# haowenz/chromap

Measured on AMD Instinct MI355X. Metric: M paired reads mapped/s (ATAC preset, GRCh38 index), higher is better.
Workload: dtype u64

## Files before the change

chromap_amd/csrc/cm_api.hip:

```cpp
#include <hip/hip_runtime.h>
#include <math.h>
#include <stdio.h>
#include <stdlib.h>
#include <string.h>

#include <string>
#include <vector>

#include "../../include/chromap_amd.h"
#include "cm_ctx.h"
#include "cm_kernels.h"
#include "cm_classes.h"
#include "cm_summary.h"
#include "cm_coop.h"
#include <chrono>
#include <mutex>
#include "cm_mapq_tables.h"

static thread_local std::string g_last_error;

#define HIPCHECK(ctx, call)                                                                      \
  do {                                                                                           \
    hipError_t e_ = (call);                                                                      \
    if (e_ != hipSuccess) {                                                                      \
// ... 770 lines not shown
  CmDev d;
  uint32_t n_mm = 0;
  bool s3a_done = false;
  uint32_t n_heavy[CM_HV_LISTS] = {};
  unsigned long long hits_total = 0;
  uint32_t n_hits = 0;
  bool planes = false;
  bool spec = false;
  uint32_t n_m = 0;
  void bind() { cm_bind_dev(c, d, rlo, rhi); }
};
static int stage_begin(RangeRun &r) {
  cmgpu_ctx *c = r.c;
  c->n_ev = 0;
  c->use_perm = false;
  const int rc = ensure_pair_arrays(c, r.n);
  if (rc) return rc;
  HIPCHECK(c, hipMemsetAsync(c->stats.p, 0, CM_ST_N * 8, r.s));
  memset(&r.d, 0, sizeof(r.d));
  cm_ensure_goff(c);
  cm_set_classes(c, r.d);
  r.bind();
  mark(c, "begin");
  if (c->has_barcodes) {
    cm_launch_k_s0b_barcode(r.d, r.n, r.s);
    mark(c, "s0b_barcode");
  }
  return CMGPU_OK;
}
struct MmChunks {
  uint32_t n_chunks;
  uint32_t lo[CM_MM_CHUNKS + 1];
  uint64_t entries[CM_MM_CHUNKS];
  uint32_t part_off[CM_MM_CHUNKS + 1];
};
static uint32_t mm_chunk_count(const RangeRun &r) { return r.n >= (1u << 20) ? (uint32_t)r.c->opt.mm_chunks : (r.n >= (1u << 17) ? 2 : 1); }
static void mm_probe_grids(const cmgpu_ctx *c, MmChunks &k) {
  k.part_off[0] = 0;
  for (uint32_t ch = 0; ch < k.n_chunks; ++ch) k.part_off[ch + 1] = k.part_off[ch] + cm_probe_range_blocks(k.entries[ch], c->opt.probe_variant);
}
template <class Fill>
static int mm_fill_and_probe(RangeRun &r, const MmChunks &k, uint32_t mm_cap, Fill fill) {
  cmgpu_ctx *c = r.c;
  const unsigned long long *marks = (const unsigned long long *)c->mm_marks.p;
  HIPCHECK(c, hipMemsetAsync(r.d.stats + CM_ST_PROBE_STEPS, 0, 2 * 8, r.s));
  for (uint32_t ch = 0; ch < k.n_chunks; ++ch) {
    fill(ch);
    HIPCHECK(c, hipEventRecord(c->chunk_ev[ch], r.s));
    HIPCHECK(c, hipStreamWaitEvent(c->stream2, c->chunk_ev[ch], 0));
    cm_launch_k_probe_range(r.d, marks + ch, k.entries[ch], mm_cap, (uint2 *)c->partials.p + k.part_off[ch], c->stream2, c->opt.probe_variant);
  }
  HIPCHECK(c, hipEventRecord(c->chunk_ev[CM_MM_CHUNKS], c->stream2));
  HIPCHECK(c, hipStreamWaitEvent(r.s, c->chunk_ev[CM_MM_CHUNKS], 0));
  cm_launch_k_probe_reduce(c->partials.p, k.part_off[k.n_chunks], r.d.stats + CM_ST_PROBE_STEPS, r.s);
  return CMGPU_OK;
}
static int stage_minimizers_fused(RangeRun &r, bool flat) {
  cmgpu_ctx *c = r.c; CmDev &d = r.d; hipStream_t s = r.s;
  const uint32_t n = r.n, n2 = r.n2;
  int rc;
  uint64_t cap = (uint64_t)n2 * (c->max_read_len / 4 + 3);
  const uint64_t bound = (uint64_t)c->bases0 + c->bases1 + 1;
  if (cap > bound) cap = bound;
  const uint32_t ppb = flat ? 128u : cm_prep_mm_pairs_per_block(d, c->max_read_len);
  const uint64_t per_read_bound = c->max_read_len > (uint32_t)c->p.k ? c->max_read_len - (uint32_t)c->p.k + 1 : 1;
  MmChunks k;
  k.n_chunks = mm_chunk_count(r);
  for (int attempt = 0; attempt < 2; ++attempt) {
    if (cap > r.limit) return CM_RC_SPLIT;
    k.lo[0] = 0;
    uint32_t chunk_pairs = 0;
    for (uint32_t ch = 0; ch < k.n_chunks; ++ch) {
      uint64_t hi = (uint64_t)n * (ch + 1) / k.n_chunks;
      hi = ch + 1 == k.n_chunks ? n : hi / ppb * ppb;
      k.lo[ch + 1] = (uint32_t)hi;
      const uint32_t pairs = k.lo[ch + 1] - k.lo[ch];
      chunk_pairs = pairs > chunk_pairs ? pairs : chunk_pairs;
      const uint64_t me = 2ull * pairs * (attempt == 0 ? (uint64_t)(c->max_read_len / 4 + 3) : per_read_bound);
      k.entries[ch] = me > cap ? cap : me;
    }
    mm_probe_grids(c, k);
    if (c->mm_hash.ensure((size_t)cap * 8 + 8) || c->mm_ps.ensure((size_t)cap * 4 + 4) || c->pr_val.ensure((size_t)cap * 8 + 8) ||
        (!flat && c->mm_stage.ensure(cm_prep_mm_stage_bytes(d, c->max_read_len, chunk_pairs) + 8)) ||
        c->pr_kind.ensure((size_t)cap + 4) || c->mm_cursor.ensure(8) || c->mm_marks.ensure((CM_MM_CHUNKS + 1) * 8) ||
        c->partials.ensure(((size_t)k.part_off[k.n_chunks] + 1) * 8 + cm_stats_partial_words(n) * 8)) {
      cm_set_error(c, "out of device memory (minimizers)"); return CMGPU_ENOMEM;
    }
    r.bind();
    HIPCHECK(c, hipMemsetAsync(c->mm_cursor.p, 0, 8, s));
    HIPCHECK(c, hipMemsetAsync(c->mm_marks.p, 0, 8, s));
    unsigned long long *cursor = (unsigned long long *)c->mm_cursor.p, *marks = (unsigned long long *)c->mm_marks.p;
    rc = mm_fill_and_probe(r, k, (uint32_t)cap, [&](uint32_t ch) {
      if (flat) cm_launch_k_prep_flat(d, k.lo[ch], k.lo[ch + 1], c->max_read_len, (uint32_t)c->opt.prep_tile_reads, (uint32_t)cap, cursor, s);
      else cm_launch_k_prep_mm(d, k.lo[ch], k.lo[ch + 1], c->max_read_len, (uint32_t)cap, cursor, s, c->mm_stage.p);
      cm_launch_k_copy_u64(cursor, marks + ch + 1, s);
    });
    if (rc) return rc;
    d.mm_cap = (uint32_t)cap;
    HIPCHECK(c, hipMemsetAsync(c->hv_cnt.p, 0, 256, s));
    cm_launch_k_s3a_count(d, n2, s);
    d.mm_cap = 0;
    if ((rc = scan_with_total(c, d.hit_tot, d.hit_off, n2, &r.hits_total, false))) return rc;
    HIPCHECK(c, hipMemcpyAsync(r.n_heavy, c->hv_cnt.p, sizeof(r.n_heavy), hipMemcpyDeviceToHost, s));
    r.s3a_done = true;
    unsigned long long hm[CM_MM_CHUNKS + 1];
    HIPCHECK(c, hipMemcpyAsync(hm, marks, ((size_t)k.n_chunks + 1) * 8, hipMemcpyDeviceToHost, s));
    HIPCHECK(c, cm_stream_sync(s));
    const unsigned long long tot = hm[k.n_chunks];
    bool grid_short = false;
    if (attempt == 0 && tot <= cap)
      for (uint32_t ch = 0; ch < k.n_chunks; ++ch) grid_short = grid_short || hm[ch + 1] - hm[ch] > k.entries[ch];
    if (tot <= cap && !grid_short) { r.n_mm = (uint32_t)tot; break; }
    if (attempt == 1) { cm_set_error(c, "minimizer arrays overflowed twice"); return CMGPU_ECAPACITY; }
    cap = bound;
  }
  mark(c, "s0_s1_s2_trim_minimizers_probe");
  return CMGPU_OK;
}
static int stage_minimizers_two_pass(RangeRun &r) {
  cmgpu_ctx *c = r.c; CmDev &d = r.d; hipStream_t s = r.s;
  int rc;
  cm_launch_k_prep_count(d, r.n, c->max_read_len, s);
  unsigned long long mm_total = 0;
  if ((rc = scan_with_total(c, d.mm_cnt, d.mm_off, r.n2, &mm_total))) return rc;
  if (mm_total > r.limit) return CM_RC_SPLIT;
  const uint32_t n_mm = r.n_mm = (uint32_t)mm_total;
  mark(c, "s0_s1a_trim_count");
  if (c->mm_hash.ensure((size_t)n_mm * 8 + 8) || c->mm_ps.ensure((size_t)n_mm * 4 + 4) || c->pr_val.ensure((size_t)n_mm * 8 + 8) ||
      c->pr_kind.ensure((size_t)n_mm + 4)) { cm_set_error(c, "out of device memory (minimizers)"); return CMGPU_ENOMEM; }
  r.bind();
  MmChunks k;
  k.n_chunks = mm_chunk_count(r);
  for (uint32_t ch = 0; ch <= k.n_chunks; ++ch) k.lo[ch] = (uint32_t)((uint64_t)r.n * ch / k.n_chunks);
  if (c->mm_marks.ensure((CM_MM_CHUNKS + 1) * 8)) { cm_set_error(c, "out of device memory (minimizers)"); return CMGPU_ENOMEM; }
  unsigned long long *marks = (unsigned long long *)c->mm_marks.p;
  unsigned long long hm[CM_MM_CHUNKS + 1];
  cm_launch_k_mm_marks(d.mm_off, k.lo, k.n_chunks + 1, marks, s);
  HIPCHECK(c, hipMemcpyAsync(hm, marks, ((size_t)k.n_chunks + 1) * 8, hipMemcpyDeviceToHost, s));
  HIPCHECK(c, cm_stream_sync(s));
  for (uint32_t ch = 0; ch < k.n_chunks; ++ch) k.entries[ch] = hm[ch + 1] - hm[ch];
  mm_probe_grids(c, k);
  if (c->partials.ensure(((size_t)k.part_off[k.n_chunks] + 1) * 8 + cm_stats_partial_words(r.n) * 8)) { cm_set_error(c, "out of device memory (partials)"); return CMGPU_ENOMEM; }
  if ((rc = mm_fill_and_probe(r, k, n_mm, [&](uint32_t ch) { cm_launch_k_mm_fill(d, k.lo[ch], k.lo[ch + 1], c->max_read_len, s); }))) return rc;
  mark(c, "s1b_s2_minimizers_probe");
  return CMGPU_OK;
}
static int stage_pack_reads(RangeRun &r) {
  cmgpu_ctx *c = r.c;
  r.planes = c->ref_pl_words != 0 && c->opt.planes;
  if (r.planes && c->read_planes.ensure((size_t)r.n2 * cm_read_pl_stride((c->max_read_len + 31) / 32) * 4 + 16)) r.planes = false;
  if (!r.planes) return CMGPU_OK;
  if (!c->stream_pack) {
    int prio_least = 0, prio_greatest = 0;
    (void)hipDeviceGetStreamPriorityRange(&prio_least, &prio_greatest);
    HIPCHECK(c, hipStreamCreateWithPriority(&c->stream_pack, hipStreamNonBlocking, prio_greatest));
  }
  HIPCHECK(c, hipEventRecord(c->chunk_ev[1], r.s));
  HIPCHECK(c, hipStreamWaitEvent(c->stream_pack, c->chunk_ev[1], 0));
  r.d.read_pl = (uint32_t *)c->read_planes.p; r.d.read_pl_w = (c->max_read_len + 31) / 32;
  cm_launch_k_pack_reads(r.d, r.n2, c->stream_pack);
  HIPCHECK(c, hipEventRecord(c->chunk_ev[0], c->stream_pack));
  return CMGPU_OK;
}
static int stage_s3_candidates(RangeRun &r) {
  cmgpu_ctx *c = r.c; CmDev &d = r.d; hipStream_t s = r.s;
  const uint32_t n2 = r.n2;
  if (!r.s3a_done) {
    HIPCHECK(c, hipMemsetAsync(c->hv_cnt.p, 0, 256, s));
    cm_launch_k_s3a_count(d, n2, s);
    HIPCHECK(c, hipMemcpyAsync(r.n_heavy, c->hv_cnt.p, sizeof(r.n_heavy), hipMemcpyDeviceToHost, s));
    const int rc = scan_with_total(c, d.hit_tot, d.hit_off, n2, &r.hits_total);
    if (rc) return rc;
  }
  if (r.hits_total > r.limit) return CM_RC_SPLIT;
  r.n_hits = (uint32_t)r.hits_total;
  if (c->hbuf.ensure((size_t)r.n_hits * 8 + 8) || c->hcnt.ensure((size_t)r.n_hits + 4)) { cm_set_error(c, "out of device memory (hits)"); return CMGPU_ENOMEM; }
  r.bind();
  mark(c, "s3a_count");
  cm_launch_k_s3b_candidates(d, n2, c->max_read_len, s);
  const uint32_t *nh = r.n_heavy;
  cm_launch_k_s3b_heavy(d, nh, s, (c->opt.coop & 1) != 0, c->max_read_len);
  c->use_perm = (uint64_t)nh[CM_L_HIT_B256B] + nh[CM_L_HIT_SLAB] + nh[CM_L_HIT_B512] + nh[CM_L_HIT_B1024] > n2 / 65536 || (uint64_t)nh[CM_L_HIT_WAVE] + nh[CM_L_HIT_WAVE_SMALL] + nh[CM_L_HIT_B256A] > n2 / 256;
  if (c->opt.heavy_last) c->use_perm = c->opt.heavy_last > 0;
  if (c->use_perm) {
    uint32_t *tmp = (uint32_t *)c->hv_tmp.p;
    cm_build_heavy_last(d, r.n, (uint32_t *)c->scratch_a.p, tmp, (uint32_t *)c->scratch_b.p, tmp + n2 + 1, (uint32_t *)c->perm_reads.p,
                        (uint32_t *)c->perm_pairs.p, (uint32_t *)c->scan_tmp.p, s);
  }
  r.bind();
  mark(c, "s3b_candidates");
  return CMGPU_OK;
}
static void size_rescue_pool(RangeRun &r) {
  cmgpu_ctx *c = r.c;
  uint64_t waves = (uint64_t)r.n2 / 512 + 64;
  if (waves > 8192) waves = 8192;
  const uint64_t slack = c->rs_pool_want ? waves * CM_POOL_GRANT / 2 : 0;
  uint64_t want = c->rs_pool_want + c->rs_pool_want / 4 + slack;
  if (c->rs_pool_want > c->rs_pool_cap) want = 2 * c->rs_pool_want + slack;
  if (want < (1u << 22)) want = 1u << 22;
  if (want > 0xfffffff0ull) want = 0xfffffff0ull;
  const auto dbg_t0 = std::chrono::steady_clock::now();
  if (c->rs_pool.ensure((size_t)want * 8) == 0 && c->rs_pool_off.ensure((size_t)r.n2 * 2 * 4 + 16) == 0) c->rs_pool_cap = (uint32_t)(c->rs_pool.cap / 8 > 0xfffffff0ull ? 0xfffffff0ull : c->rs_pool.cap / 8);
  else { c->rs_pool.release(); c->rs_pool_cap = 0; }
  if (cm_debug_pool()) fprintf(stderr, "pool ensure want %llu: %.3f ms\n", (unsigned long long)want, std::chrono::duration<double, std::milli>(std::chrono::steady_clock::now() - dbg_t0).count());
  r.bind();
}
static int stage_s4_rescue_filter(RangeRun &r) {
  cmgpu_ctx *c = r.c; CmDev &d = r.d; hipStream_t s = r.s;
  const uint32_t n2 = r.n2;
  const bool coop = (c->opt.coop & 2) != 0;
  HIPCHECK(c, hipMemsetAsync(c->rs_cnt.p, 0, CM_RS_SEGS * 64, s));
  if (coop) size_rescue_pool(r);
  cm_launch_k_s4a_rescue_count(d, n2, s, coop);
  cm_launch_k_s4a_rescue_list(d, n2, s, coop);
  unsigned long long m_total = 0;
  r.spec = r.allow_spec && c->opt.spec && c->pred_m_ok && (c->pred_n == r.n || c->pred_n == 0xffffffffu) && c->m_cap > 0 && c->m_cap <= r.limit;
  if (r.spec) {
    unsigned long long *acc = (unsigned long long *)c->stats.p + CM_ST_TOTAL;
    HIPCHECK(c, hipMemsetAsync(acc, 0, 8, s));
    cm_launch_k_sum_u32(d.m_tot, n2, acc, s);
    cm_scan_u32(d.m_tot, d.m_off, n2, (uint32_t *)c->scan_tmp.p, s);
    cm_launch_k_check_cap(acc, c->m_cap, (unsigned long long *)c->stats.p + CM_ST_ABORT, s);
    r.n_m = (uint32_t)c->m_cap;
  } else {
    const int rc = scan_with_total(c, d.m_tot, d.m_off, n2, &m_total);
    if (rc) return rc;
    if (m_total > r.limit) return CM_RC_SPLIT;
    uint64_t want = m_total + m_total / 4 + 1024;
    if (want > r.limit) want = r.limit;
    if (want < m_total) want = m_total;
    r.n_m = (uint32_t)want;
    if (cm_ensure_candidate_arrays(c, r.n_m)) { cm_set_error(c, "out of device memory (candidates)"); return CMGPU_ENOMEM; }
    c->m_cap = r.n_m;
  }
  if (cm_debug_pool()) fprintf(stderr, "spec %d m_cap %llu m_total %llu\n", (int)r.spec, (unsigned long long)c->m_cap, m_total);
  r.bind();
  mark(c, "s4a_rescue_count");
  cm_launch_k_s4b_rescue_merge(d, n2, s, coop, c->max_read_len);
  cm_launch_k_s4b_rescue_list(d, n2, s, coop, c->max_read_len);
  mark(c, "s4b_rescue_merge");
  HIPCHECK(c, hipMemsetAsync(c->srt_cnt.p, 0, 8, s));
  cm_launch_k_s4c_reduce(d, r.n, s, (uint32_t)c->opt.coop & (c->p.split ? ~8u : ~0u));
  if (c->use_perm) cm_launch_k_sort_lists(d, 0, s);
  mark(c, "s4c_pair_filter");
  return CMGPU_OK;
}
static int stage_s5_verify(RangeRun &r) {
  cmgpu_ctx *c = r.c; const CmDev &d = r.d; hipStream_t s = r.s;
  const bool coop = (c->opt.coop & 8) != 0 && !c->p.split;
  if (r.planes) HIPCHECK(c, hipStreamWaitEvent(s, c->chunk_ev[0], 0));
  cm_launch_k_s5a_prepare(d, r.n2, s, coop);
  cm_scan_u32(d.nv, d.v_off, r.n2, (uint32_t *)c->scan_tmp.p, s);
  mark(c, "s5a_prepare");
  cm_launch_k_s5b_verify(d, r.n_m, r.n2, s);
  mark(c, "s5b_verify");
  HIPCHECK(c, hipMemsetAsync(c->srt_cnt.p, 0, 8, s));
  cm_launch_k_s5c_finalize(d, r.n2, s, coop);
  if (c->use_perm) cm_launch_k_sort_lists(d, 1, s);
  mark(c, "s5c_accept");
  return CMGPU_OK;
}
static int stage_s6_records(RangeRun &r) {
  cmgpu_ctx *c = r.c; CmDev &d = r.d; hipStream_t s = r.s;
  const uint32_t n = r.n;
  const bool coop = (c->opt.coop & 16) != 0;
  if (c->p.sam) {
    const uint64_t slots = c->single ? n : r.n2, slot0 = c->single ? r.rlo : 2ull * r.rlo;
    const uint32_t md_cap = c->sam_md_cap;
    const uint32_t zw = (2 * c->p.e + 2 <= 18) ? 5 : 8;
    if (c->sam_z.ensure((size_t)c->max_read_len * zw * 4 * n + 16)) { cm_set_error(c, "out of device memory (SAM buffers)"); return CMGPU_ENOMEM; }
    HIPCHECK(c, hipMemsetAsync((uint8_t *)c->sam_rec.p + slot0 * 40, 0, slots * 40, s));
    d.sam_rec = (uint8_t *)c->sam_rec.p + slot0 * 40; d.sam_cigar = (uint32_t *)c->sam_cigar.p + slot0 * CM_SAM_CIGAR_CAP;
    d.sam_md = (uint8_t *)c->sam_md.p + slot0 * md_cap;
    d.sam_z = (uint32_t *)c->sam_z.p; d.sam_md_cap = md_cap;
  }
  if (c->p.sam) cm_launch_k_s6a_pair_sam(d, n, s); else cm_launch_k_s6a_pair(d, n, s, coop);
  mark(c, "s6a_pairing");
  const uint32_t n_chunks = cm_num_chunks_host(n, (uint32_t)c->p.ref_batch, (uint32_t)c->p.grain);
  cm_launch_k_s6b_sample(d, n_chunks, s);
  if (c->p.sam) cm_launch_k_s6c_multi_sam(d, n, s); else cm_launch_k_s6c_multi(d, n, s, coop);
  mark(c, "s6bc_multimappers");
  return CMGPU_OK;
}
static int stage_finish(RangeRun &r, uint64_t *k_out, cmgpu_stats *stats) {
  cmgpu_ctx *c = r.c; hipStream_t s = r.s;
  cm_launch_k_stats(r.d, r.n, (unsigned long long *)c->partials.p, s);
  unsigned long long hst[CM_ST_N];
  uint32_t h_cls[CM_HV_LISTS];
  HIPCHECK(c, hipMemcpyAsync(hst, c->stats.p, sizeof(hst), hipMemcpyDeviceToHost, s));
  HIPCHECK(c, hipMemcpyAsync(h_cls, c->hv_cnt.p, sizeof(h_cls), hipMemcpyDeviceToHost, s));
  HIPCHECK(c, cm_stream_sync(s));
  mark(c, "stats");
  HIPCHECK(c, cm_stream_sync(s));
  const bool aborted = r.spec && hst[CM_ST_ABORT];
  if (!aborted) {
    unsigned long long seen = 0, keep = 0;
    for (uint32_t l = 6; l < CM_HV_LISTS; ++l) if (h_cls[l]) seen |= 1ull << (l == 31 ? 23 : l);
    if (seen & ~r.d.cls_mask) return CM_RC_AGAIN_ALL_CLASSES;
    for (uint32_t l = 0; l < 64; ++l) {
      if ((seen >> l) & 1ull) c->cls_age[l] = 32; else if (c->cls_age[l]) --c->cls_age[l];
      if (c->cls_age[l]) keep |= 1ull << l;
    }
    c->cls_seen = keep;
  } else {
    c->pred_m_ok = false;
    return CM_RC_AGAIN_EXACT_SIZES;
  }
  c->pred_m_ok = true;
  c->pred_n = r.n;
  c->rs_pool_want = hst[CM_ST_POOL];
  if (cm_debug_pool()) fprintf(stderr, "pool: cap %u entries, asked %llu\n", c->rs_pool_cap, (unsigned long long)hst[CM_ST_POOL]);
  if (hst[CM_ST_ERR]) { cm_set_error(c, "internal device error flag " + std::to_string((unsigned long long)hst[CM_ST_ERR])); return CMGPU_ECAPACITY; }
  *k_out = hst[CM_ST_RECORDS];
  c->last_range_lo = r.rlo; c->last_range_hi = r.rhi;
  c->last_n_mm = r.n_mm; c->last_n_hits = r.n_hits; c->last_n_cand_cap = r.n_m;
  if (stats) {
    stats->num_candidates += hst[CM_ST_CAND]; stats->num_mappings += hst[CM_ST_MAPPINGS];
    stats->num_mapped_reads += hst[CM_ST_MAPPED]; stats->num_uniquely_mapped_reads += hst[CM_ST_UNIQ];
    stats->num_minimizers += r.n_mm; stats->probe_steps += hst[CM_ST_PROBE_STEPS]; stats->occurrences_read += hst[CM_ST_OCC];
    stats->num_pairs_rescued += hst[CM_ST_RESCUED]; stats->num_multi_mappers += hst[CM_ST_MULTI];
    stats->num_barcode_in_whitelist += hst[CM_ST_BC_INWL]; stats->num_corrected_barcode += hst[CM_ST_BC_CORR];
  }
  return CMGPU_OK;
}
static int map_range(cmgpu_ctx *c, uint32_t rlo, uint32_t rhi, uint64_t *k_out, cmgpu_stats *stats) {
  bool allow_spec = true;
  int rc;
  *k_out = 0;
  for (;;) {
    RangeRun r = {c, rlo, rhi, rhi - rlo, 2 * (rhi - rlo), allow_spec, c->opt.item_limit, c->stream};
    rc = stage_begin(r);
    if (!rc) {
      const bool flat = c->opt.prep_kernel == 1 && cm_prep_flat_supported(r.d, c->max_read_len, (uint32_t)c->opt.prep_tile_reads);
      const bool fused = flat || (cm_prep_mm_supported(r.d, c->max_read_len) && (c->max_read_len <= 69 || c->opt.long_fused));
      rc = fused ? stage_minimizers_fused(r, flat) : stage_minimizers_two_pass(r);
    }
    if (!rc) rc = stage_pack_reads(r);
    if (!rc) rc = stage_s3_candidates(r);
    if (!rc) rc = stage_s4_rescue_filter(r);
    if (!rc) rc = stage_s5_verify(r);
    if (!rc) rc = stage_s6_records(r);
    if (!rc) rc = stage_finish(r, k_out, stats);
    if (rc == CM_RC_AGAIN_ALL_CLASSES) c->cls_all = true;
    else if (rc == CM_RC_AGAIN_EXACT_SIZES) allow_spec = false;
    else break;
  }
  c->cls_all = false;
  return rc;
}

static int map_split(cmgpu_ctx *c, uint32_t lo, uint32_t hi, uint64_t *k_total, cmgpu_stats *stats) {
  uint64_t k = 0;
  int rc = map_range(c, lo, hi, &k, stats);
  const uint32_t rb = (uint32_t)c->p.ref_batch, n = hi - lo;
  if (rc != CM_RC_SPLIT) { *k_total += k; return rc; }
  if (n <= rb) {
    cm_set_error(c, "a reference batch of " + std::to_string(n) + " pairs needs more than " + std::to_string((unsigned long long)c->opt.item_limit) +
                        " entries in one intermediate array (hits / candidates)");
    return CMGPU_ECAPACITY;
  }
  uint32_t half = (n / 2) / rb * rb;
  if (half == 0) half = rb;
  rc = map_split(c, lo, lo + half, k_total, stats);
  if (rc) return rc;
  return map_split(c, lo + half, hi, k_total, stats);
}

static int lane_prepare(cmgpu_ctx *c, size_t i) {
  while (c->lanes.size() <= i) {
    cmgpu_ctx *l = nullptr;
    const int rc = cmgpu_create_shared(c, &l);
    if (rc) { cm_set_error(c, std::string("lane context: ") + cmgpu_last_error(nullptr)); return rc; }
    c->lanes.push_back(l);
  }
  cmgpu_ctx *l = c->lanes[i];
  auto view = [](DevBuf &dst, const DevBuf &src) { dst.p = src.p; dst.cap = src.cap; dst.owned = false; };
  view(l->bkt_fast, c->bkt_fast); l->fmask = c->fmask;
  view(l->ref_planes, c->ref_planes); l->ref_pl_words = c->ref_pl_words;
  view(l->rb0, c->rb0); view(l->rb1, c->rb1); view(l->ro0, c->ro0); view(l->ro1, c->ro1);
  view(l->rec, c->rec); view(l->rec_ok, c->rec_ok);
// ... 779 lines not shown
```

chromap_amd/csrc/cm_coop.h:

```cpp
#ifndef CM_COOP_H_
#define CM_COOP_H_

#include "cm_stages.h"

CM_HD uint32_t cm_min_u32(uint32_t a, uint32_t b) { return a < b ? a : b; }
CM_HD unsigned long long cm_fetch_add64(unsigned long long *p, unsigned long long v) {
#if defined(__HIP_DEVICE_COMPILE__)
  return atomicAdd(p, v);
#else
  const unsigned long long old = *p;
  *p = old + v;
  return old;
#endif
}
#if defined(__HIP_DEVICE_COMPILE__)
#define CM_PROF_ON(p) ((p) && (blockIdx.x & 31u) == 0u)
#define CM_PROF_BEGIN(d) long long cm_prof_t_ = CM_PROF_ON((d).prof) ? clock64() : 0
#define CM_PROF_MARK(d, g, k) do { if (CM_PROF_ON((d).prof) && (g).t == 0) { const long long now_ = clock64(); atomicAdd(&(d).prof[k], (unsigned long long)(now_ - cm_prof_t_)); cm_prof_t_ = clock64(); } } while (0)
#define CM_PROF_RESET(d) do { if (CM_PROF_ON((d).prof)) cm_prof_t_ = clock64(); } while (0)
#define CM_PROF_COUNT(d, g, k, v) do { if (CM_PROF_ON((d).prof) && (g).t == 0) atomicAdd(&(d).prof[k], (unsigned long long)(v)); } while (0)
#define CM_PROF_PTR_COUNT(p, g, k, v) do { if ((p) && (g).t == 0) atomicAdd(&(p)[k], (unsigned long long)(v)); } while (0)
#define CM_PROF_PTR_BEGIN(p) long long cm_prof_u_ = CM_PROF_ON(p) ? clock64() : 0
#define CM_PROF_PTR_MARK(p, g, k) do { if (CM_PROF_ON(p) && (g).t == 0) { const long long now_ = clock64(); atomicAdd(&(p)[k], (unsigned long long)(now_ - cm_prof_u_)); cm_prof_u_ = clock64(); } } while (0)
#else
// ... 1169 lines not shown
    const bool paired = lo < n2 && !(p2[lo] > a + dist);
    m.k1[i] = paired ? 1 : 0;
    m.x1[i] = paired ? c1[i] : 0;
    if (lo == n2 && i < my_end) my_end = i;
  }
  const uint32_t i_end = (uint32_t)g.min64((uint64_t)my_end);
  for (uint32_t j = g.t; j < n2; j += G) {
    const uint64_t b = p2[j];
    uint32_t lo = 0, hi = n1;
    while (lo < hi) {
      const uint32_t mid = (lo + hi) >> 1;
      if (b > p1[mid] + dist) lo = mid + 1; else hi = mid;
    }
    const bool covered = lo < n1 && !(p1[lo] > b + dist);
    m.k2[j] = covered ? 1 : 0;
    m.x2[j] = covered ? c2[j] : 0;
  }
  g.sync();
  (void)cm_coop_array_scan_max(g, m.x1, n1);
  (void)cm_coop_array_scan_max(g, m.x2, n2);
  for (uint32_t i = g.t; i < n1; i += G) {
    uint32_t cond = 0;
    if (!m.k1[i] && i < i_end) {
      const uint32_t mx = m.x1[i] > 6 ? m.x1[i] : 6;
      cond = ((p1[i] >> 32) == (p2[m.lo1[i]] >> 32) && (uint32_t)c1[i] >= mx) ? 1u : 0u;
    }
    m.of1[i] = (uint16_t)cond;
  }
  for (uint32_t j = g.t; j < n2; j += G) {
    uint32_t cond = 0;
    if (!m.k2[j]) {
      const uint64_t b = p2[j];
      uint32_t lo = 0, hi = n1;
      while (lo < hi) {
        const uint32_t mid = (lo + hi) >> 1;
        if (p1[mid] > b + dist) hi = mid; else lo = mid + 1;
      }
      if (lo < n1) {
        const uint32_t mx = m.x2[j] > 6 ? m.x2[j] : 6;
        cond = ((p1[lo] >> 32) == (b >> 32) && (uint32_t)c2[j] >= mx) ? 1u : 0u;
      }
    }
    m.of2[j] = (uint16_t)cond;
  }
  g.sync();
  for (uint32_t i = g.t; i < n1; i += G) m.x1[i] = (uint8_t)m.of1[i];
  for (uint32_t j = g.t; j < n2; j += G) m.x2[j] = (uint8_t)m.of2[j];
  g.sync();
  (void)cm_coop_array_scan_add(g, m.of1, n1);
  (void)cm_coop_array_scan_add(g, m.of2, n2);
  for (uint32_t i = g.t; i < n1; i += G) {
    const bool keep = (m.k1[i] && i < i_end) || (m.x1[i] && m.of1[i] < 5);
    m.k1[i] = keep ? 1 : 0;
  }
  for (uint32_t j = g.t; j < n2; j += G) {
    const bool keep = m.k2[j] || (m.x2[j] && m.of2[j] < 5);
    m.k2[j] = keep ? 1 : 0;
  }
  g.sync();
  for (uint32_t i = g.t; i < n1; i += G) m.of1[i] = m.k1[i];
  for (uint32_t j = g.t; j < n2; j += G) m.of2[j] = m.k2[j];
  g.sync();
  const uint32_t t1 = cm_coop_array_scan_add(g, m.of1, n1);
  const uint32_t t2 = cm_coop_array_scan_add(g, m.of2, n2);
  for (uint32_t i = g.t; i < n1; i += G)
    if (m.k1[i]) { f1[m.of1[i]] = p1[i]; fc1[m.of1[i]] = c1[i]; }
  for (uint32_t j = g.t; j < n2; j += G)
    if (m.k2[j]) { f2[m.of2[j]] = p2[j]; fc2[m.of2[j]] = c2[j]; }
  *nf1 = t1;
  *nf2 = t2;
}

template <bool STAGED, class GT>
CM_HD void cm_coop_s4c(const CmDev &d, uint32_t pair, GT &g, const CmCoopPairMem &m) {
  const uint32_t r1 = 2 * pair, r2 = r1 + 1;
  const uint32_t G = (uint32_t)GT::G;
  const uint32_t mo1 = d.m_off[r1], mo2 = d.m_off[r2], sh1 = d.ncp[r1] + d.resc_p[r1], sh2 = d.ncp[r2] + d.resc_p[r2];
  const uint32_t mcp1 = d.mcp[r1], mcn1 = d.mcn[r1], mcp2 = d.mcp[r2], mcn2 = d.mcn[r2];
  if (mcp1 > m.P || mcn1 > m.P || mcp2 > m.P || mcn2 > m.P) {
    if (g.t == 0) { cm_s4c_filter(d, pair); cm_s4c_post(d, pair); }
    return;
  }
  uint32_t a, b, c, e2;
  cm_coop_reduce_dir<STAGED>(g, m, (uint32_t)d.p.max_insert, d.mbuf + mo1, d.mcnt + mo1, mcp1, d.mbuf + mo2 + sh2, d.mcnt + mo2 + sh2, mcn2,
                     d.fbuf + mo1, d.fcnt + mo1, &a, d.fbuf + mo2 + sh2, d.fcnt + mo2 + sh2, &b);
  g.sync();
  cm_coop_reduce_dir<STAGED>(g, m, (uint32_t)d.p.max_insert, d.mbuf + mo1 + sh1, d.mcnt + mo1 + sh1, mcn1, d.mbuf + mo2, d.mcnt + mo2, mcp2,
                     d.fbuf + mo1 + sh1, d.fcnt + mo1 + sh1, &c, d.fbuf + mo2, d.fcnt + mo2, &e2);
  g.sync();
  const bool alive = a + c > 0 && b + e2 > 0;
  if (g.t == 0) {
    d.fcp[r1] = a; d.fcn[r2] = b; d.fcn[r1] = c; d.fcp[r2] = e2;
    d.alive[pair] = alive ? 1 : 0;
  }
  if (alive && d.rid_rank) {
    uint64_t *l[4] = {d.fbuf + mo1, d.fbuf + mo1 + sh1, d.fbuf + mo2, d.fbuf + mo2 + sh2};
    const uint32_t n[4] = {a, c, e2, b};
    for (int q = 0; q < 4; ++q)
      for (uint32_t i = g.t; i < n[q]; i += G) l[q][i] = (l[q][i] & 0xffffffffull) | ((uint64_t)d.rid_rank[(uint32_t)(l[q][i] >> 32)] << 32);
  }
}

template <class GT>
CM_HD uint32_t cm_coop_array_scan_max16(GT &g, uint16_t *a, uint32_t n) {
  const uint32_t VT = cm_coop_chunk(n, (uint32_t)GT::G);
  const uint32_t c0 = cm_min_u32(n, g.t * VT), c1 = cm_min_u32(n, c0 + VT);
  uint32_t mx = 0;
  for (uint32_t i = c0; i < c1; ++i) mx = a[i] > mx ? a[i] : mx;
  uint32_t total;
  uint32_t run = g.scanmax(mx, &total);
  for (uint32_t i = c0; i < c1; ++i) { const uint32_t x = a[i]; a[i] = (uint16_t)run; run = x > run ? x : run; }
  g.sync();
  return total;
}

struct CmTwo { int lo, n_lo, hi, n_hi; };
CM_HD void cm_two_add(CmTwo &s, int v, int cnt) {
  if (cnt <= 0) return;
  if (v < s.lo) { s.hi = s.lo; s.n_hi = s.n_lo; s.lo = v; s.n_lo = cnt; }
  else if (v == s.lo) s.n_lo += cnt;
  else if (v == s.hi) s.n_hi += cnt;
  else if (v < s.hi) { s.hi = v; s.n_hi = cnt; }
}
template <class GT>
CM_HD CmTwo cm_coop_two_merge(GT &g, const CmTwo &mine, int none) {
  const int BIAS = 1 << 20;
  CmTwo out;
  out.lo = (int)g.min64((uint64_t)(mine.lo + BIAS)) - BIAS;
  out.n_lo = (int)g.sum(mine.lo == out.lo ? (uint32_t)mine.n_lo : 0u);
  const int c2 = mine.lo > out.lo ? mine.lo : mine.hi;
  out.hi = (int)g.min64((uint64_t)(c2 + BIAS)) - BIAS;
  out.n_hi = (int)g.sum((mine.lo == out.hi ? (uint32_t)mine.n_lo : 0u) + (mine.hi == out.hi ? (uint32_t)mine.n_hi : 0u));
  if (out.lo == none) { out.n_lo = 0; out.hi = none; out.n_hi = 0; }
  if (out.hi == none) out.n_hi = 0;
  return out;
}

struct CmCoopVerMem {
  uint16_t *of, *fr, *pm;
  int16_t *pe;
  uint8_t *vf;
  uint8_t *sc;
  uint32_t P;
};
CM_HD size_t cm_coop_ver_mem_bytes(uint32_t P) { return (size_t)(P + 1) * 6 + (size_t)P * 4 + 32; }
CM_HD CmCoopVerMem cm_coop_ver_mem_at(uint8_t *base, uint32_t P) {
  CmCoopVerMem m;
  m.P = P;
  m.of = reinterpret_cast<uint16_t *>(base);
  m.fr = m.of + P + 1;
  m.pm = m.fr + P + 1;
  m.pe = reinterpret_cast<int16_t *>(m.pm + P + 1);
  m.vf = reinterpret_cast<uint8_t *>(m.pe + P);
  m.sc = m.vf + P;
  return m;
}
template <class GT>
CM_HD uint32_t cm_coop_draft_strand(const CmDev &d, GT &g, const CmCoopVerMem &m, uint32_t L, int strand, const uint64_t *cp, const uint8_t *cc,
                                    uint32_t nc, CmTwo &best, uint64_t *dp, int16_t *de, const int16_t *pre_err, const int16_t *pre_end) {
  const uint32_t G = (uint32_t)GT::G;
  const int e = d.p.e;
  const uint32_t lanes = (uint32_t)d.p.lanes;
  if (nc == 0) return 0;
  for (uint32_t ci = g.t; ci < nc; ci += G) {
    const uint64_t cpos = cp[ci];
    m.pe[ci] = pre_err[ci];
    m.sc[ci] = cc[ci];
    const uint32_t rid = (uint32_t)(cpos >> 32);
    uint32_t position = (uint32_t)cpos;
    if (strand == 1) position = position - L + 1;
// ... 416 lines not shown
```

chromap_amd/csrc/cm_kernels.h:

```cpp
#ifndef CM_KERNELS_H_
#define CM_KERNELS_H_
#include <hip/hip_runtime.h>

#include "cm_types.h"

#define CM_SLAB_CAP 65535u
#define CM_SLAB_BLOCKS 128u
#define CM_DECL_LAUNCH(kname) void cm_launch_##kname(const CmDev &d, uint32_t n, hipStream_t s);
void cm_launch_k_prep_count(const CmDev &d, uint32_t n_pairs, uint32_t max_read_len, hipStream_t s);
void cm_launch_k_mm_fill(const CmDev &d, uint32_t pair_lo, uint32_t pair_hi, uint32_t max_read_len, hipStream_t s);
void cm_launch_k_mm_marks(const uint32_t *mm_off, const uint32_t *lo, uint32_t n_marks, unsigned long long *marks, hipStream_t s);
bool cm_prep_mm_supported(const CmDev &d, uint32_t max_read_len);
bool cm_prep_flat_supported(const CmDev &d, uint32_t max_read_len, uint32_t tile_reads);
void cm_launch_k_prep_flat(const CmDev &d, uint32_t pair_lo, uint32_t pair_hi, uint32_t max_read_len, uint32_t tile_reads, uint32_t mm_cap,
                           unsigned long long *cursor, hipStream_t s);
uint32_t cm_prep_mm_pairs_per_block(const CmDev &d, uint32_t max_read_len);
size_t cm_prep_mm_stage_bytes(const CmDev &d, uint32_t max_read_len, uint32_t pairs);
void cm_launch_k_prep_mm(const CmDev &d, uint32_t pair_lo, uint32_t pair_hi, uint32_t max_read_len, uint32_t mm_cap,
                         unsigned long long *cursor, hipStream_t s, void *gstage);
uint32_t cm_probe_range_blocks(uint64_t max_entries, int variant);
void cm_launch_k_probe_range(const CmDev &d, const unsigned long long *range, uint64_t max_entries, uint32_t cap, void *partials, hipStream_t s, int variant);
void cm_launch_k_probe_reduce(const void *partials, uint32_t blocks, unsigned long long *counters, hipStream_t s);
CM_DECL_LAUNCH(k_s3a_count)
void cm_launch_k_sort_lists(const CmDev &d, int mode, hipStream_t s);
uint32_t cm_s3b_lane_cap(uint32_t max_read_len);
void cm_s3b_heavy_classes(uint32_t *hv_max, uint32_t *hv_big);
void cm_launch_k_s3b_heavy(const CmDev &d, const uint32_t *n_cls, hipStream_t s, bool coop, uint32_t max_read_len);
void cm_launch_k_s3b_candidates(const CmDev &d, uint32_t n, uint32_t max_read_len, hipStream_t s);
void cm_launch_k_s4a_rescue_count(const CmDev &d, uint32_t n, hipStream_t s, bool coop);
void cm_launch_k_s4b_rescue_merge(const CmDev &d, uint32_t n, hipStream_t s, bool coop, uint32_t max_read_len);
uint32_t cm_rescue_seg_cap(uint32_t n_reads);
void cm_launch_k_s4a_rescue_list(const CmDev &d, uint32_t n_reads, hipStream_t s, bool coop);
void cm_launch_k_s4b_rescue_list(const CmDev &d, uint32_t n_reads, hipStream_t s, bool coop, uint32_t max_read_len);
void cm_launch_k_s4c_reduce(const CmDev &d, uint32_t n, hipStream_t s, uint32_t coop);
void cm_launch_k_s5a_prepare(const CmDev &d, uint32_t n, hipStream_t s, bool coop);
void cm_launch_k_s5c_finalize(const CmDev &d, uint32_t n, hipStream_t s, bool coop);
void cm_launch_k_s5b_verify(const CmDev &d, uint32_t max_items, uint32_t n_reads, hipStream_t s);
void cm_launch_k_s6a_pair(const CmDev &d, uint32_t n, hipStream_t s, bool coop);
void cm_launch_k_s6c_multi(const CmDev &d, uint32_t n, hipStream_t s, bool coop);
CM_DECL_LAUNCH(k_s6a_pair_sam)
CM_DECL_LAUNCH(k_s6c_multi_sam)
void cm_launch_k_s6b_sample(const CmDev &d, uint32_t n_chunks, hipStream_t s);
void cm_launch_k_s0b_barcode(const CmDev &d, uint32_t n, hipStream_t s);
void cm_launch_k_bc_abundance(const uint8_t *bcb, const uint32_t *bco, uint32_t lo, uint32_t hi, uint64_t *wl, uint32_t wl_mask,
                              unsigned long long *num_sample, hipStream_t s);
size_t cm_probe_partial_words(uint32_t n);
void cm_launch_k_probe(const uint64_t *bkt, uint32_t bmask, const uint64_t *hash, uint64_t *val, uint8_t *kind,
                       uint32_t n, void *partials, unsigned long long *counters, hipStream_t s, int variant = 0);
size_t cm_stats_partial_words(uint32_t n);
void cm_launch_k_stats(const CmDev &d, uint32_t n, unsigned long long *partials, hipStream_t s);

void cm_build_heavy_last(const CmDev &d, uint32_t n_pairs, uint32_t *fr, uint32_t *sr, uint32_t *fp, uint32_t *sp, uint32_t *perm_reads,
                         uint32_t *perm_pairs, uint32_t *scan_tmp, hipStream_t s);
void cm_launch_k_pack_ref(const uint8_t *ref, uint64_t n_bytes, CmPlRec *pl, hipStream_t s);
void cm_launch_k_pack_reads(const CmDev &d, uint32_t n_reads, hipStream_t s);
void cm_launch_k_check_cap(const unsigned long long *total, unsigned long long cap, unsigned long long *flag, hipStream_t s);
void cm_launch_k_copy_u64(const unsigned long long *src, unsigned long long *dst, hipStream_t s);
void cm_launch_k_sum_u32(const uint32_t *in, uint32_t n, unsigned long long *out, hipStream_t s);
size_t cm_scan_tmp_words(uint32_t n);
void cm_scan_u32(const uint32_t *in, uint32_t *out, uint32_t n, uint32_t *tmp, hipStream_t s);

#endif
```

chromap_amd/csrc/cm_kernels.hip:

```cpp
#include <hip/hip_runtime.h>
#include <stdio.h>
#include <string.h>
#include <cstring>
#include <atomic>
#include <map>
#include <mutex>
#include <utility>
#include <rocprim/rocprim.hpp>

#include "cm_kernels.h"
#include "cm_stages.h"
#include "cm_coop.h"

#define CM_BLOCK 256

#define CM_ITEM_KERNEL(kname, fn, perm)                                      \
  __global__ __launch_bounds__(CM_BLOCK) void kname(CmDev d, uint32_t n) {   \
    if (d.abort && *d.abort) return;                                         \
    const uint32_t i = blockIdx.x * CM_BLOCK + threadIdx.x;                  \
    if (i < n) fn(d, d.perm ? d.perm[i] : i);                                \
  }



extern __shared__ __align__(16) uint8_t cm_lds[];
static inline dim3 grid_for_n(uint32_t n) { return dim3((n + CM_BLOCK - 1) / CM_BLOCK); }

__device__ __forceinline__ void cm_stage_range(uint8_t *dst, const uint8_t *src, uint64_t a0, uint64_t g1) {
  for (uint64_t off = a0 + (uint64_t)threadIdx.x * 16; off < g1; off += (uint64_t)blockDim.x * 16)
    *reinterpret_cast<uint4 *>(dst + (off - a0)) = *reinterpret_cast<const uint4 *>(src + off);
}

struct CmStaged { const uint8_t *m0, *m1; };
__device__ __forceinline__ CmStaged cm_stage_pairs(const CmDev &d, uint32_t p0, uint32_t p1, uint32_t pair, uint32_t lds_half) {
  const uint64_t g0a = d.ro0[p0], g0b = d.ro0[p1], g1a = d.ro1[p0], g1b = d.ro1[p1];
  const uint64_t a0 = g0a & ~15ull, a1 = g1a & ~15ull;
  uint8_t *l0 = cm_lds, *l1 = cm_lds + lds_half;
  cm_stage_range(l0, d.rb0, a0, g0b);
  cm_stage_range(l1, d.rb1, a1, g1b);
  __syncthreads();
  CmStaged s;
  s.m0 = l0 + (d.ro0[pair < p1 ? pair : p0] - a0);
  s.m1 = l1 + (d.ro1[pair < p1 ? pair : p0] - a1);
  return s;
}

__global__ void k_prep_count(CmDev d, uint32_t n_pairs, uint32_t lds_half) {
  const uint32_t PB = blockDim.x >> 1;
  const uint32_t p0 = blockIdx.x * PB, p1 = p0 + PB < n_pairs ? p0 + PB : n_pairs;
  const uint32_t t = threadIdx.x, lp = t < PB ? t : t - PB, pair = p0 + lp;
  const CmStaged s = cm_stage_pairs(d, p0, p1, pair, lds_half);
  if (t < PB && pair < p1) cm_s0_prep_ptr(d, pair, s.m0, s.m1);
  __syncthreads();
  if (pair < p1) cm_s1_count(d, 2 * pair + (t < PB ? 0 : 1), t < PB ? s.m0 : s.m1);
}

__global__ void k_mm_fill(CmDev d, uint32_t pair_lo, uint32_t n_pairs , uint32_t lds_half) {
  const uint32_t PB = blockDim.x >> 1;
  const uint32_t p0 = pair_lo + blockIdx.x * PB, p1 = p0 + PB < n_pairs ? p0 + PB : n_pairs;
  const uint32_t t = threadIdx.x, lp = t < PB ? t : t - PB, pair = p0 + lp;
  const CmStaged s = cm_stage_pairs(d, p0, p1, pair, lds_half);
  if (pair < p1) cm_s1_fill(d, 2 * pair + (t < PB ? 0 : 1), t < PB ? s.m0 : s.m1);
}

template <bool GSTAGE, bool E6>
__global__ void k_prep_mm(CmDev d, uint32_t pair_lo, uint32_t n_pairs , uint32_t lds_half, uint32_t stg,
                          uint32_t mm_cap, unsigned long long *cursor, uint64_t *gstage) {
  const uint32_t T = blockDim.x, PB = T >> 1;
  const uint32_t p0 = pair_lo + blockIdx.x * PB, p1 = p0 + PB < n_pairs ? p0 + PB : n_pairs;
  const uint32_t t = threadIdx.x, lp = t < PB ? t : t - PB, pair = p0 + lp;
  const CmStaged s = cm_stage_pairs(d, p0, p1, pair, lds_half);
  if (t < PB && pair < p1) cm_s0_prep_ptr(d, pair, s.m0, s.m1);
  __syncthreads();
  uint64_t *sh_e = GSTAGE ? gstage + (size_t)blockIdx.x * stg * T : reinterpret_cast<uint64_t *>(cm_lds + 2 * lds_half);
  uint32_t *sh_lo = reinterpret_cast<uint32_t *>(cm_lds + 2 * lds_half);
  uint16_t *sh_hi = reinterpret_cast<uint16_t *>(sh_lo + (size_t)stg * T);
  uint32_t *sh_w = reinterpret_cast<uint32_t *>(cm_lds + 2 * lds_half + (GSTAGE ? 0 : (size_t)stg * T * (E6 ? 6 : 8)));
  uint32_t *sh_off = sh_w + 16, *sh_cnt = sh_off + T + 1;
  const bool valid = pair < p1;
  const uint32_t r = 2 * pair + (t < PB ? 0 : 1);
  const uint8_t *seq = t < PB ? s.m0 : s.m1;
  const int k = d.p.k;
  const uint32_t hb = 2 * (uint32_t)k;
  uint32_t cnt = 0, len = 0;
  if (valid) {
    len = d.rlen[r];
    cnt = cm_minimizers_w7(seq, len, k, [&](uint32_t n, uint64_t h, uint32_t p) {
      const uint64_t v = h | ((uint64_t)p << hb);
      if (n < stg) { if (E6) { sh_lo[(size_t)n * T + t] = (uint32_t)v; sh_hi[(size_t)n * T + t] = (uint16_t)(v >> 32); } else sh_e[(size_t)n * T + t] = v; }
    });
  }
  const uint32_t lane = t & 63, wave = t >> 6;
  uint32_t incl = cnt;
#pragma unroll
  for (int dlt = 1; dlt < 64; dlt <<= 1) {
    const uint32_t v = __shfl_up(incl, dlt, 64);
    if (lane >= (uint32_t)dlt) incl += v;
  }
  if (lane == 63 || t == T - 1) sh_w[wave] = incl;
  __syncthreads();
  const uint32_t n_waves = (T + 63) >> 6;
  if (t == 0) {
    uint32_t tot = 0;
    for (uint32_t wv = 0; wv < n_waves; ++wv) { const uint32_t x = sh_w[wv]; sh_w[wv] = tot; tot += x; }
    const unsigned long long base = tot ? atomicAdd(cursor, (unsigned long long)tot) : 0ull;
    sh_w[8] = (uint32_t)base;
    sh_w[9] = (uint32_t)(base >> 32);
    sh_w[10] = tot;
  }
  __syncthreads();
  const unsigned long long base = (unsigned long long)sh_w[8] | ((unsigned long long)sh_w[9] << 32);
  const uint32_t loc = sh_w[wave] + (incl - cnt);
  const unsigned long long off64 = base + loc;
  const uint64_t hmask = (1ull << hb) - 1;
  if (valid) {
    d.mm_cnt[r] = cnt;
    d.mm_off[r] = (uint32_t)off64;
  }
  if (GSTAGE) {
    sh_off[t] = loc;
    sh_cnt[t] = cnt;
    if (t == T - 1) sh_off[T] = loc + cnt;
    __syncthreads();
    const uint32_t tot = sh_w[10];
    for (uint32_t o = t; o < tot; o += T) {
      uint32_t lo = 0, hi = T;
      while (hi - lo > 1) {
        const uint32_t mid = (lo + hi) >> 1;
        if (sh_off[mid] <= o) lo = mid; else hi = mid;
      }
      if (sh_cnt[lo] > stg || base + o >= mm_cap) continue;
      const uint64_t v = sh_e[(size_t)(o - sh_off[lo]) * T + lo];
      d.mm_hash[base + o] = v & hmask;
      d.mm_ps[base + o] = (uint32_t)(v >> hb);
    }
    if (valid && cnt > stg && off64 + cnt <= mm_cap) cm_minimizers_window<7>(seq, len, k, d.mm_hash + (uint32_t)off64, d.mm_ps + (uint32_t)off64, cnt);
    return;
  }
  if (!valid) return;
  if (cnt == 0 || off64 + cnt > mm_cap) return;
  const uint32_t off = (uint32_t)off64;
  if (cnt <= stg) {
    for (uint32_t e = 0; e < cnt; ++e) {
      const uint64_t v = E6 ? ((uint64_t)sh_lo[(size_t)e * T + t] | ((uint64_t)sh_hi[(size_t)e * T + t] << 32)) : sh_e[(size_t)e * T + t];
      d.mm_hash[off + e] = v & hmask;
      d.mm_ps[off + e] = (uint32_t)(v >> hb);
    }
  } else {
    cm_minimizers_window<7>(seq, len, k, d.mm_hash + off, d.mm_ps + off, cnt);
  }
}

struct CmFlatRead { uint32_t at; uint16_t cnt; uint8_t fb; uint8_t mate; };

__global__ __launch_bounds__(CM_BLOCK) void k_prep_flat(CmDev d, uint32_t pair_lo, uint32_t n_pairs ,
                                                        uint32_t lds_half, uint32_t nt_max, uint32_t tile_reads, uint32_t mm_cap,
                                                        unsigned long long *cursor) {
  constexpr uint32_t T = CM_BLOCK, PB = T / 2;
  const uint32_t p0 = pair_lo + blockIdx.x * PB, p1 = p0 + PB < n_pairs ? p0 + PB : n_pairs;
  const uint32_t t = threadIdx.x, lp = t < PB ? t : t - PB, pair = p0 + lp, mate = t < PB ? 0u : 1u;
  const int k = d.p.k;
  const uint32_t region0 = 2 * lds_half > 16 * nt_max ? 2 * lds_half : 16 * nt_max;
  const uint32_t nw = lds_half / 16 + 1;
  uint64_t *H = reinterpret_cast<uint64_t *>(cm_lds), *M = H + nt_max;
  uint32_t *pk0 = reinterpret_cast<uint32_t *>(cm_lds + region0), *pk1 = pk0 + nw + 3;
  uint16_t *bd0 = reinterpret_cast<uint16_t *>(pk1 + nw + 3), *bd1 = bd0 + nw + 1;
  CmFlatRead *ri = reinterpret_cast<CmFlatRead *>(reinterpret_cast<uint8_t *>(bd1 + nw + 1) + ((8 - ((uintptr_t)(2 * (nw + 1) * 2)) % 8) % 8));
  uint32_t *pos_off = reinterpret_cast<uint32_t *>(ri + T);
  uint16_t *meta = reinterpret_cast<uint16_t *>(pos_off + T + 1 + 1);
  uint16_t *pref = meta + nt_max + (nt_max & 1);
  uint32_t *misc = reinterpret_cast<uint32_t *>(pref + nt_max + 2 + (nt_max & 1));
  const uint64_t g0a = d.ro0[p0], g0b = d.ro0[p1], g1a = d.ro1[p0], g1b = d.ro1[p1];
  const uint64_t a0 = g0a & ~15ull, a1 = g1a & ~15ull;
  uint8_t *l0 = cm_lds, *l1 = cm_lds + lds_half;
  cm_stage_range(l0, d.rb0, a0, g0b);
  cm_stage_range(l1, d.rb1, a1, g1b);
  __syncthreads();
  const bool valid = pair < p1;
  const uint32_t off_m0 = valid ? (uint32_t)(d.ro0[pair] - a0) : 0u, off_m1 = valid ? (uint32_t)(d.ro1[pair] - a1) : 0u;
  {
    const uint32_t n0 = (uint32_t)(g0b - a0), n1 = (uint32_t)(g1b - a1);
    const uint32_t w0 = (n0 + 15) / 16, w1 = (n1 + 15) / 16;
    for (uint32_t w = t; w < w0 + w1; w += T) {
      const bool second = w >= w0;
      const uint32_t wi = second ? w - w0 : w;
      const uint4 q = *reinterpret_cast<const uint4 *>((second ? l1 : l0) + 16 * wi);
      uint32_t b0, b1, b2, b3;
      const uint32_t word = cm_mmf_pack4(q.x, &b0) | (cm_mmf_pack4(q.y, &b1) << 8) | (cm_mmf_pack4(q.z, &b2) << 16) | (cm_mmf_pack4(q.w, &b3) << 24);
      (second ? pk1 : pk0)[wi] = word;
      (second ? bd1 : bd0)[wi] = (uint16_t)(b0 | (b1 << 4) | (b2 << 8) | (b3 << 12));
    }
    if (t < 3) { pk0[w0 + t] = 0; pk1[w1 + t] = 0; }
    if (t == 3) { bd0[w0] = 0; bd1[w1] = 0; }
  }
  if (t < PB && valid) cm_s0_prep_ptr(d, pair, l0 + off_m0, l1 + off_m1);
  __syncthreads();
  const uint32_t r = 2 * pair + mate;
  uint32_t len = 0, cnt = 0, fb = 0;
  const uint32_t at = mate ? off_m1 : off_m0;
  if (valid) {
    len = d.rlen[r];
    const uint32_t m = len >= (uint32_t)k ? len - (uint32_t)k + 1 : 0;
    bool bad = false;
    if (m) {
      const uint16_t *bd = mate ? bd1 : bd0;
      const uint32_t wa = at >> 4, wb = (at + len - 1) >> 4;
      for (uint32_t w = wa; w <= wb; ++w) {
        uint32_t mk = bd[w];
        if (w == wa) mk &= 0xFFFFu << (at & 15u);
        if (w == wb) mk &= 0xFFFFu >> (15u - ((at + len - 1) & 15u));
        bad = bad || mk != 0;
      }
    }
    if (m && (bad || m < 7)) fb = 1; else cnt = m;
  }
  ri[t].at = at; ri[t].cnt = (uint16_t)cnt; ri[t].fb = (uint8_t)fb; ri[t].mate = (uint8_t)mate;
  {
    const uint32_t lane = t & 63, wave = t >> 6;
    uint32_t incl = cnt;
#pragma unroll
    for (int dlt = 1; dlt < 64; dlt <<= 1) {
      const uint32_t v = __shfl_up(incl, dlt, 64);
      if (lane >= (uint32_t)dlt) incl += v;
    }
    if (lane == 63) misc[wave] = incl;
    __syncthreads();
    uint32_t wbase = 0;
    for (uint32_t q = 0; q < wave; ++q) wbase += misc[q];
    pos_off[t] = wbase + incl - cnt;
    if (t == T - 1) pos_off[T] = wbase + incl;
  }
  __syncthreads();
  for (uint32_t r0 = 0; r0 < T; r0 += tile_reads) {
    const uint32_t r1 = r0 + tile_reads < T ? r0 + tile_reads : T;
    const uint32_t P0 = pos_off[r0], NT = pos_off[r1] - P0;
    const float per_pos = NT ? (float)(r1 - r0) / (float)NT : 0.0f;
    for (uint32_t p = t; p < NT; p += T) {
      uint32_t lr = r0 + (uint32_t)((float)p * per_pos);
      lr = lr < r1 ? lr : r1 - 1;
      while (pos_off[lr + 1] - P0 <= p) ++lr;
      while (pos_off[lr] - P0 > p) --lr;
      const uint32_t i = p - (pos_off[lr] - P0);
      uint32_t sd;
      H[p] = cm_mmf_hash(cm_mmf_kmer(ri[lr].mate ? pk1 : pk0, ri[lr].at + i, k), k, &sd);
      meta[p] = (uint16_t)(((lr - r0) << 7) | (i << 1) | sd);
    }
    __syncthreads();
    for (uint32_t p = t; p < NT; p += T) {
      const uint32_t mt = meta[p], lr = r0 + (mt >> 7), i = (mt >> 1) & 63u, m = ri[lr].cnt;
      if (i + 7 <= m) {
        uint64_t x = H[p];
#pragma unroll
        for (int q = 1; q < 6; ++q) x = H[p + q] < x ? H[p + q] : x;
        const uint64_t h6 = H[p + 6];
        if (i == 0 && h6 == x) ri[lr].fb = 2;
        M[p] = h6 < x ? h6 : x;
      }
    }
    __syncthreads();
    for (uint32_t p = t; p < NT; p += T) {
      const uint32_t mt = meta[p], lr = r0 + (mt >> 7), i = (mt >> 1) & 63u, m = ri[lr].cnt;
      const uint32_t j0 = i >= 6 ? i - 6 : 0, j1 = i + 7 <= m ? i : m - 7, b = p - i;
      uint64_t x = 0;
      for (uint32_t j = j0; j <= j1; ++j) x = M[b + j] > x ? M[b + j] : x;
      const bool fl = x == H[p] && ri[lr].fb == 0;
      meta[p] = (uint16_t)(mt | (fl ? 0x8000u : 0u));
    }
    __syncthreads();
    {
      const uint32_t chunk = (NT + T - 1) / T, c0 = t * chunk < NT ? t * chunk : NT, c1 = c0 + chunk < NT ? c0 + chunk : NT;
      uint32_t sum = 0;
      for (uint32_t p = c0; p < c1; ++p) sum += meta[p] >> 15;
      const uint32_t lane = t & 63, wave = t >> 6;
      uint32_t incl = sum;
#pragma unroll
      for (int dlt = 1; dlt < 64; dlt <<= 1) {
        const uint32_t v = __shfl_up(incl, dlt, 64);
        if (lane >= (uint32_t)dlt) incl += v;
      }
      if (lane == 63) misc[8 + wave] = incl;
      __syncthreads();
      uint32_t run = incl - sum;
      for (uint32_t q = 0; q < wave; ++q) run += misc[8 + q];
      for (uint32_t p = c0; p < c1; ++p) { pref[p] = (uint16_t)run; run += meta[p] >> 15; }
      if (t == T - 1) {
        pref[NT] = (uint16_t)run;
        const unsigned long long base = run ? atomicAdd(cursor, (unsigned long long)run) : 0ull;
        misc[16] = (uint32_t)base; misc[17] = (uint32_t)(base >> 32);
      }
    }
    __syncthreads();
    const unsigned long long base = (unsigned long long)misc[16] | ((unsigned long long)misc[17] << 32);
    for (uint32_t p = t; p < NT; p += T) {
      const uint32_t mt = meta[p];
      if (mt >> 15) {
        const unsigned long long o = base + pref[p];
        if (o < mm_cap) { d.mm_hash[o] = H[p]; d.mm_ps[o] = ((((mt >> 1) & 63u) + (uint32_t)k - 1u) << 1) | (mt & 1u); }
      }
    }
    if (t >= r0 && t < r1 && valid && ri[t].fb == 0) {
      const uint32_t a = pos_off[t] - P0, b = pos_off[t + 1] - P0;
      d.mm_cnt[r] = (uint32_t)pref[b] - (uint32_t)pref[a];
      d.mm_off[r] = (uint32_t)(base + pref[a]);
    }
    __syncthreads();
  }
  if (valid && ri[t].fb) {
    const uint8_t *seq = cm_read_ptr(d, r);
    const uint32_t c = cm_minimizers_window<7>(seq, len, k, nullptr, nullptr, 0);
    const unsigned long long off = c ? atomicAdd(cursor, (unsigned long long)c) : 0ull;
    d.mm_cnt[r] = c;
    d.mm_off[r] = (uint32_t)off;
    if (c && off + c <= mm_cap) cm_minimizers_window<7>(seq, len, k, d.mm_hash + off, d.mm_ps + off, c);
  }
}

__global__ __launch_bounds__(CM_BLOCK) void k_s3a_count(CmDev d, uint32_t n) {
  const uint32_t i = blockIdx.x * CM_BLOCK + threadIdx.x;
  uint32_t tot = 0;
  if (i < n) {
    cm_s3a_count(d, i);
    tot = d.hit_tot[i];
  }
  const uint32_t cls = tot <= d.s3b_cap ? 5u  : tot <= d.hv_mid ? CM_L_HIT_G16 : tot <= d.hv_sub ? CM_L_HIT_WAVE_SMALL : tot <= d.hv_max[0] ? CM_L_HIT_WAVE : tot <= d.hv_max[1] ? CM_L_HIT_B256A
                       : tot <= d.hv_max[2] ? CM_L_HIT_B256B : tot <= d.hv_max[3] ? CM_L_HIT_B512 : tot <= d.hv_big ? CM_L_HIT_B1024 : CM_L_HIT_SLAB;
  __shared__ uint32_t sh_cnt[8], sh_base[8];
  if (threadIdx.x < 8) sh_cnt[threadIdx.x] = 0;
  __syncthreads();
  const uint32_t lane = threadIdx.x & 63u;
  const uint32_t ids[8] = {CM_L_HIT_WAVE, CM_L_HIT_B256A, CM_L_HIT_B256B, CM_L_HIT_SLAB, CM_L_HIT_G16, CM_L_HIT_B512, CM_L_HIT_WAVE_SMALL, CM_L_HIT_B1024};
  uint32_t slot = 0, mine = 8;
#pragma unroll
  for (uint32_t q = 0; q < 8; ++q) {
    const unsigned long long m = __ballot(cls == ids[q]);
    if (m == 0) continue;
    uint32_t base = 0;
    if (lane == (uint32_t)(__ffsll((long long)m) - 1)) base = atomicAdd(&sh_cnt[q], (uint32_t)__popcll(m));
    base = __shfl(base, __ffsll((long long)m) - 1, 64);
    if (cls == ids[q]) { slot = base + (uint32_t)__popcll(m & ((1ull << lane) - 1ull)); mine = q; }
  }
  __syncthreads();
  if (threadIdx.x < 8 && sh_cnt[threadIdx.x]) sh_base[threadIdx.x] = atomicAdd(&d.hv_cnt[ids[threadIdx.x]], sh_cnt[threadIdx.x]);
  __syncthreads();
  if (mine < 8) d.hv_list[(size_t)ids[mine] * d.hv_stride + sh_base[mine] + slot] = i;
}
__global__ __launch_bounds__(CM_BLOCK) void k_s3b_candidates(CmDev d, uint32_t n, uint32_t cap) {
  uint64_t *sh_h = reinterpret_cast<uint64_t *>(cm_lds);
  uint8_t *sh_c = cm_lds + (size_t)cap * blockDim.x * 8;
  const uint32_t i = blockIdx.x * blockDim.x + threadIdx.x;
  if (i < n && d.hit_tot[i] <= cap) cm_s3b_candidates_lds(d, i, sh_h + threadIdx.x, sh_c + threadIdx.x, cap, blockDim.x);
}

template <int G>
__device__ __forceinline__ void cm_group_sync() {
  if (G <= 64) {
    __builtin_amdgcn_fence(__ATOMIC_RELEASE, "workgroup");
    __builtin_amdgcn_wave_barrier();
    __builtin_amdgcn_fence(__ATOMIC_ACQUIRE, "workgroup");
  } else {
    __syncthreads();
  }
}

template <int G>
__global__ __launch_bounds__(CM_BLOCK) void k_s3b_heavy(CmDev d, const uint32_t *__restrict__ list, uint32_t n_list, uint32_t P,
                                                        const uint32_t *__restrict__ n_list_dev) {
  constexpr int GPB = CM_BLOCK / G;
  const uint32_t grp = threadIdx.x / G, t = threadIdx.x % G;
  if (n_list_dev) n_list = *n_list_dev;
  uint64_t *S = reinterpret_cast<uint64_t *>(cm_lds) + (size_t)grp * P;
  uint16_t *oc = reinterpret_cast<uint16_t *>(cm_lds + (size_t)GPB * P * 8) + (size_t)grp * P;
  uint32_t *ctr = reinterpret_cast<uint32_t *>(cm_lds + (size_t)GPB * P * 10) + (size_t)grp * (G + 8);
  for (uint32_t gid = blockIdx.x * GPB + grp; gid < n_list; gid += gridDim.x * GPB) {
  const uint32_t r = list[gid];
  const uint32_t tot = d.hit_tot[r];
  const uint32_t b = d.mm_off[r], n = d.mm_cnt[r];
  const uint32_t maxf = d.round2[r] ? (uint32_t)d.p.f1 : (uint32_t)d.p.f0;
  const uint64_t SB = 1ull << 63;
  uint32_t P2 = 2;
  while (P2 < tot) P2 <<= 1;
  if (t == 0) { ctr[0] = 0; ctr[1] = 0; }
  for (uint32_t i = tot + t; i < P2; i += G) S[i] = ~0ull;
  cm_group_sync<G>();
  uint32_t my_pos = 0;
  if (G < 64) {
    for (uint32_t mi = t; mi < n; mi += G) {
      const uint8_t kind = d.pr_kind[b + mi];
      if (kind == CM_PR_MISS) continue;
      const uint64_t val = d.pr_val[b + mi];
      const uint32_t ps = d.mm_ps[b + mi];
      bool same;
      if (kind == CM_PR_SINGLE) {
        const uint64_t cp = cm_cand_from_hit(val, ps, d.p.k, &same);
        S[atomicAdd(&ctr[0], 1u)] = same ? cp : (cp | SB);
        my_pos += same ? 1u : 0u;
        continue;
      }
// ... 289 lines not shown
  const uint32_t o = r ^ 1u;
  return (d.ncp[o] >= CM_RS_HEAVY || d.ncn[o] >= CM_RS_HEAVY) && d.mm_cnt[r] <= CM_RS_MAXMM && !cm_rescue_is_wave(d, r, coop);
}
__device__ __forceinline__ void cm_group_best(const uint8_t *mc, uint32_t mn, uint32_t t, int *max_count, int *best_num) {
  int lmax = 0, lnum = 0;
  for (uint32_t i = t; i < mn; i += CM_RS_G) {
    const int c = mc[i];
    if (c > lmax) { lmax = c; lnum = 1; } else if (c == lmax) ++lnum;
  }
  for (int off = CM_RS_G / 2; off > 0; off >>= 1) {
    const int om = __shfl_xor(lmax, off, CM_RS_G), on = __shfl_xor(lnum, off, CM_RS_G);
    if (om > lmax) { lmax = om; lnum = on; } else if (om == lmax) lnum += on;
  }
  *max_count = lmax;
  *best_num = lnum;
}
__device__ __forceinline__ int cm_group_rescue_count(const CmDev &d, uint32_t r, int strand, const uint64_t *mp, const uint8_t *mc, uint32_t mn,
                                                     uint32_t t, uint32_t *cnt, uint32_t *rl) {
  int max_count, best_num;
  cm_group_best(mc, mn, t, &max_count, &best_num);
  *cnt = 0;
  if (cm_rescue_bails(d, max_count, best_num, mn)) {
    if (d.prof && t == 0) atomicAdd(&d.prof[26], 1ull);
    return -max_count;
  }
  const uint32_t b = d.mm_off[r], n = d.mm_cnt[r];
  if (d.prof && t == 0) {
    unsigned long long so = 0;
    for (uint32_t mi = 0; mi < n; ++mi) if (d.pr_kind[b + mi] == CM_PR_MULTI) so += (uint32_t)d.pr_val[b + mi];
    atomicAdd(&d.prof[16], 1ull); atomicAdd(&d.prof[17], (unsigned long long)best_num); atomicAdd(&d.prof[18], (unsigned long long)mn);
    atomicAdd(&d.prof[19], so); atomicAdd(&d.prof[20], (unsigned long long)n);
    atomicAdd(&d.prof[best_num < 4 ? 22 : best_num < 16 ? 23 : best_num < 64 ? 24 : 25], 1ull);
  }
  uint32_t lc = 0;
  for (uint32_t mi = t; mi < n; mi += CM_RS_G)
    lc += cm_rescue_minimizer(d, strand, mp, mc, mn, max_count, d.pr_kind[b + mi], d.pr_val[b + mi], d.mm_ps[b + mi], nullptr, nullptr);
  for (int off = CM_RS_G / 2; off > 0; off >>= 1) lc += __shfl_xor(lc, off, CM_RS_G);
  uint32_t rep_len = 0;
  if (t == 0) {
    uint32_t prev_rep = ~0u;
    for (uint32_t mi = 0; mi < n; ++mi) cm_rescue_rep(d, d.pr_kind[b + mi], d.pr_val[b + mi], d.mm_ps[b + mi], &rep_len, &prev_rep);
  }
  *rl = __shfl(rep_len, 0, CM_RS_G);
  *cnt = lc;
  if (d.prof && t == 0) atomicAdd(&d.prof[21], (unsigned long long)lc);
  return max_count;
}
__global__ __launch_bounds__(64) void k_s4a_rescue_list(CmDev d, uint32_t seg_cap, uint32_t coop) {
  const uint32_t cnt = d.rs_cnt[blockIdx.y * 16];
  const uint32_t *list = d.rs_list + (uint64_t)blockIdx.y * seg_cap;
  const long long t1 = d.prof ? clock64() : 0;
  for (uint32_t j = blockIdx.x * 64 + threadIdx.x; j < cnt; j += gridDim.x * 64) {
    const uint32_t r = list[j];
    if (!cm_rescue_is_heavy(d, r, coop)) cm_s4a_rescue(d, r);
  }
  const long long t2 = d.prof ? clock64() : 0;
  if (d.prof && threadIdx.x == 0) { const unsigned long long dt = (unsigned long long)(t2 - t1); atomicAdd(&d.prof[29], dt); atomicMax(&d.prof[30], dt); }
  const uint32_t t = threadIdx.x % CM_RS_G, grp = threadIdx.x / CM_RS_G, gpb = 64 / CM_RS_G;
  for (uint32_t j = blockIdx.x * gpb + grp; j < cnt; j += gridDim.x * gpb) {
    const uint32_t r = list[j];
    if (!cm_rescue_is_heavy(d, r, coop)) continue;
    const uint32_t o = r ^ 1u;
    uint32_t cntn = 0, cntp = 0, rl = 0, rl_val = 0;
    int res_neg = 0, res_pos = 0;
    bool set_rl = false;
    if (d.ncp[o] > 0) {
      res_neg = cm_group_rescue_count(d, r, 1, cm_c0_pos(d, o), cm_c0_pcnt(d, o), d.ncp[o], t, &cntn, &rl);
      if (res_neg >= 0) { set_rl = true; rl_val = rl; }
    }
    if (d.ncn[o] > 0) {
      res_pos = cm_group_rescue_count(d, r, 0, cm_c0_neg(d, o), cm_c0_ncnt(d, o), d.ncn[o], t, &cntp, &rl);
      if (res_pos >= 0) { set_rl = true; rl_val = rl; }
    }
    if (t == 0) {
      d.aug[r] = 1;
      d.res_neg[r] = res_neg; d.res_pos[r] = res_pos;
      d.resc_n[r] = cntn; d.resc_p[r] = cntp;
      if (set_rl) d.rep_len[r] = rl_val;
      d.m_tot[r] = d.ncp[r] + d.ncn[r] + cntn + cntp;
    }
  }
  if (d.prof && threadIdx.x == 0) { const unsigned long long dt = (unsigned long long)(clock64() - t2); atomicAdd(&d.prof[31], dt); atomicMax(&d.prof[15], dt); }
}
#define CM_S4B_COPY_MIN 64u
__global__ __launch_bounds__(CM_BLOCK) void k_s4b_rescue_merge(CmDev d, uint32_t n, uint32_t coop) {
  if (d.abort && *d.abort) return;
  const uint32_t i0 = blockIdx.x * CM_BLOCK + threadIdx.x;
  const uint32_t i = i0 < n ? (d.perm_reads ? d.perm_reads[i0] : i0) : 0u;
  const bool mine = i0 < n && !(d.aug[i] && d.resc_n[i] + d.resc_p[i] > 0);
  const bool to_wave = mine && coop && d.m_tot[i] > CM_S4B_COPY_MIN;
  if (mine && !to_wave) cm_s4b_rescue_merge(d, i);
  if (to_wave) { d.mcp[i] = 0; d.mcn[i] = 0; }
  if (coop) cm_wave_append(d.hv_list + (size_t)CM_L_RS_WAVE * d.hv_stride, d.hv_cnt + CM_L_RS_WAVE, to_wave, i);
}
__device__ __forceinline__ void cm_group_rescue_fill(const CmDev &d, uint32_t r, int strand, const uint64_t *mp, const uint8_t *mc, uint32_t mn,
                                                     uint32_t t, uint32_t *lds_cnt, uint64_t *out) {
  int max_count, best_num;
  cm_group_best(mc, mn, t, &max_count, &best_num);
  const uint32_t b = d.mm_off[r], n = d.mm_cnt[r];
  for (uint32_t mi = t; mi < n; mi += CM_RS_G)
    lds_cnt[mi] = cm_rescue_minimizer(d, strand, mp, mc, mn, max_count, d.pr_kind[b + mi], d.pr_val[b + mi], d.mm_ps[b + mi], nullptr, nullptr);
  cm_group_sync<CM_RS_G>();
  if (t == 0) {
    uint32_t run = 0;
    for (uint32_t mi = 0; mi < n; ++mi) { const uint32_t x = lds_cnt[mi]; lds_cnt[mi] = run; run += x; }
  }
  cm_group_sync<CM_RS_G>();
  for (uint32_t mi = t; mi < n; mi += CM_RS_G)
    (void)cm_rescue_minimizer(d, strand, mp, mc, mn, max_count, d.pr_kind[b + mi], d.pr_val[b + mi], d.mm_ps[b + mi], out + lds_cnt[mi], nullptr);
  cm_group_sync<CM_RS_G>();
}
#define CM_RS_COOP_MIN 32u
#define CM_S4B_PMAX 7680u
__host__ __device__ inline uint32_t cm_s4b_pmax(const CmDev &d) { return d.rs_big; }
__device__ __forceinline__ uint32_t cm_rescue_coop_class(const CmDev &d, uint32_t r, uint32_t coop) {
  const uint32_t big = d.resc_p[r] > d.resc_n[r] ? d.resc_p[r] : d.resc_n[r];
  if (!coop || big <= CM_RS_COOP_MIN || d.hv_max[0] == 0) return 0;
  return big <= d.hv_max[0] ? CM_L_RS_WAVE : big <= d.hv_max[1] ? CM_L_RS_B256A : big <= d.hv_max[2] ? CM_L_RS_B256B : big <= d.rs_max3 ? CM_L_RS_B512 : big <= d.rs_big ? CM_L_RS_B1024
         : (d.coop_slab && big <= d.coop_slab_cap) ? CM_L_RS_SLAB : 0u;
}
__global__ __launch_bounds__(64) void k_s4b_rescue_list(CmDev d, uint32_t seg_cap, uint32_t coop) {
  if (d.abort && *d.abort) return;
  __shared__ uint32_t sh_cnt[64 / CM_RS_G][CM_RS_MAXMM];
  const uint32_t cnt = d.rs_cnt[blockIdx.y * 16];
  const uint32_t *list = d.rs_list + (uint64_t)blockIdx.y * seg_cap;
  const long long tl0 = d.prof ? clock64() : 0;
  for (uint32_t j0 = blockIdx.x * 64; j0 < cnt; j0 += gridDim.x * 64) {
    const uint32_t j = j0 + threadIdx.x;
    const uint32_t r = j < cnt ? list[j] : 0u;
    const bool mine = j < cnt && d.resc_n[r] + d.resc_p[r] > 0 && !cm_rescue_is_heavy(d, r, coop);
    const uint32_t cls = mine ? cm_rescue_coop_class(d, r, coop) : 0u;
    if (mine) cm_s4b_rescue_merge(d, r, cls ? CM_S4B_FILL_ONLY : CM_S4B_ALL);
    for (uint32_t c = 6; c <= 8; ++c) cm_wave_append(d.hv_list + (size_t)c * d.hv_stride, d.hv_cnt + c, cls == c, r);
    cm_wave_append(d.hv_list + (size_t)CM_L_RS_B512 * d.hv_stride, d.hv_cnt + CM_L_RS_B512, cls == CM_L_RS_B512, r);
    cm_wave_append(d.hv_list + (size_t)CM_L_RS_B1024 * d.hv_stride, d.hv_cnt + CM_L_RS_B1024, cls == CM_L_RS_B1024, r);
    cm_wave_append(d.hv_list + (size_t)CM_L_RS_SLAB * d.hv_stride, d.hv_cnt + CM_L_RS_SLAB, cls == CM_L_RS_SLAB, r);
  }
  const long long tg0 = d.prof ? clock64() : 0;
  if (d.prof && threadIdx.x == 0) { const unsigned long long dt = (unsigned long long)(tg0 - tl0); atomicAdd(&d.prof[34], dt); atomicMax(&d.prof[35], dt); }
  const uint32_t t = threadIdx.x % CM_RS_G, grp = threadIdx.x / CM_RS_G, gpb = 64 / CM_RS_G;
  for (uint32_t j0 = blockIdx.x * gpb; j0 < cnt; j0 += gridDim.x * gpb) {
    const uint32_t j = j0 + grp;
    const uint32_t r = j < cnt ? list[j] : 0u;
    const bool mine = j < cnt && cm_rescue_is_heavy(d, r, coop) && d.resc_n[r] + d.resc_p[r] > 0;
    uint32_t cls = 0;
    if (mine) {
      const uint32_t o = r ^ 1u;
      const uint32_t ncp = d.ncp[r], ncn = d.ncn[r], rp = d.resc_p[r], rn = d.resc_n[r];
      uint64_t *P = d.mbuf + d.m_off[r];
      uint64_t *N = P + ncp + rp;
      if (d.ncp[o] > 0 && d.res_neg[r] >= 0 && rn > 0)
        cm_group_rescue_fill(d, r, 1, cm_c0_pos(d, o), cm_c0_pcnt(d, o), d.ncp[o], t, sh_cnt[grp], N + ncn);
      if (d.ncn[o] > 0 && d.res_pos[r] >= 0 && rp > 0)
        cm_group_rescue_fill(d, r, 0, cm_c0_neg(d, o), cm_c0_ncnt(d, o), d.ncn[o], t, sh_cnt[grp], P + ncp);
      if (t == 0) { d.mcp[r] = 0; d.mcn[r] = 0; }
      __threadfence_block();
      cls = cm_rescue_coop_class(d, r, coop);
      if (t == 0 && !cls) cm_s4b_rescue_merge(d, r, CM_S4B_PREFILLED);
    }
    for (uint32_t c = 6; c <= 8; ++c) cm_wave_append(d.hv_list + (size_t)c * d.hv_stride, d.hv_cnt + c, t == 0 && cls == c, r);
    cm_wave_append(d.hv_list + (size_t)CM_L_RS_B512 * d.hv_stride, d.hv_cnt + CM_L_RS_B512, t == 0 && cls == CM_L_RS_B512, r);
    cm_wave_append(d.hv_list + (size_t)CM_L_RS_B1024 * d.hv_stride, d.hv_cnt + CM_L_RS_B1024, t == 0 && cls == CM_L_RS_B1024, r);
    cm_wave_append(d.hv_list + (size_t)CM_L_RS_SLAB * d.hv_stride, d.hv_cnt + CM_L_RS_SLAB, t == 0 && cls == CM_L_RS_SLAB, r);
  }
  if (d.prof && threadIdx.x == 0) { const unsigned long long dt = (unsigned long long)(clock64() - tg0); atomicAdd(&d.prof[36], dt); atomicMax(&d.prof[37], dt); }
}
template <bool SMALL>
__global__ __launch_bounds__(64) void k_s4a_rescue_wave(CmDev d) {
  __shared__ __attribute__((aligned(16))) uint8_t rmem[SMALL ? CM_RESCUE_MEM_BYTES_S : CM_RESCUE_MEM_BYTES];
  const uint32_t li = SMALL ? CM_L_SEARCH_WAVE : CM_L_SEARCH_WAVE_BIG;
  const uint32_t cnt = d.hv_cnt[li];
  if (blockIdx.x >= cnt) return;
  const uint32_t *list = d.hv_list + (size_t)li * d.hv_stride;
  const CmCoopRescueMem m = SMALL ? cm_coop_rescue_mem_at(rmem, CM_RESCUE_WMAX_S, CM_RESCUE_PAIRS_S) : cm_coop_rescue_mem_at(rmem);
  CmDevGroup<64> g;
  g.t = threadIdx.x;
  g.xw = nullptr;
// ... 206 lines not shown
__global__ __launch_bounds__(CM_BLOCK) void k_sort_lists(CmDev d) {
  if (d.abort && *d.abort) return;
  const uint32_t wv = threadIdx.x >> 6, t = threadIdx.x & 63;
  uint64_t *K = reinterpret_cast<uint64_t *>(cm_lds) + (size_t)wv * CM_SORT_WAVE_MAX;
  uint16_t *V = reinterpret_cast<uint16_t *>(cm_lds + (size_t)(CM_BLOCK / 64) * CM_SORT_WAVE_MAX * 8) + (size_t)wv * CM_SORT_WAVE_MAX;
  const uint32_t n_items = d.srt_cnt[0];
  for (;;) {
    uint32_t item = 0;
    if (t == 0) item = atomicAdd(&d.srt_cnt[1], 1u);
    item = __shfl(item, 0, 64);
    if (item >= n_items) return;
    const uint32_t code = d.srt_list[item], r = code >> 1, strand = code & 1u;
    const uint32_t base = d.m_off[r] + (strand ? d.ncp[r] + d.resc_p[r] : 0);
    const uint32_t n = MODE == 0 ? (strand ? d.fcn[r] : d.fcp[r]) : (strand ? d.ndn[r] : d.ndp[r]);
    uint64_t *gk = (MODE == 0 ? d.fbuf : d.dpos) + base;
    uint32_t P2 = 2;
    while (P2 < n) P2 <<= 1;
    for (uint32_t i = t; i < P2; i += 64) {
      if (i < n) {
        K[i] = gk[i];
        V[i] = MODE == 0 ? (uint16_t)(255u - d.fcnt[base + i]) : (uint16_t)d.derr[base + i];
      } else {
        K[i] = ~0ull;
        V[i] = 0xffffu;
      }
    }
    cm_group_sync<64>();
    for (uint32_t k2 = 2; k2 <= P2; k2 <<= 1) {
      for (uint32_t j = k2 >> 1, lj = 31u - (uint32_t)__clz(k2 >> 1); j > 0; j >>= 1, --lj) {
        for (uint32_t i = t; i < (P2 >> 1); i += 64) {
          const uint32_t a = ((i >> lj) << (lj + 1)) | (i & (j - 1)), c = a + j;
          const uint64_t xa = K[a], xc = K[c];
          const uint16_t va = V[a], vc = V[c];
          const bool gt = MODE == 0 ? (va != vc ? va > vc : xa > xc) : (xa != xc ? xa > xc : va > vc);
          const bool up = (a & k2) == 0;
          if (gt == up && (xa != xc || va != vc)) { K[a] = xc; K[c] = xa; V[a] = vc; V[c] = va; }
        }
        cm_group_sync<64>();
      }
    }
    for (uint32_t i = t; i < n; i += 64) {
      gk[i] = K[i];
      if (MODE == 0) d.fcnt[base + i] = (uint8_t)(255u - V[i]); else d.derr[base + i] = (int16_t)V[i];
    }
    cm_group_sync<64>();
  }
}
void cm_launch_k_sort_lists(const CmDev &d, int mode, hipStream_t s) {
  const size_t lds = (size_t)(CM_BLOCK / 64) * CM_SORT_WAVE_MAX * 10;
  if (mode == 0) hipLaunchKernelGGL(k_sort_lists<0>, dim3(1024), dim3(CM_BLOCK), lds, s, d);
  else hipLaunchKernelGGL(k_sort_lists<1>, dim3(1024), dim3(CM_BLOCK), lds, s, d);
}
__global__ __launch_bounds__(CM_BLOCK) void k_s5b_verify(CmDev d, uint32_t n_reads) {
  if (d.abort && *d.abort) return;
  const uint32_t n_items = d.v_off[n_reads];
  for (uint32_t j = blockIdx.x * CM_BLOCK + threadIdx.x; j < n_items; j += gridDim.x * CM_BLOCK) cm_s5b_verify_item(d, j, n_reads);
}
#define CM_S6A_COOP_MIN 48u
#define CM_S6A_P_SMALL 256u
#define CM_S6A_P_WAVE 1024u
#define CM_S6A_P_BLOCK 8192u
__device__ __forceinline__ uint32_t cm_s6_class(const CmDev &d, uint32_t pair, uint32_t small_list, uint32_t wave_list, uint32_t block_list) {
  const uint32_t r1 = 2 * pair, r2 = r1 + 1;
  uint32_t big2 = d.ndp[r2] > d.ndn[r2] ? d.ndp[r2] : d.ndn[r2], big = big2;
  big = d.ndp[r1] > big ? d.ndp[r1] : big;
  big = d.ndn[r1] > big ? d.ndn[r1] : big;
  if (big <= CM_S6A_COOP_MIN) return 0;
  return big2 <= CM_S6A_P_SMALL ? small_list : big2 <= CM_S6A_P_WAVE ? wave_list : block_list;
}
__global__ __launch_bounds__(CM_BLOCK) void k_s6a_pair(CmDev d, uint32_t n, uint32_t coop) {
  if (d.abort && *d.abort) return;
  const uint32_t i = blockIdx.x * CM_BLOCK + threadIdx.x;
  const uint32_t pair = i < n ? (d.perm_pairs ? d.perm_pairs[i] : i) : 0u;
  uint32_t cls = 0;
  if (i < n && cm_s6a_pre<false>(d, pair)) {
    cls = coop ? cm_s6_class(d, pair, CM_L_S6A_SMALL, CM_L_S6A_WAVE, CM_L_S6A_BLOCK) : 0u;
    if (!cls) cm_s6a_sweeps<false>(d, pair);
  }
  if (coop) {
    cm_wave_append(d.hv_list + (size_t)CM_L_S6A_SMALL * d.hv_stride, d.hv_cnt + CM_L_S6A_SMALL, cls == CM_L_S6A_SMALL, pair);
    cm_wave_append(d.hv_list + (size_t)CM_L_S6A_WAVE * d.hv_stride, d.hv_cnt + CM_L_S6A_WAVE, cls == CM_L_S6A_WAVE, pair);
    cm_wave_append(d.hv_list + (size_t)CM_L_S6A_BLOCK * d.hv_stride, d.hv_cnt + CM_L_S6A_BLOCK, cls == CM_L_S6A_BLOCK, pair);
  }
}
template <int G>
__global__ __launch_bounds__(CM_BLOCK, 6) void k_s6a_coop(CmDev d, uint32_t P, uint32_t lid) {
  if (d.abort && *d.abort) return;
  const uint32_t gpb = blockDim.x / G, grp = threadIdx.x / G;
  const uint32_t n_list = d.hv_cnt[lid];
  const uint32_t *list = d.hv_list + (size_t)lid * d.hv_stride;
  const size_t gb = ((cm_coop_pe_mem_bytes(P) + 15) & ~(size_t)15) + CM_XW_BYTES;
  uint8_t *base = cm_lds + (size_t)grp * gb;
  const CmCoopPeMem m = cm_coop_pe_mem_at(base, P);
  CmDevGroup<G> g;
  g.t = threadIdx.x % G;
  g.xw = reinterpret_cast<uint32_t *>(base + gb - CM_XW_BYTES);
  for (uint32_t j = blockIdx.x * gpb + grp; j < n_list; j += gridDim.x * gpb) cm_coop_s6a<false>(d, list[j], g, m);
}
__global__ __launch_bounds__(CM_BLOCK) void k_s6c_multi(CmDev d, uint32_t n, uint32_t coop) {
  if (d.abort && *d.abort) return;
  const uint32_t i = blockIdx.x * CM_BLOCK + threadIdx.x;
  const uint32_t pair = i < n ? (d.perm_pairs ? d.perm_pairs[i] : i) : 0u;
  uint32_t cls = 0;
  if (i < n) {
    if (coop && !d.p.single && !d.p.split && d.pe_nbest[pair] > 1) cls = cm_s6_class(d, pair, CM_L_S6C_SMALL, CM_L_S6C_WAVE, CM_L_S6C_BLOCK);
    if (!cls) cm_s6c_multi<false>(d, pair);
  }
  if (coop) {
    cm_wave_append(d.hv_list + (size_t)CM_L_S6C_SMALL * d.hv_stride, d.hv_cnt + CM_L_S6C_SMALL, cls == CM_L_S6C_SMALL, pair);
    cm_wave_append(d.hv_list + (size_t)CM_L_S6C_WAVE * d.hv_stride, d.hv_cnt + CM_L_S6C_WAVE, cls == CM_L_S6C_WAVE, pair);
    cm_wave_append(d.hv_list + (size_t)CM_L_S6C_BLOCK * d.hv_stride, d.hv_cnt + CM_L_S6C_BLOCK, cls == CM_L_S6C_BLOCK, pair);
  }
}
template <int G>
__global__ __launch_bounds__(CM_BLOCK) void k_s6c_coop(CmDev d, uint32_t P, uint32_t lid) {
  if (d.abort && *d.abort) return;
  const uint32_t gpb = blockDim.x / G, grp = threadIdx.x / G;
  const uint32_t n_list = d.hv_cnt[lid];
  const uint32_t *list = d.hv_list + (size_t)lid * d.hv_stride;
  const size_t gb = ((cm_coop_pe_mem_bytes(P) + 15) & ~(size_t)15) + CM_XW_BYTES;
  uint8_t *base = cm_lds + (size_t)grp * gb;
  const CmCoopPeMem m = cm_coop_pe_mem_at(base, P);
  CmDevGroup<G> g;
  g.t = threadIdx.x % G;
  g.xw = reinterpret_cast<uint32_t *>(base + gb - CM_XW_BYTES);
  for (uint32_t j = blockIdx.x * gpb + grp; j < n_list; j += gridDim.x * gpb) cm_coop_s6c<false>(d, list[j], g, m);
}
CM_ITEM_KERNEL(k_s6a_pair_sam, cm_s6a_pair<true>, perm_pairs)
CM_ITEM_KERNEL(k_s6c_multi_sam, cm_s6c_multi<true>, perm_pairs)

__global__ __launch_bounds__(64) void k_s6b_sample(CmDev d, uint32_t n_chunks) {
  if (d.abort && *d.abort) return;
  const uint32_t chunk = blockIdx.x;
  if (chunk >= n_chunks) return;
  __shared__ CmMt g;
  uint32_t lo, hi;
  cm_chunk_range(d.n_pairs, (uint32_t)d.p.ref_batch, (uint32_t)d.p.grain, chunk, &lo, &hi);
  bool seeded = false;
  for (uint32_t base = lo; base < hi; base += 64) {
    const uint32_t pair = base + threadIdx.x;
    int nb = 0;
    if (pair < hi) nb = d.pe_nbest[pair];
    const bool multi = nb > 1 && (d.p.single || nb <= d.p.drop_rep);
    unsigned long long m = __ballot(multi);
    if (m == 0) continue;
    if (threadIdx.x == 0) {
      while (m) {
        if (!seeded || d.p.single) { cm_mt_seed(g, 11); seeded = true; }
        const int l = __ffsll((long long)m) - 1;
        m &= m - 1;
        const uint32_t pr = base + (uint32_t)l;
        cm_reservoir(d, pr, d.pe_nbest[pr], g);
      }
    }
    seeded = __shfl((int)seeded, 0, 64) != 0;
  }
}

__global__ __launch_bounds__(CM_BLOCK) void k_s0b_barcode(CmDev d, uint32_t n) {
  const uint32_t i = blockIdx.x * CM_BLOCK + threadIdx.x;
  uint32_t a = 0, b = 0;
  if (i < n) cm_s0b_barcode(d, i, &a, &b);
  for (int off = 32; off > 0; off >>= 1) {
    a += __shfl_down(a, off, 64);
    b += __shfl_down(b, off, 64);
  }
  __shared__ uint32_t sa[CM_BLOCK / 64], sb[CM_BLOCK / 64];
  if ((threadIdx.x & 63) == 0) { sa[threadIdx.x >> 6] = a; sb[threadIdx.x >> 6] = b; }
  __syncthreads();
  if (threadIdx.x == 0) {
    for (int j = 1; j < CM_BLOCK / 64; ++j) { a += sa[j]; b += sb[j]; }
    if (a) atomicAdd(&d.stats[CM_ST_BC_INWL], (unsigned long long)a);
    if (b) atomicAdd(&d.stats[CM_ST_BC_CORR], (unsigned long long)b);
  }
}

__global__ __launch_bounds__(CM_BLOCK) void k_bc_abundance(const uint8_t *__restrict__ bcb, const uint32_t *__restrict__ bco,
                                                            uint32_t lo, uint32_t hi, uint64_t *__restrict__ wl,
                                                            uint32_t wl_mask, unsigned long long *__restrict__ num_sample) {
  const uint32_t i = lo + blockIdx.x * CM_BLOCK + threadIdx.x;
  uint32_t hit = 0;
  if (i < hi) {
    const uint8_t *s = bcb + bco[i];
    const uint32_t l = bco[i + 1] - bco[i];
    bool has_n = false;
    for (uint32_t j = 0; j < l; ++j) has_n |= s[j] == 'N';
    if (!has_n) {
      const uint64_t key = cm_seed_from_sequence(s, l);
      const uint64_t x = key * 0x9E3779B97F4A7C15ull;
      uint32_t b = (uint32_t)(x >> 32) & wl_mask;
      for (;;) {
        const uint64_t k = wl[2 * (uint64_t)b];
        if (k == ~0ull) break;
        if (k == key) { atomicAdd(reinterpret_cast<unsigned long long *>(wl + 2 * (uint64_t)b + 1), 1ull); hit = 1; break; }
// ... 150 lines not shown
      const unsigned long long per = d.p.single ? 1ull : 2ull;
      if (nd1 > 0 && (d.p.single || nd2 > 0)) {
        const int nb = d.pe_nbest[pair];
        if (nb == 1) v[3] += per;
        v[1] += per * (unsigned long long)(nb < d.p.max_best ? nb : d.p.max_best);
        if (nb > 0) v[2] += per;
        if (nb > 1 && (d.p.single || nb <= d.p.drop_rep)) v[4] += 1;
      }
    }
    v[5] += (unsigned long long)d.aug[r1] + d.aug[r2];
    v[6] += (unsigned long long)d.hit_tot[r1] + d.hit_tot[r2];
    for (uint32_t t = 0; t < (uint32_t)d.p.max_best; ++t) v[7] += d.rec_ok[(uint64_t)pair * (uint32_t)d.p.max_best + t];
  }
  __shared__ unsigned long long sh[CM_BLOCK / 64][CM_NSTAT];
#pragma unroll
  for (int k = 0; k < CM_NSTAT; ++k) {
    unsigned long long x = v[k];
    for (int off = 32; off > 0; off >>= 1) x += __shfl_down(x, off, 64);
    if ((threadIdx.x & 63) == 0) sh[threadIdx.x >> 6][k] = x;
  }
  __syncthreads();
  if (threadIdx.x < CM_NSTAT) {
    unsigned long long x = 0;
    for (int j = 0; j < CM_BLOCK / 64; ++j) x += sh[j][threadIdx.x];
    partials[(uint64_t)blockIdx.x * CM_NSTAT + threadIdx.x] = x;
  }
}

__global__ __launch_bounds__(CM_BLOCK) void k_stats_reduce(const unsigned long long *__restrict__ partials,
                                                            uint32_t n_blocks, unsigned long long *__restrict__ stats) {
  const int k = threadIdx.x % CM_NSTAT, lane_row = threadIdx.x / CM_NSTAT;
  unsigned long long x = 0;
  for (uint32_t r = lane_row; r < n_blocks; r += CM_BLOCK / CM_NSTAT) x += partials[(uint64_t)r * CM_NSTAT + k];
  __shared__ unsigned long long sh[CM_BLOCK];
  sh[threadIdx.x] = x;
  __syncthreads();
  if (threadIdx.x < CM_NSTAT) {
    unsigned long long t = 0;
    for (int j = 0; j < CM_BLOCK / CM_NSTAT; ++j) t += sh[j * CM_NSTAT + threadIdx.x];
    const int slot[CM_NSTAT] = {CM_ST_CAND, CM_ST_MAPPINGS, CM_ST_MAPPED, CM_ST_UNIQ, CM_ST_MULTI, CM_ST_RESCUED, CM_ST_OCC, CM_ST_RECORDS};
    stats[slot[threadIdx.x]] += t;
  }
}

size_t cm_scan_tmp_words(uint32_t n) {
  size_t bytes = 0;
  (void)rocprim::exclusive_scan(nullptr, bytes, (const uint32_t *)nullptr, (uint32_t *)nullptr, 0u, (size_t)n + 1,
                                rocprim::plus<uint32_t>(), hipStream_t(0));
  return bytes / 4 + 64;
}

void cm_scan_u32(const uint32_t *in, uint32_t *out, uint32_t n, uint32_t *tmp, hipStream_t s) {
  (void)hipMemsetAsync(const_cast<uint32_t *>(in) + n, 0, sizeof(uint32_t), s);
  size_t bytes = 0;
  (void)rocprim::exclusive_scan(nullptr, bytes, in, out, 0u, (size_t)n + 1, rocprim::plus<uint32_t>(), s);
  (void)rocprim::exclusive_scan((void *)tmp, bytes, in, out, 0u, (size_t)n + 1, rocprim::plus<uint32_t>(), s);
}

__global__ __launch_bounds__(CM_BLOCK) void k_hv_flags(CmDev d, uint32_t n_pairs, uint32_t *__restrict__ fr, uint32_t *__restrict__ fp) {
  const uint32_t p = blockIdx.x * CM_BLOCK + threadIdx.x;
  if (p >= n_pairs) return;
  const uint32_t lim = d.hv_mid > d.s3b_cap ? d.hv_mid : d.s3b_cap;
  const uint32_t a = d.hit_tot[2 * p] > lim ? 1u : 0u, b = d.hit_tot[2 * p + 1] > lim ? 1u : 0u;
  fr[2 * p] = a; fr[2 * p + 1] = b;
  fp[p] = a | b;
}
__global__ __launch_bounds__(CM_BLOCK) void k_hv_scatter(const uint32_t *__restrict__ flag, const uint32_t *__restrict__ scan, uint32_t n,
                                                          uint32_t *__restrict__ perm) {
  const uint32_t i = blockIdx.x * CM_BLOCK + threadIdx.x;
  if (i >= n) return;
  const uint32_t heavy_before = scan[i], n_light = n - scan[n];
  perm[flag[i] ? n_light + heavy_before : i - heavy_before] = i;
}
void cm_build_heavy_last(const CmDev &d, uint32_t n_pairs, uint32_t *fr, uint32_t *sr, uint32_t *fp, uint32_t *sp, uint32_t *perm_reads,
                         uint32_t *perm_pairs, uint32_t *scan_tmp, hipStream_t s) {
  if (!n_pairs) return;
  hipLaunchKernelGGL(k_hv_flags, grid_for_n(n_pairs), dim3(CM_BLOCK), 0, s, d, n_pairs, fr, fp);
  cm_scan_u32(fr, sr, 2 * n_pairs, scan_tmp, s);
  cm_scan_u32(fp, sp, n_pairs, scan_tmp, s);
  hipLaunchKernelGGL(k_hv_scatter, grid_for_n(2 * n_pairs), dim3(CM_BLOCK), 0, s, (const uint32_t *)fr, (const uint32_t *)sr, 2 * n_pairs, perm_reads);
  hipLaunchKernelGGL(k_hv_scatter, grid_for_n(n_pairs), dim3(CM_BLOCK), 0, s, (const uint32_t *)fp, (const uint32_t *)sp, n_pairs, perm_pairs);
}

__global__ void k_copy_u64(const unsigned long long *__restrict__ src, unsigned long long *__restrict__ dst) { dst[0] = src[0]; }
__global__ void k_check_cap(const unsigned long long *__restrict__ total, unsigned long long cap, unsigned long long *__restrict__ flag) {
  if (*total > cap) *flag = 1ull;
}
void cm_launch_k_check_cap(const unsigned long long *total, unsigned long long cap, unsigned long long *flag, hipStream_t s) {
  hipLaunchKernelGGL(k_check_cap, dim3(1), dim3(1), 0, s, total, cap, flag);
}
__global__ __launch_bounds__(CM_BLOCK) void k_pack_ref(const uint8_t *__restrict__ ref, uint64_t n_bytes, CmPlRec *__restrict__ pl) {
  const uint64_t w = (uint64_t)blockIdx.x * CM_BLOCK + threadIdx.x;
  if (w * 32 >= n_bytes) return;
  const uint64_t left = n_bytes - w * 32;
  CmPlRec r;
  cm_pack_planes32(ref + w * 32, left < 32 ? (uint32_t)left : 32u, &r.p0, &r.p1, &r.pn, &r.pc);
  pl[w] = r;
}
void cm_launch_k_pack_ref(const uint8_t *ref, uint64_t n_bytes, CmPlRec *pl, hipStream_t s) {
  const uint64_t n = (n_bytes + 31) / 32;
  if (!n) return;
  hipLaunchKernelGGL(k_pack_ref, dim3((unsigned)((n + CM_BLOCK - 1) / CM_BLOCK)), dim3(CM_BLOCK), 0, s, ref, n_bytes, pl);
}
template <int W>
__global__ __launch_bounds__(CM_BLOCK) void k_pack_reads(CmDev d, uint32_t n_reads) {
  const uint32_t r = blockIdx.x * CM_BLOCK + threadIdx.x;
  if (r >= n_reads) return;
  if (W == 0) cm_pack_read_planes_any(d, r); else cm_pack_read_planes_w<(W > 0 ? W : 1)>(d, r);
}
void cm_launch_k_pack_reads(const CmDev &d, uint32_t n_reads, hipStream_t s) {
  if (!n_reads) return;
#define CM_PACK_CASE(W_) case W_: hipLaunchKernelGGL(k_pack_reads<W_>, grid_for_n(n_reads), dim3(CM_BLOCK), 0, s, d, n_reads); break;
  switch (d.read_pl_w) {
    CM_PACK_CASE(1) CM_PACK_CASE(2) CM_PACK_CASE(3) CM_PACK_CASE(4) CM_PACK_CASE(5) CM_PACK_CASE(6) CM_PACK_CASE(7) CM_PACK_CASE(8)
    default: hipLaunchKernelGGL(k_pack_reads<0>, grid_for_n(n_reads), dim3(CM_BLOCK), 0, s, d, n_reads);
  }
#undef CM_PACK_CASE
}
void cm_launch_k_copy_u64(const unsigned long long *src, unsigned long long *dst, hipStream_t s) {
  hipLaunchKernelGGL(k_copy_u64, dim3(1), dim3(1), 0, s, src, dst);
}

__global__ __launch_bounds__(CM_BLOCK) void k_sum_u32(const uint32_t *__restrict__ in, uint32_t n, unsigned long long *__restrict__ out) {
  unsigned long long a = 0;
  for (uint32_t i = blockIdx.x * CM_BLOCK + threadIdx.x; i < n; i += gridDim.x * CM_BLOCK) a += in[i];
  for (int off = 32; off > 0; off >>= 1) a += __shfl_down(a, off, 64);
  __shared__ unsigned long long sa[CM_BLOCK / 64];
  if ((threadIdx.x & 63) == 0) sa[threadIdx.x >> 6] = a;
  __syncthreads();
  if (threadIdx.x == 0) {
    for (int j = 1; j < CM_BLOCK / 64; ++j) a += sa[j];
    if (a) atomicAdd(out, a);
  }
}
void cm_launch_k_sum_u32(const uint32_t *in, uint32_t n, unsigned long long *out, hipStream_t s) {
  if (!n) return;
  uint32_t blocks = (n + CM_BLOCK * 8 - 1) / (CM_BLOCK * 8);
  if (blocks > 2048) blocks = 2048;
  hipLaunchKernelGGL(k_sum_u32, dim3(blocks), dim3(CM_BLOCK), 0, s, in, n, out);
}

static inline dim3 grid_for(uint32_t n) { return dim3((n + CM_BLOCK - 1) / CM_BLOCK); }

#define CM_LAUNCH(kname)                                                               \
  void cm_launch_##kname(const CmDev &d, uint32_t n, hipStream_t s) {                  \
    if (n) hipLaunchKernelGGL(kname, grid_for(n), dim3(CM_BLOCK), 0, s, d, n);         \
  }
void cm_launch_k_s3a_count(const CmDev &d, uint32_t n, hipStream_t s) {
  if (n) hipLaunchKernelGGL(k_s3a_count, grid_for(n), dim3(CM_BLOCK), 0, s, d, n);
}
uint32_t cm_s3b_lane_cap(uint32_t max_read_len) {
  uint32_t cap = max_read_len / 3;
  return cap < 16 ? 16 : (cap > 64 ? 64 : cap);
}
void cm_s3b_heavy_classes(uint32_t *hv_max, uint32_t *hv_big) {
  static std::atomic<int> big_ok[64];
  int dev = 0;
  (void)hipGetDevice(&dev);
  const int slot = dev >= 0 && dev < 64 ? dev : 0;
  int st = big_ok[slot].load(std::memory_order_acquire);
  if (st == 0 || dev != slot) {
    st = hipFuncSetAttribute(reinterpret_cast<const void *>(&k_s3b_heavy<CM_BLOCK>), hipFuncAttributeMaxDynamicSharedMemorySize, 8192 * 10 + (CM_BLOCK + 8) * 4) == hipSuccess ? 1 : 2;
    (void)hipGetLastError();
    if (dev == slot) big_ok[slot].store(st, std::memory_order_release);
  }
  hv_max[0] = 512; hv_max[1] = 1024; hv_max[2] = 2048; hv_max[3] = 4096;
  *hv_big = st == 1 ? 8192 : 0;
}
static inline bool cm_cls_on(const CmDev &d, uint32_t list) { return (d.cls_mask >> list) & 1ull; }
template <class K>
static bool cm_lds_optin(K kernel, size_t bytes) {
  if (bytes <= 64 * 1024) return true;
  if (bytes > 160 * 1024) return false;
  static std::mutex mu;
  static std::map<std::pair<int, const void *>, std::pair<size_t, size_t>> seen;
  int dev = 0;
  (void)hipGetDevice(&dev);
  const std::pair<int, const void *> key(dev, reinterpret_cast<const void *>(kernel));
  std::lock_guard<std::mutex> lk(mu);
  auto it = seen.find(key);
  if (it != seen.end()) {
    if (bytes <= it->second.first) return true;
    if (it->second.second && bytes >= it->second.second) return false;
  }
  const hipError_t e = hipFuncSetAttribute(reinterpret_cast<const void *>(kernel), hipFuncAttributeMaxDynamicSharedMemorySize, (int)bytes);
  (void)hipGetLastError();
  std::pair<size_t, size_t> &v = seen[key];
  if (e == hipSuccess) { if (bytes > v.first) v.first = bytes; } else if (!v.second || bytes < v.second) v.second = bytes;
  return e == hipSuccess;
}
static inline uint32_t cm_coop_mm(const CmDev &d, uint32_t max_read_len) {
  uint32_t MM = max_read_len > (uint32_t)d.p.k ? max_read_len - (uint32_t)d.p.k + 1 : 1;
  return MM > 256 ? 256 : MM;
}
void cm_launch_k_s3b_heavy(const CmDev &d, const uint32_t *n_cls, hipStream_t s, bool coop, uint32_t max_read_len) {
  auto pow2 = [](uint32_t x) { uint32_t p = 2; while (p < x) p <<= 1; return p; };
  auto lst = [&](uint32_t c) { return (const uint32_t *)(d.hv_list + (size_t)c * d.hv_stride); };
  uint32_t rest[CM_HV_LISTS];
  for (int c = 0; c < CM_HV_LISTS; ++c) rest[c] = n_cls[c];
  if (coop && d.hv_max[0]) {
    const uint32_t MM = cm_coop_mm(d, max_read_len);
    const uint32_t RB = d.coop_rb ? d.coop_rb : 3 * MM + 2;
    uint32_t *fb_list = d.hv_list + CM_L_HIT_DECLINED * (size_t)d.hv_stride, *fb_cnt = d.hv_cnt + CM_L_HIT_DECLINED;
// ... 43 lines not shown
        uint32_t *sl = d.hv_list + CM_L_HIT_SERIAL * (size_t)d.hv_stride, *sc = d.hv_cnt + CM_L_HIT_SERIAL;
        hipLaunchKernelGGL((k_s3b_coop<1024, false>), dim3(blocks), dim3(1024), lds, s, d, lst(CM_L_HIT_SLAB), n_cls[CM_L_HIT_SLAB], d.hv_max[3], MM, RB, sl, sc, 1u);
        hipLaunchKernelGGL(k_s3b_serial, dim3(64), dim3(64), 0, s, d, (const uint32_t *)sl, 0u, (const uint32_t *)sc);
        rest[CM_L_HIT_SLAB] = 0;
      }
    }
    if (any_coop) {
      const uint32_t P = pow2(d.hv_big > d.hv_max[3] ? d.hv_big : d.hv_max[3]);
      hipLaunchKernelGGL(k_s3b_heavy<CM_BLOCK>, dim3(512), dim3(CM_BLOCK), (size_t)P * 10 + (CM_BLOCK + 8) * 4, s, d, (const uint32_t *)fb_list, 0u, P, (const uint32_t *)fb_cnt);
    }
  }
  if (rest[CM_L_HIT_WAVE_SMALL]) {
    const uint32_t P = pow2(d.hv_max[0]), gpb = CM_BLOCK / 64;
    hipLaunchKernelGGL(k_s3b_heavy<64>, dim3((rest[CM_L_HIT_WAVE_SMALL] + gpb - 1) / gpb), dim3(CM_BLOCK), (size_t)gpb * P * 10 + gpb * (64 + 8) * 4, s, d, lst(CM_L_HIT_WAVE_SMALL), rest[CM_L_HIT_WAVE_SMALL], P, (const uint32_t *)nullptr);
  }
  if (rest[CM_L_HIT_WAVE]) {
    const uint32_t P = pow2(d.hv_max[0]), gpb = CM_BLOCK / 64;
    hipLaunchKernelGGL(k_s3b_heavy<64>, dim3((rest[CM_L_HIT_WAVE] + gpb - 1) / gpb), dim3(CM_BLOCK), (size_t)gpb * P * 10 + gpb * (64 + 8) * 4, s, d, lst(CM_L_HIT_WAVE), rest[CM_L_HIT_WAVE], P, (const uint32_t *)nullptr);
  }
  const uint32_t blk[3][2] = {{1, 1}, {2, 2}, {10, 3}};
  for (int q = 0; q < 3; ++q) {
    const uint32_t c = blk[q][0];
    if (!rest[c]) continue;
    const uint32_t P = pow2(d.hv_max[blk[q][1]]);
    hipLaunchKernelGGL(k_s3b_heavy<CM_BLOCK>, dim3(rest[c]), dim3(CM_BLOCK), (size_t)P * 10 + (CM_BLOCK + 8) * 4, s, d, lst(c), rest[c], P, (const uint32_t *)nullptr);
  }
  if (rest[CM_L_HIT_B1024]) {
    const uint32_t P = pow2(d.hv_big);
    hipLaunchKernelGGL(k_s3b_heavy<CM_BLOCK>, dim3(rest[CM_L_HIT_B1024]), dim3(CM_BLOCK), (size_t)P * 10 + (CM_BLOCK + 8) * 4, s, d, lst(CM_L_HIT_B1024), rest[CM_L_HIT_B1024], P, (const uint32_t *)nullptr);
  }
  if (rest[CM_L_HIT_SLAB]) hipLaunchKernelGGL(k_s3b_serial, dim3((rest[CM_L_HIT_SLAB] + 63) / 64), dim3(64), 0, s, d, lst(CM_L_HIT_SLAB), rest[CM_L_HIT_SLAB], (const uint32_t *)nullptr);
  if (rest[CM_L_HIT_G16]) {
    const uint32_t P = pow2(d.hv_mid), gpb = CM_BLOCK / 16;
    hipLaunchKernelGGL(k_s3b_heavy<16>, dim3((rest[CM_L_HIT_G16] + gpb - 1) / gpb), dim3(CM_BLOCK), (size_t)gpb * P * 10 + gpb * (16 + 8) * 4, s, d, lst(CM_L_HIT_G16), rest[CM_L_HIT_G16], P, (const uint32_t *)nullptr);
  }
}
void cm_launch_k_s3b_candidates(const CmDev &d, uint32_t n, uint32_t max_read_len, hipStream_t s) {
  if (!n) return;
  const uint32_t cap = d.s3b_cap;
  (void)max_read_len;
  uint32_t threads = 256;
  while (threads > 64 && (size_t)cap * threads * 9 > 36 * 1024 + 1024) threads >>= 1;
  hipLaunchKernelGGL(k_s3b_candidates, dim3((n + threads - 1) / threads), dim3(threads), (size_t)cap * threads * 9, s, d, n, cap);
}
uint32_t cm_rescue_seg_cap(uint32_t n_reads) { return ((n_reads + CM_BLOCK - 1) / CM_BLOCK / CM_RS_SEGS + 1) * CM_BLOCK; }
void cm_launch_k_s4a_rescue_count(const CmDev &d, uint32_t n, hipStream_t s, bool coop) {
  if (n) hipLaunchKernelGGL(k_s4a_rescue_count, grid_for(n), dim3(CM_BLOCK), 0, s, d, n, cm_rescue_seg_cap(n), coop ? 1u : 0u);
}
static inline uint32_t rescue_wave_blocks(uint32_t n_reads) {
  uint32_t b = n_reads / 512 + 64;
  return b > 8192u ? 8192u : b;
}
static inline dim3 rescue_list_grid(uint32_t n_reads) {
  uint32_t b = n_reads / 64 / CM_RS_SEGS / 4 + 1;
  if (b > 256u) b = 256u;
  return dim3(b, CM_RS_SEGS);
}
void cm_launch_k_s4a_rescue_list(const CmDev &d, uint32_t n_reads, hipStream_t s, bool coop) {
  if (!n_reads) return;
  hipLaunchKernelGGL(k_s4a_rescue_list, rescue_list_grid(n_reads), dim3(64), 0, s, d, cm_rescue_seg_cap(n_reads), coop ? 1u : 0u);
  if ((coop) && cm_cls_on(d, CM_L_SEARCH_WAVE)) {
    hipLaunchKernelGGL(k_s4a_rescue_wave<true>, dim3(rescue_wave_blocks(n_reads)), dim3(64), 0, s, d);
    hipLaunchKernelGGL(k_s4a_rescue_wave<false>, dim3(rescue_wave_blocks(n_reads)), dim3(64), 0, s, d);
  }
}
static bool cm_s4b_coop_ready(const CmDev &d, uint32_t RB, size_t *lds) {
  if (!d.hv_max[0]) return false;
  lds[0] = 2 * cm_coop_group_bytes(d.hv_max[0], 1, RB, true);
  lds[1] = cm_coop_group_bytes(d.hv_max[1], 1, RB, true);
  lds[2] = cm_coop_group_bytes(d.hv_max[2], 1, RB, true);
  lds[3] = cm_coop_group_bytes(d.rs_max3, 1, RB, true);
  lds[4] = cm_coop_group_bytes(d.rs_big > d.rs_max3 ? d.rs_big : d.rs_max3, 1, RB, true);
  const bool ok = cm_lds_optin(&k_s4b_coop<64>, lds[0]) && cm_lds_optin(&k_s4b_coop<256>, lds[1] > lds[2] ? lds[1] : lds[2]) && cm_lds_optin(&k_s4b_coop<512>, lds[3]) &&
                  cm_lds_optin(&k_s4b_coop<1024>, lds[4]);
  if (!ok) {
    static std::atomic<int> told{0};
    if (!told.exchange(1)) fprintf(stderr, "chromap_amd: the cooperative rescue kernels do not fit this device's shared memory (%zu / %zu / %zu / %zu bytes); using the one-lane forms\n", lds[0], lds[1], lds[2], lds[4]);
  }
  return ok;
}
static inline uint32_t cm_s4b_rb(const CmDev &d, uint32_t max_read_len) {
  return d.coop_rb ? d.coop_rb : 2 * cm_coop_mm(d, max_read_len) + 2;
}
void cm_launch_k_s4b_rescue_merge(const CmDev &d, uint32_t n, hipStream_t s, bool coop, uint32_t max_read_len) {
  if (!n) return;
  size_t lds[5];
  const bool all = coop && cm_s4b_coop_ready(d, cm_s4b_rb(d, max_read_len), lds);
  hipLaunchKernelGGL(k_s4b_rescue_merge, grid_for(n), dim3(CM_BLOCK), 0, s, d, n, all ? 1u : 0u);
}
void cm_launch_k_s4b_rescue_list(const CmDev &d, uint32_t n_reads, hipStream_t s, bool coop, uint32_t max_read_len) {
  if (!n_reads) return;
  const uint32_t RB = cm_s4b_rb(d, max_read_len);
  size_t lds[5];
  const bool all = coop && cm_s4b_coop_ready(d, RB, lds);
  hipLaunchKernelGGL(k_s4b_rescue_list, rescue_list_grid(n_reads), dim3(64), 0, s, d, cm_rescue_seg_cap(n_reads), all ? 1u : 0u);
  if ((coop) && cm_cls_on(d, CM_L_SEARCH_WAVE)) {
    hipLaunchKernelGGL(k_s4b_rescue_wave<true>, dim3(rescue_wave_blocks(n_reads)), dim3(64), 0, s, d, all ? 1u : 0u);
    hipLaunchKernelGGL(k_s4b_rescue_wave<false>, dim3(rescue_wave_blocks(n_reads)), dim3(64), 0, s, d, all ? 1u : 0u);
  }
  if (!all) return;
  uint32_t blocks = n_reads / 2048 + 64;
  if (blocks > 2048) blocks = 2048;
  auto lst = [&](uint32_t c) { return (const uint32_t *)(d.hv_list + (size_t)c * d.hv_stride); };
  if (cm_cls_on(d, CM_L_RS_WAVE)) hipLaunchKernelGGL(k_s4b_coop<64>, dim3(blocks), dim3(128), lds[0], s, d, lst(CM_L_RS_WAVE), (const uint32_t *)(d.hv_cnt + CM_L_RS_WAVE), d.hv_max[0], RB, 0u);
  if ((d.hv_max[1] > d.hv_max[0]) && cm_cls_on(d, CM_L_RS_B256A)) hipLaunchKernelGGL(k_s4b_coop<256>, dim3(blocks), dim3(256), lds[1], s, d, lst(CM_L_RS_B256A), (const uint32_t *)(d.hv_cnt + CM_L_RS_B256A), d.hv_max[1], RB, 0u);
  if ((d.hv_max[2] > d.hv_max[1]) && cm_cls_on(d, CM_L_RS_B256B)) hipLaunchKernelGGL(k_s4b_coop<256>, dim3(blocks), dim3(256), lds[2], s, d, lst(CM_L_RS_B256B), (const uint32_t *)(d.hv_cnt + CM_L_RS_B256B), d.hv_max[2], RB, 0u);
  if ((d.rs_max3 > d.hv_max[2]) && cm_cls_on(d, CM_L_RS_B512)) hipLaunchKernelGGL(k_s4b_coop<512>, dim3(blocks > 512 ? 512 : blocks), dim3(512), lds[3], s, d, lst(CM_L_RS_B512), (const uint32_t *)(d.hv_cnt + CM_L_RS_B512), d.rs_max3, RB, 0u);
  if ((d.rs_big > d.rs_max3) && cm_cls_on(d, CM_L_RS_B1024)) hipLaunchKernelGGL(k_s4b_coop<1024>, dim3(blocks > 256 ? 256 : blocks), dim3(1024), lds[4], s, d, lst(CM_L_RS_B1024), (const uint32_t *)(d.hv_cnt + CM_L_RS_B1024), d.rs_big, RB, 0u);
  if (d.coop_slab && cm_cls_on(d, CM_L_RS_SLAB))
    hipLaunchKernelGGL(k_s4b_coop<1024>, dim3(d.coop_slab_blocks), dim3(1024), lds[4], s, d, lst(CM_L_RS_SLAB), (const uint32_t *)(d.hv_cnt + CM_L_RS_SLAB), d.rs_big > d.rs_max3 ? d.rs_big : d.rs_max3, RB, 1u);
}
void cm_launch_k_s4c_reduce(const CmDev &d, uint32_t n, hipStream_t s, uint32_t coop) {
  if (!n) return;
  const size_t gw = ((cm_coop_pair_mem_bytes(CM_S4C_P_WAVE) + 15) & ~(size_t)15) + CM_XW_BYTES;
  const size_t gbk = ((cm_coop_pair_mem_bytes(CM_S4C_P_BLOCK) + 15) & ~(size_t)15) + CM_XW_BYTES;
  uint32_t pbig = CM_S4C_P_BIG;
  while (pbig > CM_S4C_P_BLOCK && !cm_lds_optin(&k_s4c_coop<1024, false>, ((cm_coop_pair_mem_bytes(pbig, false) + 15) & ~(size_t)15) + CM_XW_BYTES)) pbig >>= 1;
  if (!cm_lds_optin(&k_s4c_coop<CM_BLOCK, true>, gbk)) coop &= ~4u;
  CmDev d2 = d;
  d2.s4c_pbig = pbig > CM_S4C_P_BLOCK ? pbig : 0;
  hipLaunchKernelGGL(k_s4c_reduce, grid_for(n), dim3(CM_BLOCK), 0, s, d2, n, coop);
  if (!(coop & 4u)) return;
  uint32_t blocks = n / 2048 + 64;
  if (blocks > 4096) blocks = 4096;
  const size_t gs = ((cm_coop_pair_mem_bytes(CM_S4C_P_SMALL) + 15) & ~(size_t)15) + CM_XW_BYTES;
  if (cm_cls_on(d, CM_L_PF_WAVE)) hipLaunchKernelGGL((k_s4c_coop<64, true>), dim3(blocks), dim3(CM_BLOCK), (CM_BLOCK / 64) * gs, s, d, CM_S4C_P_SMALL, CM_L_PF_WAVE, coop);
  if (cm_cls_on(d, CM_L_PF_BLOCK)) hipLaunchKernelGGL((k_s4c_coop<CM_BLOCK, true>), dim3(blocks), dim3(CM_BLOCK), gw, s, d, CM_S4C_P_WAVE, CM_L_PF_BLOCK, coop);
  if (cm_cls_on(d, CM_L_PF_BLOCK_BIG)) hipLaunchKernelGGL((k_s4c_coop<CM_BLOCK, true>), dim3(256), dim3(CM_BLOCK), gbk, s, d, CM_S4C_P_BLOCK, CM_L_PF_BLOCK_BIG, coop);
  if (d2.s4c_pbig && cm_cls_on(d, CM_L_PF_HUGE))
    hipLaunchKernelGGL((k_s4c_coop<1024, false>), dim3(128), dim3(1024), ((cm_coop_pair_mem_bytes(pbig, false) + 15) & ~(size_t)15) + CM_XW_BYTES, s, d, pbig, 19u, coop);
}
void cm_launch_k_s5a_prepare(const CmDev &d, uint32_t n, hipStream_t s, bool coop) {
  if (!n) return;
  hipLaunchKernelGGL(k_s5a_prepare, grid_for(n), dim3(CM_BLOCK), 0, s, d, n, coop ? 1u : 0u);
  if (coop) {
    if (cm_cls_on(d, CM_L_S5_SMALL)) hipLaunchKernelGGL(k_s5_sort_coop, dim3(4096), dim3(CM_BLOCK), 0, s, d, CM_L_S5_SMALL);
    if (cm_cls_on(d, CM_L_S5_WAVE)) hipLaunchKernelGGL(k_s5_sort_coop, dim3(2048), dim3(CM_BLOCK), 0, s, d, CM_L_S5_WAVE);
    if (cm_cls_on(d, CM_L_S5_BLOCK)) hipLaunchKernelGGL(k_s5_sort_coop, dim3(64), dim3(CM_BLOCK), 0, s, d, CM_L_S5_BLOCK);
  }
}
void cm_launch_k_s5c_finalize(const CmDev &d, uint32_t n, hipStream_t s, bool coop) {
  if (!n) return;
  hipLaunchKernelGGL(k_s5c_finalize, grid_for(n), dim3(CM_BLOCK), 0, s, d, n, coop ? 1u : 0u);
  if (!coop) return;
  auto gbytes = [](uint32_t P) {
    const size_t b1 = cm_coop_ver_mem_bytes(P), b2 = cm_coop_sort_mem_bytes(CM_S5C_SORT_P, CM_S5C_SORT_RB);
    return (((b1 > b2 ? b1 : b2) + 15) & ~(size_t)15) + CM_XW_BYTES;
  };
  uint32_t blocks = n / 4096 + 64;
  if (blocks > 2048) blocks = 2048;
  if (cm_cls_on(d, CM_L_S5_SMALL)) hipLaunchKernelGGL(k_s5c_coop<64>, dim3(blocks), dim3(CM_BLOCK), (CM_BLOCK / 64) * gbytes(CM_S5C_P_SMALL), s, d, CM_S5C_P_SMALL, CM_L_S5_SMALL);
  if (cm_cls_on(d, CM_L_S5_WAVE)) hipLaunchKernelGGL(k_s5c_coop<64>, dim3(blocks), dim3(192), 3 * gbytes(CM_S5C_P_WAVE), s, d, CM_S5C_P_WAVE, CM_L_S5_WAVE);
  uint32_t pb = CM_S5C_P_BLOCK;
  while (pb > CM_S5C_P_WAVE && !cm_lds_optin(&k_s5c_coop<CM_BLOCK>, gbytes(pb))) pb >>= 1;
  if (cm_cls_on(d, CM_L_S5_BLOCK)) hipLaunchKernelGGL(k_s5c_coop<CM_BLOCK>, dim3(128), dim3(CM_BLOCK), gbytes(pb), s, d, pb, CM_L_S5_BLOCK);
}
CM_LAUNCH(k_s6a_pair_sam)
CM_LAUNCH(k_s6c_multi_sam)
void cm_launch_k_s5b_verify(const CmDev &d, uint32_t max_items, uint32_t n_reads, hipStream_t s) {
  if (!max_items) return;
  uint32_t blocks = (max_items + CM_BLOCK - 1) / CM_BLOCK;
  if (blocks > 65536) blocks = 65536;
  hipLaunchKernelGGL(k_s5b_verify, dim3(blocks), dim3(CM_BLOCK), 0, s, d, n_reads);
}
static inline size_t cm_s6_group_bytes(uint32_t P) { return ((cm_coop_pe_mem_bytes(P) + 15) & ~(size_t)15) + CM_XW_BYTES; }
void cm_launch_k_s6a_pair(const CmDev &d, uint32_t n, hipStream_t s, bool coop) {
  if (!n) return;
  const size_t lw = (CM_BLOCK / 64) * cm_s6_group_bytes(CM_S6A_P_WAVE), lb = cm_s6_group_bytes(CM_S6A_P_BLOCK);
  if (coop && !(cm_lds_optin(&k_s6a_coop<64>, lw) && cm_lds_optin(&k_s6a_coop<CM_BLOCK>, lb))) coop = false;
  hipLaunchKernelGGL(k_s6a_pair, grid_for(n), dim3(CM_BLOCK), 0, s, d, n, coop ? 1u : 0u);
  if (!coop) return;
  uint32_t blocks = n / 4096 + 64;
  if (blocks > 2048) blocks = 2048;
  if (cm_cls_on(d, CM_L_S6A_SMALL)) hipLaunchKernelGGL(k_s6a_coop<64>, dim3(blocks), dim3(CM_BLOCK), (CM_BLOCK / 64) * cm_s6_group_bytes(CM_S6A_P_SMALL), s, d, CM_S6A_P_SMALL, CM_L_S6A_SMALL);
  if (cm_cls_on(d, CM_L_S6A_WAVE)) hipLaunchKernelGGL(k_s6a_coop<64>, dim3(blocks), dim3(CM_BLOCK), lw, s, d, CM_S6A_P_WAVE, CM_L_S6A_WAVE);
  if (cm_cls_on(d, CM_L_S6A_BLOCK)) hipLaunchKernelGGL(k_s6a_coop<CM_BLOCK>, dim3(256), dim3(CM_BLOCK), lb, s, d, CM_S6A_P_BLOCK, CM_L_S6A_BLOCK);
}
void cm_launch_k_s6c_multi(const CmDev &d, uint32_t n, hipStream_t s, bool coop) {
  if (!n) return;
  const size_t lw = (CM_BLOCK / 64) * cm_s6_group_bytes(CM_S6A_P_WAVE), lb = cm_s6_group_bytes(CM_S6A_P_BLOCK);
  if (coop && !(cm_lds_optin(&k_s6c_coop<64>, lw) && cm_lds_optin(&k_s6c_coop<CM_BLOCK>, lb))) coop = false;
  hipLaunchKernelGGL(k_s6c_multi, grid_for(n), dim3(CM_BLOCK), 0, s, d, n, coop ? 1u : 0u);
  if (!coop) return;
  uint32_t blocks = n / 4096 + 64;
  if (blocks > 2048) blocks = 2048;
  if (cm_cls_on(d, CM_L_S6C_SMALL)) hipLaunchKernelGGL(k_s6c_coop<64>, dim3(blocks), dim3(CM_BLOCK), (CM_BLOCK / 64) * cm_s6_group_bytes(CM_S6A_P_SMALL), s, d, CM_S6A_P_SMALL, CM_L_S6C_SMALL);
  if (cm_cls_on(d, CM_L_S6C_WAVE)) hipLaunchKernelGGL(k_s6c_coop<64>, dim3(blocks), dim3(CM_BLOCK), lw, s, d, CM_S6A_P_WAVE, CM_L_S6C_WAVE);
  if (cm_cls_on(d, CM_L_S6C_BLOCK)) hipLaunchKernelGGL(k_s6c_coop<CM_BLOCK>, dim3(256), dim3(CM_BLOCK), lb, s, d, CM_S6A_P_BLOCK, CM_L_S6C_BLOCK);
}

static inline void staging_geometry(uint32_t max_read_len, uint32_t *threads, uint32_t *lds_half) {
  uint32_t pb = 128;
  while (pb > 16 && (uint64_t)pb * max_read_len + 64 > 24 * 1024) pb >>= 1;
  *threads = 2 * pb;
  *lds_half = (uint32_t)(((uint64_t)pb * max_read_len + 64 + 15) & ~15ull);
}
static bool prep_mm_geometry(const CmDev &d, uint32_t max_read_len, uint32_t *threads, uint32_t *half, uint32_t *stg, size_t *lds, bool *gstage = nullptr, bool *e6_out = nullptr) {
  if (d.p.w != 7 || 2 * d.p.k + 12 > 64) return false;
  *stg = max_read_len / 4 + 4;
  const bool g = max_read_len > 69;
  const bool e6 = !g && 2 * d.p.k + 8 <= 48;
  if (gstage) *gstage = g;
  if (e6_out) *e6_out = e6;
  uint32_t t = 256;
  for (;; t >>= 1) {
    *half = (uint32_t)(((uint64_t)(t / 2) * max_read_len + 64 + 15) & ~15ull);
    *lds = 2 * (size_t)*half + (g ? (size_t)(2 * t + 1) * 4 : (size_t)*stg * t * (e6 ? 6 : 8)) + 64;
    if (*lds <= (g ? 48 : 60) * 1024) break;
    if (t == 64) return false;
  }
  *threads = t;
  return true;
}
static bool prep_flat_geometry(const CmDev &d, uint32_t max_read_len, uint32_t tile_reads, uint32_t *half, uint32_t *nt_max, size_t *lds) {
  if (d.p.w != 7 || !(d.p.k & 1) || d.p.k > 26 || max_read_len > 69 || max_read_len < (uint32_t)d.p.k + 6) return false;
  *half = (uint32_t)(((uint64_t)(CM_BLOCK / 2) * max_read_len + 64 + 15) & ~15ull);
  *nt_max = tile_reads * (max_read_len - (uint32_t)d.p.k + 1);
  const size_t region0 = 2 * (size_t)*half > 16 * (size_t)*nt_max ? 2 * (size_t)*half : 16 * (size_t)*nt_max;
  const size_t nw = *half / 16 + 1;
  *lds = region0 + 2 * (nw + 3) * 4 + 2 * (nw + 1) * 2 + 8 + CM_BLOCK * sizeof(CmFlatRead) + (CM_BLOCK + 2) * 4 + ((size_t)*nt_max + 2) * 2 * 2 + 8 + 32 * 4;
  return *lds <= 64 * 1024;
}
bool cm_prep_flat_supported(const CmDev &d, uint32_t max_read_len, uint32_t tile_reads) {
  uint32_t h, n;
  size_t l;
  return prep_flat_geometry(d, max_read_len, tile_reads, &h, &n, &l);
}
void cm_launch_k_prep_flat(const CmDev &d, uint32_t pair_lo, uint32_t pair_hi, uint32_t max_read_len, uint32_t tile_reads, uint32_t mm_cap,
                           unsigned long long *cursor, hipStream_t s) {
  uint32_t half, nt_max;
  size_t lds;
  if (pair_hi <= pair_lo || !prep_flat_geometry(d, max_read_len, tile_reads, &half, &nt_max, &lds)) return;
  const uint32_t pb = CM_BLOCK / 2;
  hipLaunchKernelGGL(k_prep_flat, dim3((pair_hi - pair_lo + pb - 1) / pb), dim3(CM_BLOCK), lds, s, d, pair_lo, pair_hi, half, nt_max, tile_reads, mm_cap, cursor);
}
bool cm_prep_mm_supported(const CmDev &d, uint32_t max_read_len) {
  uint32_t t, h, g;
  size_t l;
  return prep_mm_geometry(d, max_read_len, &t, &h, &g, &l);
}
uint32_t cm_prep_mm_pairs_per_block(const CmDev &d, uint32_t max_read_len) {
  uint32_t threads, half, stg;
  size_t lds;
  return prep_mm_geometry(d, max_read_len, &threads, &half, &stg, &lds) ? threads / 2 : 0;
}
size_t cm_prep_mm_stage_bytes(const CmDev &d, uint32_t max_read_len, uint32_t pairs) {
  uint32_t threads, half, stg;
  size_t lds;
  bool g = false;
  if (!prep_mm_geometry(d, max_read_len, &threads, &half, &stg, &lds, &g) || !g) return 0;
  const uint32_t pb = threads / 2;
  return (size_t)((pairs + pb - 1) / pb) * stg * threads * 8;
}
void cm_launch_k_prep_mm(const CmDev &d, uint32_t pair_lo, uint32_t pair_hi, uint32_t max_read_len, uint32_t mm_cap,
                         unsigned long long *cursor, hipStream_t s, void *gstage) {
  uint32_t threads, half, stg;
  size_t lds;
  bool g = false, e6 = false;
  if (pair_hi <= pair_lo || !prep_mm_geometry(d, max_read_len, &threads, &half, &stg, &lds, &g, &e6)) return;
  const uint32_t pb = threads / 2;
  if (g) hipLaunchKernelGGL((k_prep_mm<true, false>), dim3((pair_hi - pair_lo + pb - 1) / pb), dim3(threads), lds, s, d, pair_lo, pair_hi, half, stg, mm_cap, cursor, (uint64_t *)gstage);
  else if (e6) hipLaunchKernelGGL((k_prep_mm<false, true>), dim3((pair_hi - pair_lo + pb - 1) / pb), dim3(threads), lds, s, d, pair_lo, pair_hi, half, stg, mm_cap, cursor, (uint64_t *)nullptr);
  else hipLaunchKernelGGL((k_prep_mm<false, false>), dim3((pair_hi - pair_lo + pb - 1) / pb), dim3(threads), lds, s, d, pair_lo, pair_hi, half, stg, mm_cap, cursor, (uint64_t *)nullptr);
}
static inline int probe_variant_norm(int variant) {
  if (variant == 0) variant = CM_PROBE_U;
  const int u = variant & 15;
  return ((u == 2 || u == 4 || u == 8) ? u : 1) | (variant & 16);
}
uint32_t cm_probe_range_blocks(uint64_t max_entries, int variant) {
  const uint64_t per = (uint64_t)(probe_variant_norm(variant) & 15) * CM_BLOCK;
  return (uint32_t)((max_entries + per - 1) / per);
}
void cm_launch_k_probe_range(const CmDev &d, const unsigned long long *range, uint64_t max_entries, uint32_t cap, void *partials, hipStream_t s, int variant) {
  const uint32_t blocks = cm_probe_range_blocks(max_entries, variant);
  if (!blocks) return;
  variant = probe_variant_norm(variant);
  const int u = variant & 15;
  const bool pair = (variant & 16) != 0;
#define CM_PROBE_CASE(U_, P_) hipLaunchKernelGGL((k_probe_range<U_, P_>), dim3(blocks), dim3(CM_BLOCK), 0, s, d.bkt, d.bmask, d.mm_hash, d.pr_val, d.pr_kind, range, cap, (uint2 *)partials)
  if (u == 1) { if (pair) CM_PROBE_CASE(1, true); else CM_PROBE_CASE(1, false); }
  else if (u == 2) { if (pair) CM_PROBE_CASE(2, true); else CM_PROBE_CASE(2, false); }
  else if (u == 8) { if (pair) CM_PROBE_CASE(8, true); else CM_PROBE_CASE(8, false); }
  else { if (pair) CM_PROBE_CASE(4, true); else CM_PROBE_CASE(4, false); }
#undef CM_PROBE_CASE
}
void cm_launch_k_probe_reduce(const void *partials, uint32_t blocks, unsigned long long *counters, hipStream_t s) {
  if (blocks) hipLaunchKernelGGL(k_probe_reduce, dim3(blocks / (CM_BLOCK * 8) + 1), dim3(CM_BLOCK), 0, s, (const uint2 *)partials, blocks, counters);
}
void cm_launch_k_prep_count(const CmDev &d, uint32_t n_pairs, uint32_t max_read_len, hipStream_t s) {
  if (!n_pairs) return;
  uint32_t threads, half;
  staging_geometry(max_read_len, &threads, &half);
  const uint32_t pb = threads / 2;
  hipLaunchKernelGGL(k_prep_count, dim3((n_pairs + pb - 1) / pb), dim3(threads), 2 * half, s, d, n_pairs, half);
}
void cm_launch_k_mm_fill(const CmDev &d, uint32_t pair_lo, uint32_t pair_hi, uint32_t max_read_len, hipStream_t s) {
  if (pair_hi <= pair_lo) return;
  uint32_t threads, half;
  staging_geometry(max_read_len, &threads, &half);
  const uint32_t pb = threads / 2;
  hipLaunchKernelGGL(k_mm_fill, dim3((pair_hi - pair_lo + pb - 1) / pb), dim3(threads), 2 * half, s, d, pair_lo, pair_hi, half);
}
struct CmChunkLo { uint32_t lo[CM_MM_CHUNKS + 1]; };
__global__ void k_mm_marks(const uint32_t *__restrict__ mm_off, CmChunkLo cl, uint32_t n_marks, unsigned long long *__restrict__ marks) {
  if (threadIdx.x < n_marks) marks[threadIdx.x] = mm_off[2 * (size_t)cl.lo[threadIdx.x]];
}
void cm_launch_k_mm_marks(const uint32_t *mm_off, const uint32_t *lo, uint32_t n_marks, unsigned long long *marks, hipStream_t s) {
  CmChunkLo cl;
  for (uint32_t i = 0; i < n_marks && i <= CM_MM_CHUNKS; ++i) cl.lo[i] = lo[i];
  hipLaunchKernelGGL(k_mm_marks, dim3(1), dim3(64), 0, s, mm_off, cl, n_marks, marks);
}
void cm_launch_k_s0b_barcode(const CmDev &d, uint32_t n, hipStream_t s) {
  if (n) hipLaunchKernelGGL(k_s0b_barcode, grid_for(n), dim3(CM_BLOCK), 0, s, d, n);
}
void cm_launch_k_bc_abundance(const uint8_t *bcb, const uint32_t *bco, uint32_t lo, uint32_t hi, uint64_t *wl, uint32_t wl_mask,
                              unsigned long long *num_sample, hipStream_t s) {
  if (hi > lo) hipLaunchKernelGGL(k_bc_abundance, grid_for(hi - lo), dim3(CM_BLOCK), 0, s, bcb, bco, lo, hi, wl, wl_mask, num_sample);
}
void cm_launch_k_s6b_sample(const CmDev &d, uint32_t n_chunks, hipStream_t s) {
  if (n_chunks) hipLaunchKernelGGL(k_s6b_sample, dim3(n_chunks), dim3(64), 0, s, d, n_chunks);
}
size_t cm_stats_partial_words(uint32_t n) { return (size_t)((n + CM_BLOCK - 1) / CM_BLOCK) * CM_NSTAT + CM_NSTAT; }
void cm_launch_k_stats(const CmDev &d, uint32_t n, unsigned long long *partials, hipStream_t s) {
  if (!n) return;
  uint32_t blocks = (n + CM_BLOCK - 1) / CM_BLOCK;
  if (blocks > CM_STATS_BLOCKS) blocks = CM_STATS_BLOCKS;
  hipLaunchKernelGGL(k_stats, dim3(blocks), dim3(CM_BLOCK), 0, s, d, n, partials);
  hipLaunchKernelGGL(k_stats_reduce, dim3(1), dim3(CM_BLOCK), 0, s, (const unsigned long long *)partials, blocks, d.stats);
}
size_t cm_probe_partial_words(uint32_t n) { return (size_t)((n + CM_BLOCK - 1) / CM_BLOCK) + 1; }
void cm_launch_k_probe(const uint64_t *bkt, uint32_t bmask, const uint64_t *hash, uint64_t *val, uint8_t *kind,
                       uint32_t n, void *partials, unsigned long long *counters, hipStream_t s, int variant) {
  if (!n) return;
  variant = probe_variant_norm(variant);
  const int u = variant & 15;
  const bool pair = (variant & 16) != 0;
  const uint32_t blocks = (n + u * CM_BLOCK - 1) / (u * CM_BLOCK);
#define CM_PROBE_CASE(U_, P_) hipLaunchKernelGGL((k_probe<U_, P_>), dim3(blocks), dim3(CM_BLOCK), 0, s, bkt, bmask, hash, val, kind, n, (uint2 *)partials)
  if (u == 1) { if (pair) CM_PROBE_CASE(1, true); else CM_PROBE_CASE(1, false); }
  else if (u == 2) { if (pair) CM_PROBE_CASE(2, true); else CM_PROBE_CASE(2, false); }
  else if (u == 8) { if (pair) CM_PROBE_CASE(8, true); else CM_PROBE_CASE(8, false); }
  else { if (pair) CM_PROBE_CASE(4, true); else CM_PROBE_CASE(4, false); }
#undef CM_PROBE_CASE
  if (partials && counters)
    hipLaunchKernelGGL(k_probe_reduce, dim3(blocks / (CM_BLOCK * 8) + 1), dim3(CM_BLOCK), 0, s, (const uint2 *)partials, blocks, counters);
// ... 2 lines not shown
```

chromap_amd/csrc/cm_stages.h:

```cpp
#ifndef CM_STAGES_H_
#define CM_STAGES_H_

#include "cm_types.h"

CM_HD uint32_t cm_c2u(uint8_t c) {
  const uint32_t u = c & 0xDFu;
  const uint32_t x = (u >> 1) & 3u;
  const uint32_t o = u - 0x41u;
  const bool acgt = o < 20u && ((0x80045u >> (o & 31u)) & 1u);
  return acgt ? x ^ (x >> 1) : 4u;
}
CM_HD uint8_t cm_negchar(uint8_t c) {
  const uint32_t v = 3u ^ cm_c2u(c);
  return v == 0 ? 'A' : v == 1 ? 'C' : v == 2 ? 'G' : v == 3 ? 'T' : 'N';
}

CM_HD uint64_t cm_hash64(uint64_t key, uint64_t mask) {
  key = (~key + (key << 21)) & mask;
  key = key ^ key >> 24;
  key = ((key + (key << 3)) + (key << 8)) & mask;
  key = key ^ key >> 14;
  key = ((key + (key << 2)) + (key << 4)) & mask;
  key = key ^ key >> 28;
  key = (key + (key << 31)) & mask;
// ... 1141 lines not shown
      if (!have) break;
      es = ws; ee = we; have = false; emit = true;
    }
    int32_t l = prev_l, m = 0, rr = (int32_t)(nocc - 1);
    while (l <= rr) {
      m = (l + rr) / 2;
      const uint64_t cp = o[m] >> 1;
      ++reads;
      if (cp < es) l = m + 1;
      else if (cp > es) rr = m - 1;
      else break;
    }
    prev_l = m;
    for (uint32_t oi = (uint32_t)m; oi < nocc; ++oi) {
      const uint64_t rh = o[oi];
      ++reads;
      if ((rh >> 1) > ee) break;
      const uint64_t cp = cm_cand_from_hit(rh, ps, d.p.k, &same);
      if ((same && strand == 0) || (!same && strand == 1)) { if (out) out[cnt] = cp; ++cnt; }
    }
    if (!have && ci >= mn) break;
  }
  if (reads_out) *reads_out += reads;
  return cnt;
}
CM_HD void cm_rescue_rep(const CmDev &d, uint8_t kind, uint64_t val, uint32_t ps, uint32_t *rep_len, uint32_t *prev_rep) {
  if (kind == CM_PR_MISS || kind == CM_PR_SINGLE) return;
  const uint32_t nocc = (uint32_t)val;
  if (nocc >= (uint32_t)d.p.f0) {
    const uint32_t rp = ps >> 1;
    if (*prev_rep > rp) *rep_len += (uint32_t)d.p.k;
    else if (rp < *prev_rep + (uint32_t)d.p.k + (uint32_t)d.p.w - 1) *rep_len += rp - *prev_rep;
    else *rep_len += (uint32_t)d.p.k;
    *prev_rep = rp;
  }
}
CM_HD int cm_rescue(const CmDev &d, uint32_t r, int strand, const uint64_t *mp, const uint8_t *mc, uint32_t mn,
                    uint64_t *out, uint32_t *n_out, uint32_t *rep_len_out, unsigned long long *occ_reads) {
  int max_count = 0, best_num = 0;
  for (uint32_t i = 0; i < mn; ++i) {
    const int c = mc[i];
    if (c > max_count) { max_count = c; best_num = 1; }
    else if (c == max_count) ++best_num;
  }
  *n_out = 0;
  if (cm_rescue_bails(d, max_count, best_num, mn)) return -max_count;
  const uint32_t b = d.mm_off[r], n = d.mm_cnt[r];
  uint32_t cnt = 0, rep_len = 0, prev_rep = ~0u;
  unsigned long long reads = 0;
  for (uint32_t mi0 = 0; mi0 < n; mi0 += CM_S3B_GROUP) {
    uint8_t kind_g[CM_S3B_GROUP];
    uint64_t val_g[CM_S3B_GROUP];
    uint32_t ps_g[CM_S3B_GROUP];
#pragma unroll
    for (int q = 0; q < CM_S3B_GROUP; ++q) {
      const bool in = mi0 + q < n;
      kind_g[q] = in ? d.pr_kind[b + mi0 + q] : (uint8_t)CM_PR_MISS;
      val_g[q] = in ? d.pr_val[b + mi0 + q] : 0;
      ps_g[q] = in ? d.mm_ps[b + mi0 + q] : 0;
    }
#pragma unroll
    for (int q = 0; q < CM_S3B_GROUP; ++q) {
      cnt += cm_rescue_minimizer(d, strand, mp, mc, mn, max_count, kind_g[q], val_g[q], ps_g[q], out ? out + cnt : nullptr, &reads);
      cm_rescue_rep(d, kind_g[q], val_g[q], ps_g[q], &rep_len, &prev_rep);
    }
  }
  *n_out = cnt;
  *rep_len_out = rep_len;
  if (occ_reads) *occ_reads += reads;
  return max_count;
}

CM_HD const uint64_t *cm_c0_pos(const CmDev &d, uint32_t r) { return d.hbuf + d.hit_off[r]; }
CM_HD const uint8_t *cm_c0_pcnt(const CmDev &d, uint32_t r) { return d.hcnt + d.hit_off[r]; }
CM_HD const uint64_t *cm_c0_neg(const CmDev &d, uint32_t r) { return d.hbuf + d.hit_off[r] + d.n_pos_hit[r]; }
CM_HD const uint8_t *cm_c0_ncnt(const CmDev &d, uint32_t r) { return d.hcnt + d.hit_off[r] + d.n_pos_hit[r]; }

CM_HD bool cm_s4a_decide(const CmDev &d, uint32_t r) {
  const uint32_t pair = r >> 1;
  d.aug[r] = 0; d.res_neg[r] = 0; d.res_pos[r] = 0; d.resc_n[r] = 0; d.resc_p[r] = 0;
  const bool live = d.p.single ? ((r & 1) == 0 && d.mm_cnt[r] > 0) : (d.mm_cnt[2 * pair] > 0 && d.mm_cnt[2 * pair + 1] > 0);
  const uint32_t ncp = d.ncp[r], ncn = d.ncn[r];
  d.m_tot[r] = live ? ncp + ncn : 0;
  if (!live) return false;
  const uint32_t mm_count = d.mm_cnt[r];
  bool augment = !d.p.split && !d.p.single;
  const uint8_t *pc = cm_c0_pcnt(d, r), *nc = cm_c0_ncnt(d, r);
  for (uint32_t i = 0; augment && i < ncp; ++i) if (pc[i] >= mm_count / 2) { augment = false; break; }
  if (augment) for (uint32_t i = 0; i < ncn; ++i) if (nc[i] >= mm_count / 2) { augment = false; break; }
  return augment;
}
CM_HD void cm_s4a_rescue(const CmDev &d, uint32_t r) {
  const uint32_t o = r ^ 1u;
  d.aug[r] = 1;
  uint32_t cntn = 0, cntp = 0, rl = 0;
  int res_neg = 0, res_pos = 0;
  bool set_rl = false;
  uint32_t rl_val = 0;
  unsigned long long occ_reads = 0;
  if (d.ncp[o] > 0) {
    res_neg = cm_rescue(d, r, 1, cm_c0_pos(d, o), cm_c0_pcnt(d, o), d.ncp[o], nullptr, &cntn, &rl, &occ_reads);
    if (res_neg >= 0) { set_rl = true; rl_val = rl; }
  }
  if (d.ncn[o] > 0) {
    res_pos = cm_rescue(d, r, 0, cm_c0_neg(d, o), cm_c0_ncnt(d, o), d.ncn[o], nullptr, &cntp, &rl, &occ_reads);
    if (res_pos >= 0) { set_rl = true; rl_val = rl; }
  }
  d.res_neg[r] = res_neg; d.res_pos[r] = res_pos;
  d.resc_n[r] = cntn; d.resc_p[r] = cntp;
  if (set_rl) d.rep_len[r] = rl_val;
  d.m_tot[r] = d.ncp[r] + d.ncn[r] + cntn + cntp;
}
CM_HD void cm_s4a_rescue_count(const CmDev &d, uint32_t r) {
  if (cm_s4a_decide(d, r)) cm_s4a_rescue(d, r);
}

CM_HD uint32_t cm_merge(const uint64_t *p1, const uint8_t *c1, uint32_t n1, uint64_t *out, uint8_t *outc,
                        uint32_t n2, int e) {
  const uint64_t *p2 = out + n1;
  const uint8_t *c2 = outc + n1;
  if (n1 == 0) return n2;
  uint32_t i = 0, j = 0, k = 0;
#define CM_BACK_OK(P) (k == 0 || (P) > out[k - 1] + (uint64_t)(int64_t)e)
  while (i < n1 && j < n2) {
    const uint64_t a = p1[i], b = p2[j];
    if (a == b) {
      if (CM_BACK_OK(a)) {
        const uint8_t ca = c1[i], cb = c2[j];
        if (ca > cb) { out[k] = a; outc[k] = ca; } else { out[k] = b; outc[k] = cb; }
        ++k;
      }
      ++i; ++j;
    } else if (a < b) {
      if (CM_BACK_OK(a)) { const uint8_t ca = c1[i]; out[k] = a; outc[k] = ca; ++k; }
      ++i;
    } else {
      if (CM_BACK_OK(b)) { const uint8_t cb = c2[j]; out[k] = b; outc[k] = cb; ++k; }
      ++j;
    }
  }
  while (i < n1) { const uint64_t a = p1[i]; if (CM_BACK_OK(a)) { const uint8_t ca = c1[i]; out[k] = a; outc[k] = ca; ++k; } ++i; }
  while (j < n2) { const uint64_t b = p2[j]; if (CM_BACK_OK(b)) { const uint8_t cb = c2[j]; out[k] = b; outc[k] = cb; ++k; } ++j; }
#undef CM_BACK_OK
  return k;
}

#define CM_S4B_ALL 0
#define CM_S4B_PREFILLED 1
#define CM_S4B_FILL_ONLY 2
CM_HD void cm_s4b_rescue_merge(const CmDev &d, uint32_t r, int mode = CM_S4B_ALL) {
  const bool prefilled = mode == CM_S4B_PREFILLED;
  const uint32_t o = r ^ 1u;
  d.mcp[r] = 0; d.mcn[r] = 0;
  if (d.m_tot[r] == 0) return;
  const uint32_t ncp = d.ncp[r], ncn = d.ncn[r], rp = d.resc_p[r], rn = d.resc_n[r];
  uint64_t *P = d.mbuf + d.m_off[r];
  uint8_t *PC = d.mcnt + d.m_off[r];
  uint64_t *N = P + ncp + rp;
  uint8_t *NC = PC + ncp + rp;
  const uint64_t *p0 = cm_c0_pos(d, r), *n0 = cm_c0_neg(d, r);
  const uint8_t *pc0 = cm_c0_pcnt(d, r), *nc0 = cm_c0_ncnt(d, r);
  uint32_t naug_p = 0, naug_n = 0;
  if (d.aug[r]) {
    uint32_t cnt = 0, rl = 0;
    if (d.ncp[o] > 0 && d.res_neg[r] >= 0 && rn > 0) {
      if (prefilled) cnt = rn; else cm_rescue(d, r, 1, cm_c0_pos(d, o), cm_c0_pcnt(d, o), d.ncp[o], N + ncn, &cnt, &rl, nullptr);
      if (mode != CM_S4B_FILL_ONLY) {
        cm_sort_u64(N + ncn, cnt);
        naug_n = cm_sweep(N + ncn, NC + ncn, cnt, d.p.e, 1, d.mm_cnt[r]);
      }
    }
    if (d.ncn[o] > 0 && d.res_pos[r] >= 0 && rp > 0) {
      if (prefilled) cnt = rp; else cm_rescue(d, r, 0, cm_c0_neg(d, o), cm_c0_ncnt(d, o), d.ncn[o], P + ncp, &cnt, &rl, nullptr);
      if (mode != CM_S4B_FILL_ONLY) {
        cm_sort_u64(P + ncp, cnt);
        naug_p = cm_sweep(P + ncp, PC + ncp, cnt, d.p.e, 1, d.mm_cnt[r]);
      }
    }
  }
  if (mode == CM_S4B_FILL_ONLY) return;
  if (naug_p > 0) {
    d.mcp[r] = cm_merge(p0, pc0, ncp, P, PC, naug_p, d.p.e);
  } else {
    for (uint32_t i = 0; i < ncp; ++i) { P[i] = p0[i]; PC[i] = pc0[i]; }
    d.mcp[r] = ncp;
  }
  if (naug_n > 0) {
    d.mcn[r] = cm_merge(n0, nc0, ncn, N, NC, naug_n, d.p.e);
  } else {
    for (uint32_t i = 0; i < ncn; ++i) { N[i] = n0[i]; NC[i] = nc0[i]; }
    d.mcn[r] = ncn;
  }
}

CM_HD uint64_t *cm_m_pos(const CmDev &d, uint32_t r) { return d.mbuf + d.m_off[r]; }
CM_HD uint8_t *cm_m_pcnt(const CmDev &d, uint32_t r) { return d.mcnt + d.m_off[r]; }
CM_HD uint64_t *cm_m_neg(const CmDev &d, uint32_t r) { return d.mbuf + d.m_off[r] + d.ncp[r] + d.resc_p[r]; }
CM_HD uint8_t *cm_m_ncnt(const CmDev &d, uint32_t r) { return d.mcnt + d.m_off[r] + d.ncp[r] + d.resc_p[r]; }
CM_HD uint64_t *cm_f_pos(const CmDev &d, uint32_t r) { return d.fbuf + d.m_off[r]; }
CM_HD uint8_t *cm_f_pcnt(const CmDev &d, uint32_t r) { return d.fcnt + d.m_off[r]; }
CM_HD uint64_t *cm_f_neg(const CmDev &d, uint32_t r) { return d.fbuf + d.m_off[r] + d.ncp[r] + d.resc_p[r]; }
CM_HD uint8_t *cm_f_ncnt(const CmDev &d, uint32_t r) { return d.fcnt + d.m_off[r] + d.ncp[r] + d.resc_p[r]; }

CM_HD void cm_reduce_dir(uint32_t dist, const uint64_t *p1, const uint8_t *c1, uint32_t n1, const uint64_t *p2,
                         const uint8_t *c2, uint32_t n2, uint64_t *f1, uint8_t *fc1, uint32_t *nf1, uint64_t *f2,
                         uint8_t *fc2, uint32_t *nf2) {
  uint32_t i1 = 0, i2 = 0, o1 = 0, o2 = 0;
  int unpaired1 = 0, unpaired2 = 0;
  int max1 = 6, max2 = 6;
  uint32_t prev_end_i2 = 0;
  while (i1 < n1 && i2 < n2) {
    const uint64_t a = p1[i1], b = p2[i2];
    if (a > b + dist) {
      if (i2 >= prev_end_i2 && unpaired2 < 5 && (a >> 32) == (b >> 32) && (int)c2[i2] >= max2) {
        f2[o2] = b; fc2[o2] = c2[i2]; ++o2;
        ++unpaired2;
      }
      ++i2;
    } else if (b > a + dist) {
      if (unpaired1 < 5 && (a >> 32) == (b >> 32) && (int)c1[i1] >= max1) {
        f1[o1] = a; fc1[o1] = c1[i1]; ++o1;
        ++unpaired1;
      }
      ++i1;
    } else {
      f1[o1] = a; fc1[o1] = c1[i1]; ++o1;
      if ((int)c1[i1] > max1) max1 = c1[i1];
      uint32_t cur = i2;
      while (cur < n2 && p2[cur] <= a + dist) {
        if (cur >= prev_end_i2) {
          f2[o2] = p2[cur]; fc2[o2] = c2[cur]; ++o2;
          if ((int)c2[cur] > max2) max2 = c2[cur];
        }
        ++cur;
      }
      prev_end_i2 = cur;
      ++i1;
    }
  }
  *nf1 = o1;
  *nf2 = o2;
}

CM_HD void cm_rerank(const CmDev &d, uint32_t r) {
  if (!d.rid_rank) return;
  uint64_t *fp = cm_f_pos(d, r), *fn = cm_f_neg(d, r);
  for (uint32_t i = 0; i < d.fcp[r]; ++i) fp[i] = (fp[i] & 0xffffffffull) | ((uint64_t)d.rid_rank[(uint32_t)(fp[i] >> 32)] << 32);
  for (uint32_t i = 0; i < d.fcn[r]; ++i) fn[i] = (fn[i] & 0xffffffffull) | ((uint64_t)d.rid_rank[(uint32_t)(fn[i] >> 32)] << 32);
}

CM_HD bool cm_s4c_pre(const CmDev &d, uint32_t pair) {
  const uint32_t r1 = 2 * pair, r2 = r1 + 1;
  d.fcp[r1] = d.fcn[r1] = d.fcp[r2] = d.fcn[r2] = 0;
  d.alive[pair] = 0;
  d.force0[pair] = 0;
  if (d.p.single) {
    if (d.mm_cnt[r1] == 0 || d.mcp[r1] + d.mcn[r1] == 0) return false;
    const uint64_t *mp = cm_m_pos(d, r1), *mn = cm_m_neg(d, r1);
    const uint8_t *mpc = cm_m_pcnt(d, r1), *mnc = cm_m_ncnt(d, r1);
    uint64_t *fp = cm_f_pos(d, r1), *fn = cm_f_neg(d, r1);
    uint8_t *fpc = cm_f_pcnt(d, r1), *fnc = cm_f_ncnt(d, r1);
    for (uint32_t i = 0; i < d.mcp[r1]; ++i) { fp[i] = mp[i]; fpc[i] = mpc[i]; }
    for (uint32_t i = 0; i < d.mcn[r1]; ++i) { fn[i] = mn[i]; fnc[i] = mnc[i]; }
    d.fcp[r1] = d.mcp[r1]; d.fcn[r1] = d.mcn[r1];
    d.alive[pair] = 1;
    cm_rerank(d, r1);
    return false;
  }
  if (!(d.mm_cnt[r1] > 0 && d.mm_cnt[r2] > 0)) return false;
  int ret = 0;
  for (uint32_t r = r1; r <= r2; ++r) {
    if (!d.aug[r]) continue;
    const int pr = d.res_neg[r], nr = d.res_pos[r];
    if (((pr < 0 && nr > 0 && -pr >= nr) || (pr > 0 && nr < 0 && pr <= -nr)) && d.ncp[r] + d.ncn[r] == 0) ret = 1;
  }
  d.force0[pair] = (uint8_t)ret;
  const uint32_t nc1 = d.mcp[r1] + d.mcn[r1], nc2 = d.mcp[r2] + d.mcn[r2];
  if (!(nc1 > 0 && nc2 > 0)) return false;
  if (d.p.split) {
    for (uint32_t r = r1; r <= r2; ++r) {
      const uint64_t *mp = cm_m_pos(d, r), *mn = cm_m_neg(d, r);
      const uint8_t *mpc = cm_m_pcnt(d, r), *mnc = cm_m_ncnt(d, r);
      uint64_t *fp = cm_f_pos(d, r), *fn = cm_f_neg(d, r);
      uint8_t *fpc = cm_f_pcnt(d, r), *fnc = cm_f_ncnt(d, r);
      for (uint32_t i = 0; i < d.mcp[r]; ++i) { fp[i] = mp[i]; fpc[i] = mpc[i]; }
      for (uint32_t i = 0; i < d.mcn[r]; ++i) { fn[i] = mn[i]; fnc[i] = mnc[i]; }
      d.fcp[r] = d.mcp[r]; d.fcn[r] = d.mcn[r];
    }
    d.alive[pair] = 1;
    cm_rerank(d, r1); cm_rerank(d, r2);
    return false;
  }
  return true;
}
CM_HD void cm_s4c_filter(const CmDev &d, uint32_t pair) {
  const uint32_t r1 = 2 * pair, r2 = r1 + 1;
  uint32_t a, b;
  cm_reduce_dir((uint32_t)d.p.max_insert, cm_m_pos(d, r1), cm_m_pcnt(d, r1), d.mcp[r1], cm_m_neg(d, r2),
                cm_m_ncnt(d, r2), d.mcn[r2], cm_f_pos(d, r1), cm_f_pcnt(d, r1), &a, cm_f_neg(d, r2), cm_f_ncnt(d, r2), &b);
  d.fcp[r1] = a; d.fcn[r2] = b;
  cm_reduce_dir((uint32_t)d.p.max_insert, cm_m_neg(d, r1), cm_m_ncnt(d, r1), d.mcn[r1], cm_m_pos(d, r2),
                cm_m_pcnt(d, r2), d.mcp[r2], cm_f_neg(d, r1), cm_f_ncnt(d, r1), &a, cm_f_pos(d, r2), cm_f_pcnt(d, r2), &b);
  d.fcn[r1] = a; d.fcp[r2] = b;
}
CM_HD void cm_s4c_post(const CmDev &d, uint32_t pair) {
  const uint32_t r1 = 2 * pair, r2 = r1 + 1;
  const uint32_t f1 = d.fcp[r1] + d.fcn[r1], f2 = d.fcp[r2] + d.fcn[r2];
  d.alive[pair] = (f1 > 0 && f2 > 0) ? 1 : 0;
  if (d.alive[pair]) { cm_rerank(d, r1); cm_rerank(d, r2); }
}
CM_HD void cm_s4c_reduce(const CmDev &d, uint32_t pair) {
  if (!cm_s4c_pre(d, pair)) return;
  cm_s4c_filter(d, pair);
  cm_s4c_post(d, pair);
}

CM_HD uint32_t cm_text_code(const uint8_t *read, int L, int i, bool neg) {
  if (!neg) return cm_c2u(read[i]);
  const uint32_t c = cm_c2u(read[L - 1 - i]);
  return c < 4 ? 3u ^ c : 4u;
}
CM_HD uint8_t cm_text_char(const uint8_t *read, int L, int i, bool neg) {
  return neg ? cm_negchar(read[L - 1 - i]) : read[i];
}

CM_HD uint32_t cm_peq_get(const uint32_t *P, uint32_t c) {
  return c == 0 ? P[0] : c == 1 ? P[1] : c == 2 ? P[2] : c == 3 ? P[3] : P[4];
}
CM_HD void cm_peq_or(uint32_t *P, uint32_t c, uint32_t bit) {
  P[0] |= c == 0 ? bit : 0u; P[1] |= c == 1 ? bit : 0u; P[2] |= c == 2 ? bit : 0u;
  P[3] |= c == 3 ? bit : 0u; P[4] |= c == 4 ? bit : 0u;
}

struct CmFwdReader {
  const uint64_t *ap;
  uint64_t cur, nxt;
  uint32_t left, words;
  CM_HD void init(const uint8_t *p, uint32_t n) {
    const uintptr_t a = reinterpret_cast<uintptr_t>(p);
    const uint32_t sh = (uint32_t)(a & 7);
    ap = reinterpret_cast<const uint64_t *>(a & ~(uintptr_t)7);
    words = n ? (sh + n + 7) >> 3 : 0;
    cur = 0; nxt = 0; left = 0;
    if (words) { cur = *ap++ >> (sh * 8); left = 8 - sh; --words; }
    if (words) { nxt = *ap++; --words; }
  }
  CM_HD uint8_t next() {
    if (left == 0) {
      cur = nxt; left = 8;
      if (words) { nxt = *ap++; --words; }
    }
    const uint8_t b = (uint8_t)cur;
    cur >>= 8; --left;
    return b;
  }
};
struct CmBwdReader {
  const uint64_t *ap;
  uint64_t cur, nxt;
  uint32_t left, words;
  CM_HD void init(const uint8_t *p, uint32_t n) {
    const uintptr_t a = reinterpret_cast<uintptr_t>(p);
    const uint32_t pos = (uint32_t)(a & 7);
    ap = reinterpret_cast<const uint64_t *>(a & ~(uintptr_t)7);
    words = n ? ((7 - pos) + n + 7) >> 3 : 0;
    cur = 0; nxt = 0; left = 0;
    if (words) { cur = *ap-- << ((7 - pos) * 8); left = pos + 1; --words; }
    if (words) { nxt = *ap--; --words; }
  }
  CM_HD uint8_t next() {
    if (left == 0) {
      cur = nxt; left = 8;
      if (words) { nxt = *ap--; --words; }
    }
    const uint8_t b = (uint8_t)(cur >> 56);
    cur <<= 8; --left;
    return b;
  }
};

template <bool NEG>
CM_HD int cm_banded_align_stream(int e, const uint8_t *pattern, const uint8_t *read, int Lfull, int toff, int L, int *end_pos) {
  CmFwdReader pr;
  pr.init(pattern, (uint32_t)(L + 2 * e));
  CmFwdReader tf;
// ... 1571 lines not shown
```

chromap_amd/csrc/cm_types.h:

```cpp
#ifndef CM_TYPES_H_
#define CM_TYPES_H_

#include <stdint.h>

#if defined(__HIPCC__)
#include <hip/hip_runtime.h>
#define CM_HD __host__ __device__ __forceinline__
#define CM_D __device__ __forceinline__
#else
#define CM_HD inline
#define CM_D inline
#endif

#define CM_EMPTY_KEY 0xFFFFFFFFFFFFFFFFull
#define CM_DELETED_KEY 0xFFFFFFFFFFFFFFFEull

#define CM_PR_MISS 0
#define CM_PR_SINGLE 1
#define CM_PR_MULTI 2
#define CM_V_INVALID 0x7fff
#define CM_MM_CHUNKS 8
enum CmList : uint32_t {
  CM_L_HIT_WAVE = 0, CM_L_HIT_B256A = 1, CM_L_HIT_B256B = 2, CM_L_HIT_SLAB = 3, CM_L_HIT_G16 = 4, CM_L_HIT_DECLINED = 5, CM_L_RS_WAVE = 6, CM_L_RS_B256A = 7,
  CM_L_RS_B256B = 8, CM_L_PF_BLOCK = 9, CM_L_HIT_B512 = 10, CM_L_RS_B512 = 11, CM_L_S5_WAVE = 12, CM_L_S6A_WAVE = 13, CM_L_PF_BLOCK_BIG = 14, CM_L_RS_SLAB = 15,
  CM_L_HIT_SERIAL = 16, CM_L_S6C_WAVE = 17, CM_L_S6A_BLOCK = 18, CM_L_PF_HUGE = 19, CM_L_S6C_BLOCK = 20, CM_L_HIT_WAVE_SMALL = 21, CM_L_S5_BLOCK = 22,
  CM_L_SEARCH_WAVE = 23, CM_L_HIT_B1024 = 25, CM_L_RS_B1024 = 26, CM_L_PF_WAVE = 27, CM_L_S5_SMALL = 28, CM_L_S6A_SMALL = 29, CM_L_S6C_SMALL = 30,
  CM_L_SEARCH_WAVE_BIG = 31
};
#define CM_HV_LISTS 32
#define CM_RS_SEGS 64
#define CM_MAX_BEST 8192
#define CM_SORT_SERIAL_MAX 24
#define CM_SORT_WAVE_MAX 1024

#define CM_SAM_CIGAR_CAP 64
#define CM_GOFF_GAP 2048u
#define CM_MAX_READ_LEN 1400
struct CmParams {
  int32_t e;
  int32_t min_seeds;
  int32_t f0, f1;
  int32_t max_insert;
  int32_t min_read_len;
  int32_t max_best;
  int32_t drop_rep;
  int32_t trim;
  int32_t split;
  int32_t single;
  int32_t bc_err;
  int32_t bc_keep;
  double bc_prob;
  int32_t k, w;
  int32_t lanes;
  int32_t ref_batch;
  int32_t grain;
  int32_t pairs_out;
  int32_t sam;
};

struct CmMapqTables {
  const double *len_coef;
  const uint32_t *nsec_break;
  int32_t n_break;
};

struct alignas(16) CmPlRec { uint32_t p0, p1, pn, pc; };
#define CM_PL_LEAD 4

struct CmDev {
  const uint64_t *bkt;
  uint32_t bmask;
  const uint64_t *occ;
  uint32_t n_occ;
  const uint8_t *ref;
  const uint64_t *ref_off;
  const uint32_t *ref_len;
  uint32_t n_seq;
  const uint32_t *goff;
  const CmPlRec *ref_pl;
  uint64_t ref_pl_words;
  uint32_t *read_pl;
  uint32_t read_pl_w;
  CmParams p;
  CmMapqTables mq;
  uint32_t n_pairs;
  uint32_t first_read_id;
  const uint8_t *rb0, *rb1;
  const uint32_t *ro0, *ro1;
  const uint8_t *bcb, *bcq;
  const uint32_t *bco;
  const uint64_t *wl;
  uint32_t wl_mask;
  double wl_num_sample;
  const double *pow10_tab;
  uint64_t *bc_key;
  uint8_t *bc_ok;
  uint32_t *rlen;
  uint32_t *mm_cnt;
  uint32_t *mm_off;
  uint64_t *mm_hash;
  uint32_t *mm_ps;
  uint64_t *pr_val;
  uint8_t *pr_kind;
  uint32_t *hit_tot;
  uint32_t *hit_off;
  uint8_t *round2;
  uint32_t *rep_cnt;
  uint32_t *rep_len;
  uint64_t *hbuf;
// ... 85 lines not shown
```

Measured before the change: 547.5.

## Fold chunk marks into prep kernels, drop rescue merge copy, compact multimapper list

The one-thread copy kernel that recorded each chunk's minimizer cursor is removed. Instead, the last block of each prep kernel writes the mark through an atomic completion counter. The s4b rescue-merge pass is removed: reads without rescue now read candidates directly from the hit buffer through a view helper, and s4a writes mcp/mcn. The s6c multimapper kernel now runs only over a compacted list of pairs with more than one best hit, built during s6a, instead of scanning every pair. These cuts remove launches and copy traffic, at the cost of extra atomics, a reused list slot, and more complex pointer selection.

```diff
diff --git a/chromap_amd/csrc/cm_api.hip b/chromap_amd/csrc/cm_api.hip
--- a/chromap_amd/csrc/cm_api.hip
+++ b/chromap_amd/csrc/cm_api.hip
@@ -876,18 +876,17 @@
     mm_probe_grids(c, k);
     if (c->mm_hash.ensure((size_t)cap * 8 + 8) || c->mm_ps.ensure((size_t)cap * 4 + 4) || c->pr_val.ensure((size_t)cap * 8 + 8) ||
         (!flat && c->mm_stage.ensure(cm_prep_mm_stage_bytes(d, c->max_read_len, chunk_pairs) + 8)) ||
-        c->pr_kind.ensure((size_t)cap + 4) || c->mm_cursor.ensure(8) || c->mm_marks.ensure((CM_MM_CHUNKS + 1) * 8) ||
+        c->pr_kind.ensure((size_t)cap + 4) || c->mm_cursor.ensure(16) || c->mm_marks.ensure((CM_MM_CHUNKS + 1) * 8) ||
         c->partials.ensure(((size_t)k.part_off[k.n_chunks] + 1) * 8 + cm_stats_partial_words(n) * 8)) {
       cm_set_error(c, "out of device memory (minimizers)"); return CMGPU_ENOMEM;
     }
     r.bind();
-    HIPCHECK(c, hipMemsetAsync(c->mm_cursor.p, 0, 8, s));
+    HIPCHECK(c, hipMemsetAsync(c->mm_cursor.p, 0, 16, s));
     HIPCHECK(c, hipMemsetAsync(c->mm_marks.p, 0, 8, s));
     unsigned long long *cursor = (unsigned long long *)c->mm_cursor.p, *marks = (unsigned long long *)c->mm_marks.p;
     rc = mm_fill_and_probe(r, k, (uint32_t)cap, [&](uint32_t ch) {
-      if (flat) cm_launch_k_prep_flat(d, k.lo[ch], k.lo[ch + 1], c->max_read_len, (uint32_t)c->opt.prep_tile_reads, (uint32_t)cap, cursor, s);
-      else cm_launch_k_prep_mm(d, k.lo[ch], k.lo[ch + 1], c->max_read_len, (uint32_t)cap, cursor, s, c->mm_stage.p);
-      cm_launch_k_copy_u64(cursor, marks + ch + 1, s);
+      if (flat) cm_launch_k_prep_flat(d, k.lo[ch], k.lo[ch + 1], c->max_read_len, (uint32_t)c->opt.prep_tile_reads, (uint32_t)cap, cursor, marks + ch + 1, s);
+      else cm_launch_k_prep_mm(d, k.lo[ch], k.lo[ch + 1], c->max_read_len, (uint32_t)cap, cursor, marks + ch + 1, s, c->mm_stage.p);
     });
     if (rc) return rc;
     d.mm_cap = (uint32_t)cap;
@@ -1031,7 +1030,6 @@
   if (cm_debug_pool()) fprintf(stderr, "spec %d m_cap %llu m_total %llu\n", (int)r.spec, (unsigned long long)c->m_cap, m_total);
   r.bind();
   mark(c, "s4a_rescue_count");
-  cm_launch_k_s4b_rescue_merge(d, n2, s, coop, c->max_read_len);
   cm_launch_k_s4b_rescue_list(d, n2, s, coop, c->max_read_len);
   mark(c, "s4b_rescue_merge");
   HIPCHECK(c, hipMemsetAsync(c->srt_cnt.p, 0, 8, s));
@@ -1090,7 +1088,7 @@
   const bool aborted = r.spec && hst[CM_ST_ABORT];
   if (!aborted) {
     unsigned long long seen = 0, keep = 0;
-    for (uint32_t l = 6; l < CM_HV_LISTS; ++l) if (h_cls[l]) seen |= 1ull << (l == 31 ? 23 : l);
+    for (uint32_t l = 6; l < CM_HV_LISTS; ++l) if (h_cls[l] && l != CM_L_S6C_MULTI) seen |= 1ull << (l == 31 ? 23 : l);
     if (seen & ~r.d.cls_mask) return CM_RC_AGAIN_ALL_CLASSES;
     for (uint32_t l = 0; l < 64; ++l) {
       if ((seen >> l) & 1ull) c->cls_age[l] = 32; else if (c->cls_age[l]) --c->cls_age[l];
diff --git a/chromap_amd/csrc/cm_coop.h b/chromap_amd/csrc/cm_coop.h
--- a/chromap_amd/csrc/cm_coop.h
+++ b/chromap_amd/csrc/cm_coop.h
@@ -1275,10 +1275,11 @@
     return;
   }
   uint32_t a, b, c, e2;
-  cm_coop_reduce_dir<STAGED>(g, m, (uint32_t)d.p.max_insert, d.mbuf + mo1, d.mcnt + mo1, mcp1, d.mbuf + mo2 + sh2, d.mcnt + mo2 + sh2, mcn2,
+  const CmMView v1 = cm_m_view(d, r1), v2 = cm_m_view(d, r2);
+  cm_coop_reduce_dir<STAGED>(g, m, (uint32_t)d.p.max_insert, v1.pos, v1.pcnt, mcp1, v2.neg, v2.ncnt, mcn2,
                      d.fbuf + mo1, d.fcnt + mo1, &a, d.fbuf + mo2 + sh2, d.fcnt + mo2 + sh2, &b);
   g.sync();
-  cm_coop_reduce_dir<STAGED>(g, m, (uint32_t)d.p.max_insert, d.mbuf + mo1 + sh1, d.mcnt + mo1 + sh1, mcn1, d.mbuf + mo2, d.mcnt + mo2, mcp2,
+  cm_coop_reduce_dir<STAGED>(g, m, (uint32_t)d.p.max_insert, v1.neg, v1.ncnt, mcn1, v2.pos, v2.pcnt, mcp2,
                      d.fbuf + mo1 + sh1, d.fcnt + mo1 + sh1, &c, d.fbuf + mo2, d.fcnt + mo2, &e2);
   g.sync();
   const bool alive = a + c > 0 && b + e2 > 0;
diff --git a/chromap_amd/csrc/cm_kernels.h b/chromap_amd/csrc/cm_kernels.h
--- a/chromap_amd/csrc/cm_kernels.h
+++ b/chromap_amd/csrc/cm_kernels.h
@@ -13,11 +13,11 @@
 bool cm_prep_mm_supported(const CmDev &d, uint32_t max_read_len);
 bool cm_prep_flat_supported(const CmDev &d, uint32_t max_read_len, uint32_t tile_reads);
 void cm_launch_k_prep_flat(const CmDev &d, uint32_t pair_lo, uint32_t pair_hi, uint32_t max_read_len, uint32_t tile_reads, uint32_t mm_cap,
-                           unsigned long long *cursor, hipStream_t s);
+                           unsigned long long *cursor, unsigned long long *mark, hipStream_t s);
 uint32_t cm_prep_mm_pairs_per_block(const CmDev &d, uint32_t max_read_len);
 size_t cm_prep_mm_stage_bytes(const CmDev &d, uint32_t max_read_len, uint32_t pairs);
 void cm_launch_k_prep_mm(const CmDev &d, uint32_t pair_lo, uint32_t pair_hi, uint32_t max_read_len, uint32_t mm_cap,
-                         unsigned long long *cursor, hipStream_t s, void *gstage);
+                         unsigned long long *cursor, unsigned long long *mark, hipStream_t s, void *gstage);
 uint32_t cm_probe_range_blocks(uint64_t max_entries, int variant);
 void cm_launch_k_probe_range(const CmDev &d, const unsigned long long *range, uint64_t max_entries, uint32_t cap, void *partials, hipStream_t s, int variant);
 void cm_launch_k_probe_reduce(const void *partials, uint32_t blocks, unsigned long long *counters, hipStream_t s);
@@ -28,7 +28,6 @@
 void cm_launch_k_s3b_heavy(const CmDev &d, const uint32_t *n_cls, hipStream_t s, bool coop, uint32_t max_read_len);
 void cm_launch_k_s3b_candidates(const CmDev &d, uint32_t n, uint32_t max_read_len, hipStream_t s);
 void cm_launch_k_s4a_rescue_count(const CmDev &d, uint32_t n, hipStream_t s, bool coop);
-void cm_launch_k_s4b_rescue_merge(const CmDev &d, uint32_t n, hipStream_t s, bool coop, uint32_t max_read_len);
 uint32_t cm_rescue_seg_cap(uint32_t n_reads);
 void cm_launch_k_s4a_rescue_list(const CmDev &d, uint32_t n_reads, hipStream_t s, bool coop);
 void cm_launch_k_s4b_rescue_list(const CmDev &d, uint32_t n_reads, hipStream_t s, bool coop, uint32_t max_read_len);
@@ -55,7 +54,6 @@
 void cm_launch_k_pack_ref(const uint8_t *ref, uint64_t n_bytes, CmPlRec *pl, hipStream_t s);
 void cm_launch_k_pack_reads(const CmDev &d, uint32_t n_reads, hipStream_t s);
 void cm_launch_k_check_cap(const unsigned long long *total, unsigned long long cap, unsigned long long *flag, hipStream_t s);
-void cm_launch_k_copy_u64(const unsigned long long *src, unsigned long long *dst, hipStream_t s);
 void cm_launch_k_sum_u32(const uint32_t *in, uint32_t n, unsigned long long *out, hipStream_t s);
 size_t cm_scan_tmp_words(uint32_t n);
 void cm_scan_u32(const uint32_t *in, uint32_t *out, uint32_t n, uint32_t *tmp, hipStream_t s);
diff --git a/chromap_amd/csrc/cm_kernels.hip b/chromap_amd/csrc/cm_kernels.hip
--- a/chromap_amd/csrc/cm_kernels.hip
+++ b/chromap_amd/csrc/cm_kernels.hip
@@ -63,9 +63,17 @@
   if (pair < p1) cm_s1_fill(d, 2 * pair + (t < PB ? 0 : 1), t < PB ? s.m0 : s.m1);
 }
 
+__device__ __forceinline__ void cm_chunk_mark(unsigned long long *cursor, unsigned long long *mark) {
+  __threadfence();
+  if (atomicAdd(cursor + 1, 1ull) == (unsigned long long)gridDim.x - 1ull) {
+    __threadfence();
+    *mark = atomicAdd(cursor, 0ull);
+    cursor[1] = 0;
+  }
+}
 template <bool GSTAGE, bool E6>
 __global__ void k_prep_mm(CmDev d, uint32_t pair_lo, uint32_t n_pairs , uint32_t lds_half, uint32_t stg,
-                          uint32_t mm_cap, unsigned long long *cursor, uint64_t *gstage) {
+                          uint32_t mm_cap, unsigned long long *cursor, unsigned long long *mark, uint64_t *gstage) {
   const uint32_t T = blockDim.x, PB = T >> 1;
   const uint32_t p0 = pair_lo + blockIdx.x * PB, p1 = p0 + PB < n_pairs ? p0 + PB : n_pairs;
   const uint32_t t = threadIdx.x, lp = t < PB ? t : t - PB, pair = p0 + lp;
@@ -107,6 +115,7 @@
     sh_w[8] = (uint32_t)base;
     sh_w[9] = (uint32_t)(base >> 32);
     sh_w[10] = tot;
+    cm_chunk_mark(cursor, mark);
   }
   __syncthreads();
   const unsigned long long base = (unsigned long long)sh_w[8] | ((unsigned long long)sh_w[9] << 32);
@@ -155,7 +164,7 @@
 
 __global__ __launch_bounds__(CM_BLOCK) void k_prep_flat(CmDev d, uint32_t pair_lo, uint32_t n_pairs ,
                                                         uint32_t lds_half, uint32_t nt_max, uint32_t tile_reads, uint32_t mm_cap,
-                                                        unsigned long long *cursor) {
+                                                        unsigned long long *cursor, unsigned long long *mark) {
   constexpr uint32_t T = CM_BLOCK, PB = T / 2;
   const uint32_t p0 = pair_lo + blockIdx.x * PB, p1 = p0 + PB < n_pairs ? p0 + PB : n_pairs;
   const uint32_t t = threadIdx.x, lp = t < PB ? t : t - PB, pair = p0 + lp, mate = t < PB ? 0u : 1u;
@@ -313,6 +322,8 @@
     d.mm_off[r] = (uint32_t)off;
     if (c && off + c <= mm_cap) cm_minimizers_window<7>(seq, len, k, d.mm_hash + off, d.mm_ps + off, c);
   }
+  __syncthreads();
+  if (t == 0) cm_chunk_mark(cursor, mark);
 }
 
 __global__ __launch_bounds__(CM_BLOCK) void k_s3a_count(CmDev d, uint32_t n) {
@@ -768,17 +779,6 @@
   }
   if (d.prof && threadIdx.x == 0) { const unsigned long long dt = (unsigned long long)(clock64() - t2); atomicAdd(&d.prof[31], dt); atomicMax(&d.prof[15], dt); }
 }
-#define CM_S4B_COPY_MIN 64u
-__global__ __launch_bounds__(CM_BLOCK) void k_s4b_rescue_merge(CmDev d, uint32_t n, uint32_t coop) {
-  if (d.abort && *d.abort) return;
-  const uint32_t i0 = blockIdx.x * CM_BLOCK + threadIdx.x;
-  const uint32_t i = i0 < n ? (d.perm_reads ? d.perm_reads[i0] : i0) : 0u;
-  const bool mine = i0 < n && !(d.aug[i] && d.resc_n[i] + d.resc_p[i] > 0);
-  const bool to_wave = mine && coop && d.m_tot[i] > CM_S4B_COPY_MIN;
-  if (mine && !to_wave) cm_s4b_rescue_merge(d, i);
-  if (to_wave) { d.mcp[i] = 0; d.mcn[i] = 0; }
-  if (coop) cm_wave_append(d.hv_list + (size_t)CM_L_RS_WAVE * d.hv_stride, d.hv_cnt + CM_L_RS_WAVE, to_wave, i);
-}
 __device__ __forceinline__ void cm_group_rescue_fill(const CmDev &d, uint32_t r, int strand, const uint64_t *mp, const uint8_t *mc, uint32_t mn,
                                                      uint32_t t, uint32_t *lds_cnt, uint64_t *out) {
   int max_count, best_num;
@@ -1151,6 +1151,7 @@
     cm_wave_append(d.hv_list + (size_t)CM_L_S6A_WAVE * d.hv_stride, d.hv_cnt + CM_L_S6A_WAVE, cls == CM_L_S6A_WAVE, pair);
     cm_wave_append(d.hv_list + (size_t)CM_L_S6A_BLOCK * d.hv_stride, d.hv_cnt + CM_L_S6A_BLOCK, cls == CM_L_S6A_BLOCK, pair);
   }
+  cm_wave_append(d.hv_list + (size_t)CM_L_S6C_MULTI * d.hv_stride, d.hv_cnt + CM_L_S6C_MULTI, i < n && d.pe_nbest[pair] > 1, pair);
 }
 template <int G>
 __global__ __launch_bounds__(CM_BLOCK, 6) void k_s6a_coop(CmDev d, uint32_t P, uint32_t lid) {
@@ -1164,21 +1165,30 @@
   CmDevGroup<G> g;
   g.t = threadIdx.x % G;
   g.xw = reinterpret_cast<uint32_t *>(base + gb - CM_XW_BYTES);
-  for (uint32_t j = blockIdx.x * gpb + grp; j < n_list; j += gridDim.x * gpb) cm_coop_s6a<false>(d, list[j], g, m);
-}
-__global__ __launch_bounds__(CM_BLOCK) void k_s6c_multi(CmDev d, uint32_t n, uint32_t coop) {
+  for (uint32_t j = blockIdx.x * gpb + grp; j < n_list; j += gridDim.x * gpb) {
+    const uint32_t pair = list[j];
+    cm_coop_s6a<false>(d, pair, g, m);
+    if (g.t == 0 && d.pe_nbest[pair] > 1)
+      d.hv_list[(size_t)CM_L_S6C_MULTI * d.hv_stride + atomicAdd(d.hv_cnt + CM_L_S6C_MULTI, 1u)] = pair;
+  }
+}
+__global__ __launch_bounds__(CM_BLOCK) void k_s6c_multi(CmDev d, uint32_t coop) {
   if (d.abort && *d.abort) return;
-  const uint32_t i = blockIdx.x * CM_BLOCK + threadIdx.x;
-  const uint32_t pair = i < n ? (d.perm_pairs ? d.perm_pairs[i] : i) : 0u;
-  uint32_t cls = 0;
-  if (i < n) {
-    if (coop && !d.p.single && !d.p.split && d.pe_nbest[pair] > 1) cls = cm_s6_class(d, pair, CM_L_S6C_SMALL, CM_L_S6C_WAVE, CM_L_S6C_BLOCK);
-    if (!cls) cm_s6c_multi<false>(d, pair);
-  }
-  if (coop) {
-    cm_wave_append(d.hv_list + (size_t)CM_L_S6C_SMALL * d.hv_stride, d.hv_cnt + CM_L_S6C_SMALL, cls == CM_L_S6C_SMALL, pair);
-    cm_wave_append(d.hv_list + (size_t)CM_L_S6C_WAVE * d.hv_stride, d.hv_cnt + CM_L_S6C_WAVE, cls == CM_L_S6C_WAVE, pair);
-    cm_wave_append(d.hv_list + (size_t)CM_L_S6C_BLOCK * d.hv_stride, d.hv_cnt + CM_L_S6C_BLOCK, cls == CM_L_S6C_BLOCK, pair);
+  const uint32_t n_list = d.hv_cnt[CM_L_S6C_MULTI];
+  const uint32_t *list = d.hv_list + (size_t)CM_L_S6C_MULTI * d.hv_stride;
+  for (uint32_t j0 = blockIdx.x * CM_BLOCK; j0 < n_list; j0 += gridDim.x * CM_BLOCK) {
+    const uint32_t j = j0 + threadIdx.x;
+    const uint32_t pair = j < n_list ? list[j] : 0u;
+    uint32_t cls = 0;
+    if (j < n_list) {
+      if (coop && !d.p.single && !d.p.split) cls = cm_s6_class(d, pair, CM_L_S6C_SMALL, CM_L_S6C_WAVE, CM_L_S6C_BLOCK);
+      if (!cls) cm_s6c_multi<false>(d, pair);
+    }
+    if (coop) {
+      cm_wave_append(d.hv_list + (size_t)CM_L_S6C_SMALL * d.hv_stride, d.hv_cnt + CM_L_S6C_SMALL, cls == CM_L_S6C_SMALL, pair);
+      cm_wave_append(d.hv_list + (size_t)CM_L_S6C_WAVE * d.hv_stride, d.hv_cnt + CM_L_S6C_WAVE, cls == CM_L_S6C_WAVE, pair);
+      cm_wave_append(d.hv_list + (size_t)CM_L_S6C_BLOCK * d.hv_stride, d.hv_cnt + CM_L_S6C_BLOCK, cls == CM_L_S6C_BLOCK, pair);
+    }
   }
 }
 template <int G>
@@ -1495,7 +1505,6 @@
   hipLaunchKernelGGL(k_hv_scatter, grid_for_n(n_pairs), dim3(CM_BLOCK), 0, s, (const uint32_t *)fp, (const uint32_t *)sp, n_pairs, perm_pairs);
 }
 
-__global__ void k_copy_u64(const unsigned long long *__restrict__ src, unsigned long long *__restrict__ dst) { dst[0] = src[0]; }
 __global__ void k_check_cap(const unsigned long long *__restrict__ total, unsigned long long cap, unsigned long long *__restrict__ flag) {
   if (*total > cap) *flag = 1ull;
 }
@@ -1529,9 +1538,6 @@
     default: hipLaunchKernelGGL(k_pack_reads<0>, grid_for_n(n_reads), dim3(CM_BLOCK), 0, s, d, n_reads);
   }
 #undef CM_PACK_CASE
-}
-void cm_launch_k_copy_u64(const unsigned long long *src, unsigned long long *dst, hipStream_t s) {
-  hipLaunchKernelGGL(k_copy_u64, dim3(1), dim3(1), 0, s, src, dst);
 }
 
 __global__ __launch_bounds__(CM_BLOCK) void k_sum_u32(const uint32_t *__restrict__ in, uint32_t n, unsigned long long *__restrict__ out) {
@@ -1741,12 +1747,6 @@
 static inline uint32_t cm_s4b_rb(const CmDev &d, uint32_t max_read_len) {
   return d.coop_rb ? d.coop_rb : 2 * cm_coop_mm(d, max_read_len) + 2;
 }
-void cm_launch_k_s4b_rescue_merge(const CmDev &d, uint32_t n, hipStream_t s, bool coop, uint32_t max_read_len) {
-  if (!n) return;
-  size_t lds[5];
-  const bool all = coop && cm_s4b_coop_ready(d, cm_s4b_rb(d, max_read_len), lds);
-  hipLaunchKernelGGL(k_s4b_rescue_merge, grid_for(n), dim3(CM_BLOCK), 0, s, d, n, all ? 1u : 0u);
-}
 void cm_launch_k_s4b_rescue_list(const CmDev &d, uint32_t n_reads, hipStream_t s, bool coop, uint32_t max_read_len) {
   if (!n_reads) return;
   const uint32_t RB = cm_s4b_rb(d, max_read_len);
@@ -1839,10 +1839,10 @@
   if (!n) return;
   const size_t lw = (CM_BLOCK / 64) * cm_s6_group_bytes(CM_S6A_P_WAVE), lb = cm_s6_group_bytes(CM_S6A_P_BLOCK);
   if (coop && !(cm_lds_optin(&k_s6c_coop<64>, lw) && cm_lds_optin(&k_s6c_coop<CM_BLOCK>, lb))) coop = false;
-  hipLaunchKernelGGL(k_s6c_multi, grid_for(n), dim3(CM_BLOCK), 0, s, d, n, coop ? 1u : 0u);
-  if (!coop) return;
   uint32_t blocks = n / 4096 + 64;
   if (blocks > 2048) blocks = 2048;
+  hipLaunchKernelGGL(k_s6c_multi, dim3(blocks), dim3(CM_BLOCK), 0, s, d, coop ? 1u : 0u);
+  if (!coop) return;
   if (cm_cls_on(d, CM_L_S6C_SMALL)) hipLaunchKernelGGL(k_s6c_coop<64>, dim3(blocks), dim3(CM_BLOCK), (CM_BLOCK / 64) * cm_s6_group_bytes(CM_S6A_P_SMALL), s, d, CM_S6A_P_SMALL, CM_L_S6C_SMALL);
   if (cm_cls_on(d, CM_L_S6C_WAVE)) hipLaunchKernelGGL(k_s6c_coop<64>, dim3(blocks), dim3(CM_BLOCK), lw, s, d, CM_S6A_P_WAVE, CM_L_S6C_WAVE);
   if (cm_cls_on(d, CM_L_S6C_BLOCK)) hipLaunchKernelGGL(k_s6c_coop<CM_BLOCK>, dim3(256), dim3(CM_BLOCK), lb, s, d, CM_S6A_P_BLOCK, CM_L_S6C_BLOCK);
@@ -1886,12 +1886,15 @@
   return prep_flat_geometry(d, max_read_len, tile_reads, &h, &n, &l);
 }
 void cm_launch_k_prep_flat(const CmDev &d, uint32_t pair_lo, uint32_t pair_hi, uint32_t max_read_len, uint32_t tile_reads, uint32_t mm_cap,
-                           unsigned long long *cursor, hipStream_t s) {
+                           unsigned long long *cursor, unsigned long long *mark, hipStream_t s) {
   uint32_t half, nt_max;
   size_t lds;
-  if (pair_hi <= pair_lo || !prep_flat_geometry(d, max_read_len, tile_reads, &half, &nt_max, &lds)) return;
+  if (pair_hi <= pair_lo || !prep_flat_geometry(d, max_read_len, tile_reads, &half, &nt_max, &lds)) {
+    (void)hipMemcpyAsync(mark, cursor, 8, hipMemcpyDeviceToDevice, s);
+    return;
+  }
   const uint32_t pb = CM_BLOCK / 2;
-  hipLaunchKernelGGL(k_prep_flat, dim3((pair_hi - pair_lo + pb - 1) / pb), dim3(CM_BLOCK), lds, s, d, pair_lo, pair_hi, half, nt_max, tile_reads, mm_cap, cursor);
+  hipLaunchKernelGGL(k_prep_flat, dim3((pair_hi - pair_lo + pb - 1) / pb), dim3(CM_BLOCK), lds, s, d, pair_lo, pair_hi, half, nt_max, tile_reads, mm_cap, cursor, mark);
 }
 bool cm_prep_mm_supported(const CmDev &d, uint32_t max_read_len) {
   uint32_t t, h, g;
@@ -1912,15 +1915,18 @@
   return (size_t)((pairs + pb - 1) / pb) * stg * threads * 8;
 }
 void cm_launch_k_prep_mm(const CmDev &d, uint32_t pair_lo, uint32_t pair_hi, uint32_t max_read_len, uint32_t mm_cap,
-                         unsigned long long *cursor, hipStream_t s, void *gstage) {
+                         unsigned long long *cursor, unsigned long long *mark, hipStream_t s, void *gstage) {
   uint32_t threads, half, stg;
   size_t lds;
   bool g = false, e6 = false;
-  if (pair_hi <= pair_lo || !prep_mm_geometry(d, max_read_len, &threads, &half, &stg, &lds, &g, &e6)) return;
+  if (pair_hi <= pair_lo || !prep_mm_geometry(d, max_read_len, &threads, &half, &stg, &lds, &g, &e6)) {
+    (void)hipMemcpyAsync(mark, cursor, 8, hipMemcpyDeviceToDevice, s);
+    return;
+  }
   const uint32_t pb = threads / 2;
-  if (g) hipLaunchKernelGGL((k_prep_mm<true, false>), dim3((pair_hi - pair_lo + pb - 1) / pb), dim3(threads), lds, s, d, pair_lo, pair_hi, half, stg, mm_cap, cursor, (uint64_t *)gstage);
-  else if (e6) hipLaunchKernelGGL((k_prep_mm<false, true>), dim3((pair_hi - pair_lo + pb - 1) / pb), dim3(threads), lds, s, d, pair_lo, pair_hi, half, stg, mm_cap, cursor, (uint64_t *)nullptr);
-  else hipLaunchKernelGGL((k_prep_mm<false, false>), dim3((pair_hi - pair_lo + pb - 1) / pb), dim3(threads), lds, s, d, pair_lo, pair_hi, half, stg, mm_cap, cursor, (uint64_t *)nullptr);
+  if (g) hipLaunchKernelGGL((k_prep_mm<true, false>), dim3((pair_hi - pair_lo + pb - 1) / pb), dim3(threads), lds, s, d, pair_lo, pair_hi, half, stg, mm_cap, cursor, mark, (uint64_t *)gstage);
+  else if (e6) hipLaunchKernelGGL((k_prep_mm<false, true>), dim3((pair_hi - pair_lo + pb - 1) / pb), dim3(threads), lds, s, d, pair_lo, pair_hi, half, stg, mm_cap, cursor, mark, (uint64_t *)nullptr);
+  else hipLaunchKernelGGL((k_prep_mm<false, false>), dim3((pair_hi - pair_lo + pb - 1) / pb), dim3(threads), lds, s, d, pair_lo, pair_hi, half, stg, mm_cap, cursor, mark, (uint64_t *)nullptr);
 }
 static inline int probe_variant_norm(int variant) {
   if (variant == 0) variant = CM_PROBE_U;
diff --git a/chromap_amd/csrc/cm_stages.h b/chromap_amd/csrc/cm_stages.h
--- a/chromap_amd/csrc/cm_stages.h
+++ b/chromap_amd/csrc/cm_stages.h
@@ -1247,6 +1247,7 @@
   const bool live = d.p.single ? ((r & 1) == 0 && d.mm_cnt[r] > 0) : (d.mm_cnt[2 * pair] > 0 && d.mm_cnt[2 * pair + 1] > 0);
   const uint32_t ncp = d.ncp[r], ncn = d.ncn[r];
   d.m_tot[r] = live ? ncp + ncn : 0;
+  d.mcp[r] = live ? ncp : 0; d.mcn[r] = live ? ncn : 0;
   if (!live) return false;
   const uint32_t mm_count = d.mm_cnt[r];
   bool augment = !d.p.split && !d.p.single;
@@ -1276,6 +1277,7 @@
   if (set_rl) d.rep_len[r] = rl_val;
   d.m_tot[r] = d.ncp[r] + d.ncn[r] + cntn + cntp;
 }
+CM_HD bool cm_read_merged(const CmDev &d, uint32_t r) { return d.aug[r] && d.resc_n[r] + d.resc_p[r] > 0; }
 CM_HD void cm_s4a_rescue_count(const CmDev &d, uint32_t r) {
   if (cm_s4a_decide(d, r)) cm_s4a_rescue(d, r);
 }
@@ -1358,10 +1360,22 @@
   }
 }
 
-CM_HD uint64_t *cm_m_pos(const CmDev &d, uint32_t r) { return d.mbuf + d.m_off[r]; }
-CM_HD uint8_t *cm_m_pcnt(const CmDev &d, uint32_t r) { return d.mcnt + d.m_off[r]; }
-CM_HD uint64_t *cm_m_neg(const CmDev &d, uint32_t r) { return d.mbuf + d.m_off[r] + d.ncp[r] + d.resc_p[r]; }
-CM_HD uint8_t *cm_m_ncnt(const CmDev &d, uint32_t r) { return d.mcnt + d.m_off[r] + d.ncp[r] + d.resc_p[r]; }
+struct CmMView { const uint64_t *pos, *neg; const uint8_t *pcnt, *ncnt; };
+CM_HD CmMView cm_m_view(const CmDev &d, uint32_t r) {
+  CmMView v;
+  if (cm_read_merged(d, r)) {
+    const uint32_t o = d.m_off[r], sh = d.ncp[r] + d.resc_p[r];
+    v.pos = d.mbuf + o; v.pcnt = d.mcnt + o; v.neg = d.mbuf + o + sh; v.ncnt = d.mcnt + o + sh;
+  } else {
+    const uint32_t o = d.hit_off[r], sh = d.n_pos_hit[r];
+    v.pos = d.hbuf + o; v.pcnt = d.hcnt + o; v.neg = d.hbuf + o + sh; v.ncnt = d.hcnt + o + sh;
+  }
+  return v;
+}
+CM_HD const uint64_t *cm_m_pos(const CmDev &d, uint32_t r) { return cm_m_view(d, r).pos; }
+CM_HD const uint8_t *cm_m_pcnt(const CmDev &d, uint32_t r) { return cm_m_view(d, r).pcnt; }
+CM_HD const uint64_t *cm_m_neg(const CmDev &d, uint32_t r) { return cm_m_view(d, r).neg; }
+CM_HD const uint8_t *cm_m_ncnt(const CmDev &d, uint32_t r) { return cm_m_view(d, r).ncnt; }
 CM_HD uint64_t *cm_f_pos(const CmDev &d, uint32_t r) { return d.fbuf + d.m_off[r]; }
 CM_HD uint8_t *cm_f_pcnt(const CmDev &d, uint32_t r) { return d.fcnt + d.m_off[r]; }
 CM_HD uint64_t *cm_f_neg(const CmDev &d, uint32_t r) { return d.fbuf + d.m_off[r] + d.ncp[r] + d.resc_p[r]; }
@@ -1421,8 +1435,9 @@
   d.force0[pair] = 0;
   if (d.p.single) {
     if (d.mm_cnt[r1] == 0 || d.mcp[r1] + d.mcn[r1] == 0) return false;
-    const uint64_t *mp = cm_m_pos(d, r1), *mn = cm_m_neg(d, r1);
-    const uint8_t *mpc = cm_m_pcnt(d, r1), *mnc = cm_m_ncnt(d, r1);
+    const CmMView v = cm_m_view(d, r1);
+    const uint64_t *mp = v.pos, *mn = v.neg;
+    const uint8_t *mpc = v.pcnt, *mnc = v.ncnt;
     uint64_t *fp = cm_f_pos(d, r1), *fn = cm_f_neg(d, r1);
     uint8_t *fpc = cm_f_pcnt(d, r1), *fnc = cm_f_ncnt(d, r1);
     for (uint32_t i = 0; i < d.mcp[r1]; ++i) { fp[i] = mp[i]; fpc[i] = mpc[i]; }
@@ -1444,8 +1459,9 @@
   if (!(nc1 > 0 && nc2 > 0)) return false;
   if (d.p.split) {
     for (uint32_t r = r1; r <= r2; ++r) {
-      const uint64_t *mp = cm_m_pos(d, r), *mn = cm_m_neg(d, r);
-      const uint8_t *mpc = cm_m_pcnt(d, r), *mnc = cm_m_ncnt(d, r);
+      const CmMView v = cm_m_view(d, r);
+      const uint64_t *mp = v.pos, *mn = v.neg;
+      const uint8_t *mpc = v.pcnt, *mnc = v.ncnt;
       uint64_t *fp = cm_f_pos(d, r), *fn = cm_f_neg(d, r);
       uint8_t *fpc = cm_f_pcnt(d, r), *fnc = cm_f_ncnt(d, r);
       for (uint32_t i = 0; i < d.mcp[r]; ++i) { fp[i] = mp[i]; fpc[i] = mpc[i]; }
@@ -1460,12 +1476,14 @@
 }
 CM_HD void cm_s4c_filter(const CmDev &d, uint32_t pair) {
   const uint32_t r1 = 2 * pair, r2 = r1 + 1;
+  const CmMView v1 = cm_m_view(d, r1), v2 = cm_m_view(d, r2);
+  const uint32_t mcp1 = d.mcp[r1], mcn1 = d.mcn[r1], mcp2 = d.mcp[r2], mcn2 = d.mcn[r2];
   uint32_t a, b;
-  cm_reduce_dir((uint32_t)d.p.max_insert, cm_m_pos(d, r1), cm_m_pcnt(d, r1), d.mcp[r1], cm_m_neg(d, r2),
-                cm_m_ncnt(d, r2), d.mcn[r2], cm_f_pos(d, r1), cm_f_pcnt(d, r1), &a, cm_f_neg(d, r2), cm_f_ncnt(d, r2), &b);
+  cm_reduce_dir((uint32_t)d.p.max_insert, v1.pos, v1.pcnt, mcp1, v2.neg, v2.ncnt, mcn2, cm_f_pos(d, r1), cm_f_pcnt(d, r1), &a, cm_f_neg(d, r2),
+                cm_f_ncnt(d, r2), &b);
   d.fcp[r1] = a; d.fcn[r2] = b;
-  cm_reduce_dir((uint32_t)d.p.max_insert, cm_m_neg(d, r1), cm_m_ncnt(d, r1), d.mcn[r1], cm_m_pos(d, r2),
-                cm_m_pcnt(d, r2), d.mcp[r2], cm_f_neg(d, r1), cm_f_ncnt(d, r1), &a, cm_f_pos(d, r2), cm_f_pcnt(d, r2), &b);
+  cm_reduce_dir((uint32_t)d.p.max_insert, v1.neg, v1.ncnt, mcn1, v2.pos, v2.pcnt, mcp2, cm_f_neg(d, r1), cm_f_ncnt(d, r1), &a, cm_f_pos(d, r2),
+                cm_f_pcnt(d, r2), &b);
   d.fcn[r1] = a; d.fcp[r2] = b;
 }
 CM_HD void cm_s4c_post(const CmDev &d, uint32_t pair) {
diff --git a/chromap_amd/csrc/cm_types.h b/chromap_amd/csrc/cm_types.h
--- a/chromap_amd/csrc/cm_types.h
+++ b/chromap_amd/csrc/cm_types.h
@@ -24,7 +24,7 @@
   CM_L_HIT_WAVE = 0, CM_L_HIT_B256A = 1, CM_L_HIT_B256B = 2, CM_L_HIT_SLAB = 3, CM_L_HIT_G16 = 4, CM_L_HIT_DECLINED = 5, CM_L_RS_WAVE = 6, CM_L_RS_B256A = 7,
   CM_L_RS_B256B = 8, CM_L_PF_BLOCK = 9, CM_L_HIT_B512 = 10, CM_L_RS_B512 = 11, CM_L_S5_WAVE = 12, CM_L_S6A_WAVE = 13, CM_L_PF_BLOCK_BIG = 14, CM_L_RS_SLAB = 15,
   CM_L_HIT_SERIAL = 16, CM_L_S6C_WAVE = 17, CM_L_S6A_BLOCK = 18, CM_L_PF_HUGE = 19, CM_L_S6C_BLOCK = 20, CM_L_HIT_WAVE_SMALL = 21, CM_L_S5_BLOCK = 22,
-  CM_L_SEARCH_WAVE = 23, CM_L_HIT_B1024 = 25, CM_L_RS_B1024 = 26, CM_L_PF_WAVE = 27, CM_L_S5_SMALL = 28, CM_L_S6A_SMALL = 29, CM_L_S6C_SMALL = 30,
+  CM_L_SEARCH_WAVE = 23, CM_L_S6C_MULTI = 24, CM_L_HIT_B1024 = 25, CM_L_RS_B1024 = 26, CM_L_PF_WAVE = 27, CM_L_S5_SMALL = 28, CM_L_S6A_SMALL = 29, CM_L_S6C_SMALL = 30,
   CM_L_SEARCH_WAVE_BIG = 31
 };
 #define CM_HV_LISTS 32
```

Result: slower. 439.7 (-19.7%).
